# JGCRI/hector

Hardware: AMD Instinct MI355X
Metric: ensemble-member simulated years/sec (higher is better)
Workload: dtype f64

## Files before the change

hector_amd/csrc/ensemble_core.cpp:

```cpp
#include "ensemble_core.hpp"

#include <atomic>
#include <chrono>
#include <cstdint>
#include <cstdio>
#include <cstdlib>
#include <algorithm>
#include <cmath>
#include <cstring>
#include <dlfcn.h>
#include <fstream>
#include <sstream>
#include <string>
#include <stdexcept>
#include <map>
#include <mutex>

hipError_t hx_launch_spinup(int B, const HxArgs *d_args, int nmem_launch, int *d_steps,
                            hipStream_t st);
int hx_track_value_rows(int B);
int hx_pair_available();
hipError_t hx_launch_run_pair(const HxArgs *d_args, int npad, bool heatflux, bool kpm, int iy_from,
                              int iy_to, hipStream_t st, bool cons, int nbiome);
hipError_t hx_launch_prewarm(const int *d_stop, long long max_ticks, double *d_sink, int waves,
                             const double *mem, unsigned long long n_mem, hipStream_t st);
hipError_t hx_launch_run(int B, const HxArgs *d_args, int npad, bool heatflux, bool kpm, int con,
                         int iy_from, int iy_to, hipStream_t st, bool two_wave, int cus);
int hx_doeclim_block_years();
void hx_fill_chem_table_host(double *t);
hipError_t hx_launch_broadcast(double *table, int nrows, int npad, hipStream_t st);
hipError_t hx_launch_broadcast_u32(unsigned *v, int npad, hipStream_t st);
hipError_t hx_launch_alk(const HxArgs *d_args, int nmem_launch, hipStream_t st);
hipError_t hx_launch_or_flags(unsigned *status, const double *flag_row, int npad, hipStream_t st);
hipError_t hx_launch_gas(const double *par, const double *ser, const double *h0, int nh, int ns,
                         int npad, double *n2o_out, double *rf_other_out, hipStream_t st);
hipError_t hx_launch_diag(int kind, const HxDiagArgs &a, double *out, hipStream_t st);
hipError_t hx_launch_slr(const double *tgav, int npad, int start_year, int iy_to, double *out,
                         size_t var_stride, hipStream_t st);
hipError_t hx_launch_gather(const double *src, const int *lane_of_member, double *dst, int n,
                            int npad, int nyears, hipStream_t st);
hipError_t hx_launch_stats(const double *var, int n, int npad, int iy0, int nyears,
                           double *stats, hipStream_t st);
hipError_t hx_launch_derive(const double *params, double *derived, const double *ker,
                            int ker_per_member, int ns, int nbiome, int npad, hipStream_t st);
hipError_t hx_launch_doeclim_kernel(const double *diff_row, double *ker, int ns, int count,
                                    int stride, hipStream_t st);
#ifdef HX_HOST_EMULATION
#include "hx_dev_post.h"
#else
hipError_t hx_launch_score(const double *var, int n, int npad, const int *iy, const double *obs,
                           const double *sigma, int nobs, int b0, int b1, double *out, hipStream_t st);
hipError_t hx_launch_metric(const double *var, int n, int npad, const void *groups, int ngroups,
                            const int *rows, int year_start, double *out, hipStream_t st);
hipError_t hx_launch_pair_metric(const double *a, const double *b, const double *bvec, int bvec_iy0, int n,
                                 int npad, const void *specs, int nspecs, double *out, hipStream_t st);
hipError_t hx_launch_series_ew(int op, const double *a, const double *b, const double *bvec, const double *base,
                               int npad, int ns, int y_lo, int y_hi, double c0, double c1, double *z,
                               hipStream_t st);
hipError_t hx_launch_series_base(const double *a, int npad, int r0, int r1, double *base, hipStream_t st);
hipError_t hx_launch_series_cumsum(const double *a, int npad, int ns, int y0, int y_hi, double *z,
                                   hipStream_t st);
hipError_t hx_launch_series_runmean(const double *a, int npad, int ns, int w, int back, int y_hi, double *z,
                                    hipStream_t st);
hipError_t hx_launch_series_permute(const double *src, const int *src_lane, int npad, int ns, double *dst,
                                    hipStream_t st);
hipError_t hx_launch_mseries_fill(const double *row, int ns, int npad, double *table, hipStream_t st);
hipError_t hx_launch_mseries_mix(const double *coeff, const int *member_of_lane, int n, int npad, const int *rows,
                                 const double *basis, int nrows, int nbasis, double *table, hipStream_t st);
hipError_t hx_launch_bin(const double *var, int n, int npad, int iy0, int nrows, const unsigned long long *q,
                         const double *edges, int K, unsigned long long *sums, hipStream_t stream);
hipError_t hx_launch_q_minmax(const double *var, int n, int npad, int iy0, int ny,
                              const unsigned long long *q, void *st, hipStream_t stream);
hipError_t hx_launch_q_init(const void *st, int ny, const double *probs, int np, int skip, int *lo,
                            unsigned long long *prefix, unsigned long long *rem, hipStream_t stream);
hipError_t hx_launch_q_hist(const double *var, int n, int npad, int iy0, int ny,
                            const unsigned long long *q, const int *lo, const unsigned long long *prefix,
                            int np, int aggregate, unsigned long long *hist, hipStream_t stream);
hipError_t hx_launch_q_pick(int ny, int *lo, unsigned long long *prefix, unsigned long long *rem, int np,
                            unsigned long long *hist, hipStream_t stream);
hipError_t hx_launch_mom_prepare(const unsigned long long *q_mem, const double *pred_mem, int npred, int n,
                                 int npad, const int *lane_of_member, const double *c,
                                 unsigned long long *q_lane, double *qd_lane, double *e_lane, hipStream_t st);
int hx_mom_chunks(int n);
hipError_t hx_launch_moments(const double *var, int n, int npad, int iy0, int nrows, const double *qd,
                             const double *e, int npred, const double *shift, double *part, double *out,
                             hipStream_t st);
hipError_t hx_launch_grp_prepare(const int *lab_mem, int n, int npad, const int *lane_of_member, int *lab_lane,
                                 hipStream_t st);
hipError_t hx_launch_gmom_prepare(const unsigned long long *q_mem, const double *pred_mem, const int *lab_mem,
                                  int npred, int n, int npad, const int *lane_of_member, const double *c,
                                  unsigned long long *q_lane, double *qd_lane, double *e_lane, int *lab_lane,
                                  hipStream_t st);
hipError_t hx_launch_gq_minmax(const double *var, int n, int npad, int iy0, int ny, const unsigned long long *q,
                               const int *lab, int G, void *st, hipStream_t stream);
hipError_t hx_launch_gq_hist(const double *var, int n, int npad, int iy0, int ny, const unsigned long long *q,
                             const int *lab, int G, const int *lo, const unsigned long long *prefix, int np,
                             unsigned long long *hist, hipStream_t stream);
hipError_t hx_launch_gbin(const double *var, int n, int npad, int iy0, int nrows, const unsigned long long *q,
                          const int *lab, int G, const double *edges, int K, unsigned long long *sums,
                          hipStream_t stream);
hipError_t hx_launch_gmoments(const double *var, int n, int npad, int iy0, int nrows, const double *qd,
                              const double *e, const int *lab, int G, int npred, const double *shift,
                              double *part, double *out, hipStream_t st);
int hx_sobol_chunks(int nb);
hipError_t hx_launch_sobol_prepare(const int *lane_of_member, int npad, int k, int nb, const unsigned char *use,
                                   int *tab, unsigned char *flag, hipStream_t st);
hipError_t hx_launch_sobol_part(const double *var, int npad, int iy0, int nrows, const int *tab, int nb, int k,
                                const unsigned char *flag, void *st, unsigned char *on, hipStream_t stream);
hipError_t hx_launch_sobol_sums(const double *var, int npad, int iy0, int nrows, const int *tab, int nb, int k,
                                const void *st, const unsigned char *on, double *part, double *sums, double *shift,
                                long long *npart, hipStream_t stream);
hipError_t hx_launch_co_mask(const double *va, int ia0, int na, const double *vb, int ib0, int nb, int npad,
                             unsigned long long *q_lane, double *qd_lane, hipStream_t st);
int hx_co_chunks(int n, int na, int nb);
hipError_t hx_launch_co_gram(const double *va, int ia0, int na, const double *vb, int ib0, int nb, int n,
                             int npad, int sym, const double *qd, const double *shift_a,
                             const double *shift_b, double *part, double *cross, hipStream_t st);
int hx_sw_padded(int n);
void hx_sw_pack(const double *whiten, int n, double *wf);
hipError_t hx_launch_score_whiten(const double *var, int nmem, int npad, const int *iy, const double *obs,
                                  const double *wf, int n, const double *base, double *out, hipStream_t st);
int hx_project_steps(int n);
void hx_project_pack(const double *basis, int n, int m, double *bf);
hipError_t hx_launch_project(const double *var, int nmem, int npad, const int *iy, const double *center,
// ... 9 lines not shown
namespace {

struct ParamDef {
  const char *name; int row; bool per_biome; const char *units; bool spinup;
};
const ParamDef kParams[] = {
    {"S", HXP_S, false, "degC", false},
    {"diff", HXP_DIFF, false, "cm2/s", false},
    {"qco2", HXP_QCO2, false, "W/m2", false},
    {"aero_scalar", HXP_AERO, false, "(unitless)", false},
    {"vol_scalar", HXP_VOL, false, "(unitless)", false},
    {"C0", HXP_C0, false, "ppmv CO2", true},
    {"tt", HXP_TT, false, "m3/s", true},
    {"tu", HXP_TU, false, "m3/s", true},
    {"twi", HXP_TWI, false, "m3/s", true},
    {"tid", HXP_TID, false, "m3/s", true},
    {"preind_surface_c", HXP_PRE_SURF, false, "Pg C", true},
    {"preind_interdeep_c", HXP_PRE_ID, false, "Pg C", true},
    {"lo_warming_ratio", HXP_LO_RATIO, false, "(unitless)", false},
    {"beta", HXPB_BETA, true, "(unitless)", false},
    {"q10_rh", HXPB_Q10, true, "(unitless)", false},
    {"warmingfactor", HXPB_WF, true, "(unitless)", false},
    {"npp_flux0", HXPB_NPP0, true, "Pg C/yr", true},
    {"veg_c", HXPB_VEG0, true, "Pg C", true},
    {"detritus_c", HXPB_DET0, true, "Pg C", true},
    {"soil_c", HXPB_SOIL0, true, "Pg C", true},
    {"permafrost_c", HXPB_PF0, true, "Pg C", true},
    {"f_nppv", HXPB_F_NPPV, true, "(unitless)", true},
    {"f_nppd", HXPB_F_NPPD, true, "(unitless)", true},
    {"f_litterd", HXPB_F_LITTERD, true, "(unitless)", true},
    {"rh_ch4_frac", HXPB_RH_CH4_FRAC, true, "(unitless)", false},
    {"pf_mu", HXPB_PF_MU, true, "degC", false},
    {"pf_sigma", HXPB_PF_SIGMA, true, "degC", false},
    {"fpf_static", HXPB_FPF_STATIC, true, "(unitless)", false},
};

struct OutDef { const char *name; int idx; };
const OutDef kOutputs[] = {
    {"sst", HXO_SST}, {"land_tas", HXO_TLAND}, {"CO2_concentration", HXO_CO2},
    {"global_tas", HXO_TGAV}, {"RF_tot", HXO_RF_TOT}, {"RF_CO2", HXO_RF_CO2},
    {"ocean_c", HXO_OCEAN_C}, {"HL_pH", HXO_HL_PH}, {"atmos_co2", HXO_ATMOS_C},
    {"permafrost_c", HXO_PERMAFROST_C}, {"heatflux", HXO_HEATFLUX},
    {"CH4_concentration", HXO_CH4}, {"O3_concentration", HXO_O3}, {"veg_c", HXO_VEG_C},
    {"detritus_c", HXO_DET_C}, {"soil_c", HXO_SOIL_C}, {"thawedp_c", HXO_THAWED_C},
    {"earth_c", HXO_EARTH_C}, {"NBP", HXO_NBP}, {"ocean_uptake", HXO_OCEAN_UPTAKE},
    {"timesteps", HXO_NSTASH}, {"solver_steps", HXO_NSTEPS}, {"LL_pH", HXO_LL_PH},
    {"sst_reported", HXO_SST_LO},
    {"NPP", HXO_NPP}, {"RH", HXO_RH}, {"rh_det", HXO_RH_DET}, {"rh_soil", HXO_RH_SOIL},
    {"HL_ocean_uptake", HXO_HL_UPTAKE}, {"LL_ocean_uptake", HXO_LL_UPTAKE},
    {"HL_downwelling", HXO_HL_DO}, {"atmos_c_residual", HXO_CA_RESIDUAL},
    {"rh_ch4", HXO_RH_CH4}, {"f_frozen", HXO_F_FROZEN}, {"gmst", HXO_GMST},
    {"heatflux_mixed", HXO_FLUX_MIXED}, {"heatflux_interior", HXO_FLUX_INTERIOR},
    {"HL_ocean_c", HXO_C_HL}, {"LL_ocean_c", HXO_C_LL}, {"IO_ocean_c", HXO_C_IO},
    {"DO_ocean_c", HXO_C_DO}, {"HL_PCO2", HXO_PCO2_HL}, {"LL_PCO2", HXO_PCO2_LL},
    {"TAU_OH", HXO_TAU_OH},
};
const char *kOutputNames[HXO_NVAR];

struct DerivedDef { const char *name; int kind; int box; const char *deps[4]; };
enum { DK_SLR = 100, DK_SL_RC, DK_SLR_NI, DK_SL_RC_NI };
const DerivedDef kDerived[] = {
    {"HL_sst", HXG_TEMP, 0, {"sst"}}, {"LL_sst", HXG_TEMP, 1, {"sst"}},
    {"HL_DIC", HXG_DIC, 0, {"HL_ocean_c"}}, {"LL_DIC", HXG_DIC, 1, {"LL_ocean_c"}},
    {"HL_CO3", HXG_CO3, 0, {"sst", "HL_pH", "HL_PCO2"}},
    {"LL_CO3", HXG_CO3, 1, {"sst", "LL_pH", "LL_PCO2"}},
    {"HL_OmegaAr", HXG_OMEGA_AR, 0, {"sst", "HL_pH", "HL_PCO2"}},
    {"LL_OmegaAr", HXG_OMEGA_AR, 1, {"sst", "LL_pH", "LL_PCO2"}},
    {"HL_OmegaCa", HXG_OMEGA_CA, 0, {"sst", "HL_pH", "HL_PCO2"}},
    {"LL_OmegaCa", HXG_OMEGA_CA, 1, {"sst", "LL_pH", "LL_PCO2"}},
    {"HL_Revelle", HXG_REVELLE, 0, {"sst", "HL_pH", "HL_PCO2", "HL_ocean_c"}},
    {"LL_Revelle", HXG_REVELLE, 1, {"sst", "LL_pH", "LL_PCO2", "LL_ocean_c"}},
    {"ocean_tas", HXG_OCEAN_TAS, -1, {"global_tas"}},
    {"RF_N2O", HXG_RF_N2O, -1, {"CO2_concentration", "CH4_concentration"}},
    {"RF_CH4", HXG_RF_CH4, -1, {"CH4_concentration"}},
    {"RF_H2O_strat", HXG_RF_H2O, -1, {"CH4_concentration"}},
    {"RF_O3_trop", HXG_RF_O3, -1, {"O3_concentration"}},
    {"slr", DK_SLR, -1, {"global_tas"}}, {"sl_rc", DK_SL_RC, -1, {"global_tas"}},
    {"slr_no_ice", DK_SLR_NI, -1, {"global_tas"}}, {"sl_rc_no_ice", DK_SL_RC_NI, -1, {"global_tas"}},
};
const DerivedDef *derived_of(const std::string &name) {
  for (const DerivedDef &d : kDerived) if (name == d.name) return &d;
  return nullptr;
}

}

const char *const *EnsembleCore::output_capabilities(int *count) {
  for (auto &o : kOutputs) kOutputNames[o.idx] = o.name;
  if (count) *count = HXO_BIOME0;
  return kOutputNames;
}

void EnsembleCore::check(hipError_t e, const char *what) const {
  if (e != hipSuccess)
    throw std::runtime_error(std::string("HIP error in ") + what + ": " + hipGetErrorString(e));
}

EnsembleCore::EnsembleCore(const std::string &scenario_path, int n_members, int device)
    : scen_(Scenario::load(scenario_path)), n_(n_members), B_(1), device_(device) {
  if (n_members <= 0) throw std::runtime_error("n_members must be > 0");
  npad_ = (n_ + HX_WAVE - 1) / HX_WAVE * HX_WAVE;
  int ndev = 0;
  hipError_t e = hipGetDeviceCount(&ndev);
  if (e != hipSuccess || ndev <= 0)
    throw std::runtime_error(
        "hector_amd: no HIP device available -- the ensemble integrator has no CPU path");
  if (device < 0 || device >= ndev) throw std::runtime_error("invalid device index");
  check(hipSetDevice(device_), "hipSetDevice");
#ifndef HX_HOST_EMULATION
  {
    hipDeviceProp_t prop;
    check(hipGetDeviceProperties(&prop, device_), "hipGetDeviceProperties");
    simds_ = 4 * prop.multiProcessorCount;
  }
#endif
  check(hipStreamCreate(&stream_), "hipStreamCreate");
  if (const char *e2 = std::getenv("HECTOR_AMD_PAIR_MAX_MEMBERS")) pair_max_members_ = std::atoi(e2);
  if (const char *e3 = std::getenv("HECTOR_AMD_TWO_WAVE_FROM")) two_wave_from_ = std::atoi(e3);
  if (const char *e4 = std::getenv("HECTOR_AMD_PAIR_ORDER")) pair_costly_with_cheap_ = std::atoi(e4) != 0;
  if (const char *e5 = std::getenv("HECTOR_AMD_KEY_ORDER")) key_order_mode_ = std::atoi(e5);
  if (const char *e6 = std::getenv("HECTOR_AMD_COST_MODEL")) cost_model_ = std::atoi(e6) != 0;
  if (const char *e7 = std::getenv("HECTOR_AMD_SIMDS")) simds_ = std::max(1, std::atoi(e7));
  if (const char *e8 = std::getenv("HECTOR_AMD_PREWARM_MS")) prewarm_ms_ = std::max(0, std::atoi(e8));
  try {
    check(hipEventCreate(&ev0_), "hipEventCreate");
    check(hipEventCreate(&ev1_), "hipEventCreate");
    init_from_scenario();
  } catch (...) {
    if (ev0_) (void)hipEventDestroy(ev0_);
    if (ev1_) (void)hipEventDestroy(ev1_);
    (void)hipStreamDestroy(stream_);
    throw;
  }
}

void EnsembleCore::init_from_scenario() {
  for (int v = 0; v < HXO_NVAR; ++v) { d_out_[v] = nullptr; out_enabled_[v] = false; }
  out_enabled_[HXO_SST] = out_enabled_[HXO_TLAND] = true;
  out_enabled_[HXO_CO2] = out_enabled_[HXO_TGAV] = true;
  biome_names_ = {"global"};
  params_.assign(HX_NPARAM(1), std::vector<double>((size_t)npad_, 0.0));
  row_uniform_.assign(HX_NPARAM(1), true);
  auto setrow = [&](int row, double v) { std::fill(params_[row].begin(), params_[row].end(), v); };
  const Scenario &s = scen_;
  tracking_year_ = (int)s.scalar("core", "trackingDate", 0.0);
  if (tracking_year_ >= 9999 || tracking_year_ < 0) tracking_year_ = 0;
  setrow(HXP_S, s.scalar("temperature", "S"));
  setrow(HXP_DIFF, s.scalar("temperature", "diff"));
  setrow(HXP_QCO2, s.scalar("temperature", "qco2"));
  setrow(HXP_AERO, s.scalar("forcing", "aero_scalar", 1.0));
  setrow(HXP_VOL, s.scalar("forcing", "vol_scalar", 1.0));
  setrow(HXP_C0, s.scalar("simpleNbox", "C0"));
  setrow(HXP_TT, s.scalar("ocean", "tt"));
  setrow(HXP_TU, s.scalar("ocean", "tu"));
  setrow(HXP_TWI, s.scalar("ocean", "twi"));
  setrow(HXP_TID, s.scalar("ocean", "tid"));
  setrow(HXP_PRE_SURF, s.scalar("ocean", "preind_surface_c", 900));
  setrow(HXP_PRE_ID, s.scalar("ocean", "preind_interdeep_c", 37100));
  setrow(HXP_LO_RATIO, s.scalar("temperature", "lo_warming_ratio", 0.0));
  out_enabled_[HXO_SST_LO] = s.scalar("temperature", "lo_warming_ratio", 0.0) != 0.0;
  const int r = HXP_NGLOBAL;
  setrow(r + HXPB_BETA, s.scalar("simpleNbox", "beta", 0.0));
  setrow(r + HXPB_Q10, s.scalar("simpleNbox", "q10_rh", 0.0));
  setrow(r + HXPB_WF, s.scalar("simpleNbox", "warmingfactor", 1.0));
  setrow(r + HXPB_NPP0, s.scalar("simpleNbox", "npp_flux0", 0.0));
  setrow(r + HXPB_VEG0, s.scalar("simpleNbox", "veg_c", 0.0));
// ... 333 lines not shown
  check(hipMalloc(&d_derived_, sizeof(double) * np * HX_NDERIVED(B_)), "hipMalloc derived");
  check(hipMalloc(&d_lane_of_member_, sizeof(int) * np), "hipMalloc lane map");
  if (history_) {
    check(hipMalloc(&d_hist_, sizeof(double) * ns * np * HX_NSTATE(B_)), "hipMalloc state history");
    check(hipMalloc(&d_hist_status_, sizeof(unsigned) * ns * np), "hipMalloc status history");
  }
  if (spin_record_) {
    const size_t bytes = sizeof(double) * (size_t)kc_.max_spinup * HXSR_N * np;
    size_t free_b = 0, total_b = 0;
    if (hipMemGetInfo(&free_b, &total_b) == hipSuccess && bytes > free_b)
      throw std::runtime_error("spinup record: " + std::to_string(kc_.max_spinup) + " steps x " +
                               std::to_string((int)HXSR_N) + " variables x " + std::to_string(npad_) +
                               " members need " + std::to_string(bytes >> 20) + " MiB of device memory, " +
                               std::to_string(free_b >> 20) + " MiB are free");
    check(hipMalloc(&d_spin_rec_, bytes), "hipMalloc spinup record");
    check(hipMemsetAsync(d_spin_rec_, 0, bytes, stream_), "zero");
  }
  hist_valid_to_ = 0;
  check(hipMalloc(&d_dpart_, sizeof(double) * np * 2 * (size_t)hx_doeclim_block_years()),
        "hipMalloc doeclim partial sums");
  check(hipMalloc(&d_cost_, sizeof(double) * np), "hipMalloc lane cost");
  check(hipMalloc(&d_wave_clk_, sizeof(long long) * 4 * (np / HX_WAVE)), "hipMalloc wave clock");
  check(hipMemsetAsync(d_wave_clk_, 0, sizeof(long long) * 4 * (np / HX_WAVE), stream_), "zero");
  check(hipMalloc(&d_bscratch_, sizeof(double) * np * (size_t)(3 * B_)), "hipMalloc biome scratch");
  check(hipMemsetAsync(d_bscratch_, 0, sizeof(double) * np * (size_t)(3 * B_), stream_), "zero");
  cost_from_iy_ = -1;
  for (int v = 0; v < HXO_NVAR; ++v)
    if (out_enabled_[v]) {
      check(hipMalloc(&d_out_[v], sizeof(double) * ns * np), "hipMalloc out");
      check(hipMemsetAsync(d_out_[v], 0, sizeof(double) * ns * np, stream_), "memset out");
    }
  check(hipMemcpyAsync(d_shared_, shared_.data(), sizeof(double) * shared_.size(),
                       hipMemcpyHostToDevice, stream_), "upload shared");
  layout_dirty_ = false;
  params_dirty_ = true;
  rows_all_dirty_ = true;
  need_spinup_ = true; spin_valid_ = false;
}

HxBuffers EnsembleCore::buffers() const {
  HxBuffers b;
  b.params = d_params_; b.derived = d_derived_; b.state = d_state_; b.status = d_status_; b.shared = d_shared_;
  b.ker = d_ker_;
  b.dpart = d_dpart_;
  b.dpart2 = d_dpart_ ? d_dpart_ + (size_t)npad_ * hx_doeclim_block_years() : nullptr;
  for (int v = 0; v < HXO_NVAR; ++v) b.out[v] = d_out_[v];
  b.hist = d_hist_; b.hist_status = d_hist_status_;
  for (int k = 0; k < HXM_N; ++k) b.mseries[k] = d_mseries_[k];
  b.uparams = d_uparams_;
  b.uderived = d_uparams_ ? d_uparams_ + HX_NPARAM(B_) : nullptr;
  b.uni_k = (row_uniform_[HXP_TT] && row_uniform_[HXP_TU] && row_uniform_[HXP_TWI] && row_uniform_[HXP_TID]) ? 1 : 0;
  b.uni_avc = (row_uniform_[HXP_AERO] && row_uniform_[HXP_VOL] && row_uniform_[HXP_C0]) ? 1 : 0;
  b.uni_wf = 1;
  for (int bb = 0; bb < B_; ++bb) if (!row_uniform_[HXP_NGLOBAL + bb * HXPB_N + HXPB_WF]) b.uni_wf = 0;
  b.track_out_f = d_track_out_f_; b.track_out_v = d_track_out_v_;
  b.trk_slots = trk_iy() >= 0 ? scen_.ns() - trk_iy() + 1 : 0;
  b.uni_landk = b.uni_bio = 1;
  for (int bb = 0; bb < B_; ++bb) {
    const int r = HXP_NGLOBAL + bb * HXPB_N;
    for (int k : {HXPB_NPP0, HXPB_F_NPPV, HXPB_F_NPPD, HXPB_F_LITTERD, HXPB_RH_CH4_FRAC, HXPB_FPF_STATIC})
      if (!row_uniform_[r + k]) b.uni_landk = 0;
    for (int k : {HXPB_BETA, HXPB_PF_MU, HXPB_PF_SIGMA})
      if (!row_uniform_[r + k]) b.uni_bio = 0;
  }
  b.stash_diag = b.biome_diag = b.out_rare = 0;
  for (int v = 0; v < HXO_NVAR; ++v)
    if (d_out_[v] && v != HXO_SST && v != HXO_TLAND && v != HXO_CO2 && v != HXO_TGAV) b.out_rare = 1;
  for (int v = HXO_NPP; v <= HXO_CA_RESIDUAL; ++v) if (d_out_[v]) b.stash_diag = 1;
  for (int v = HXO_BIOME0; v < HXO_NVAR; ++v) if (d_out_[v]) b.biome_diag = 1;
  for (int bb = 0; bb < HX_BDYN; ++bb)
    if (d_out_[HXO_B(HXOB_NPP, bb)] || d_out_[HXO_B(HXOB_RH, bb)]) b.stash_diag = 1;
  b.out_mask0 = 0; b.ms_mask = 0;
  for (int v = 0; v < HXO_BIOME0; ++v) if (d_out_[v]) b.out_mask0 |= 1ull << v;
  for (int bb = 0; bb < HX_BDYN; ++bb)
    if (d_out_[HXO_B(HXOB_NPP, bb)] || d_out_[HXO_B(HXOB_RH, bb)]) b.out_mask0 |= 1ull << HX_OM_BIOME_FLUX;
  if (b.biome_diag) b.out_mask0 |= 1ull << HX_OM_BIOME_ANY;
  for (int k = 0; k < HXM_N; ++k) if (d_mseries_[k]) b.ms_mask |= 1u << k;
  b.n = n_; b.npad = npad_; b.ker_per_member = ker_per_member_ ? 1 : 0;
  b.nbiome = B_;
  b.cost = d_cost_;
  b.spin_rec = d_spin_rec_;
  b.bscratch = d_bscratch_;
  b.wave_clk = d_wave_clk_;
  return b;
}

int EnsembleCore::resolve_param(const std::string &capability, const ParamRef **) const {
  std::string biome, var = capability;
  size_t dot = capability.find('.');
  if (dot != std::string::npos) { biome = capability.substr(0, dot); var = capability.substr(dot + 1); }
  for (const ParamDef &d : kParams) {
    if (var != d.name) continue;
    if (!d.per_biome) {
      if (!biome.empty()) throw std::runtime_error("variable " + var + " takes no biome prefix");
      return d.row;
    }
    int b = -1;
    if (biome.empty()) biome = "global";
    for (int i = 0; i < B_; ++i) if (biome_names_[i] == biome) b = i;
    if (b < 0)
      throw std::runtime_error("Biome '" + biome + "' missing from biome list. Hit this error "
                               "while trying to retrieve variable: '" + capability + "'.");
    return HXP_NGLOBAL + b * HXPB_N + d.row;
  }
  throw std::runtime_error("Unknown variable name while parsing: " + capability);
}

static const ParamDef &def_of(const std::string &capability) {
  std::string var = capability;
  size_t dot = capability.find('.');
  if (dot != std::string::npos) var = capability.substr(dot + 1);
  for (const ParamDef &d : kParams) if (var == d.name) return d;
  throw std::runtime_error("Unknown variable name while parsing: " + capability);
}

namespace {
struct SharedParamDef { const char *name, *section, *units; };
const SharedParamDef kSharedParams[] = {
    {"M0", "CH4", "ppbv CH4"}, {"Tsoil", "CH4", "Years"}, {"Tstrat", "CH4", "Years"},
    {"N0", "N2O", "ppbv N2O"}, {"PO3", "ozone", "DU O3"}, {"TOH0", "OH", "Years"},
    {"delta_co2", "forcing", "(unitless)"}, {"delta_ch4", "forcing", "(unitless)"},
    {"delta_n2o", "forcing", "(unitless)"}, {"rho_bc", "forcing", "W/m2/Tg"},
    {"rho_oc", "forcing", "W/m2/Tg"}, {"rho_so2", "forcing", "W/m2/Gg"},
    {"rho_nh3", "forcing", "W/m2/Tg"},
    {"TN2O0", "N2O", "Years"}, {"UC_N2O", "N2O", "Tg/ppbv"},
};
}

static std::string shared_param_section(const Scenario &scen, const std::string &capability,
                                        std::string *units, std::string *key = nullptr) {
  if (key) *key = capability;
  for (const SharedParamDef &d : kSharedParams)
    if (capability == d.name) { if (units) *units = d.units; return d.section; }
  for (const Halocarbon &h : scen.halocarbons) {
    if (capability == "rho_" + h.name) { if (units) *units = "W/m2/pptv"; return h.name + "_halocarbon"; }
    if (capability == "delta_" + h.name) { if (units) *units = "(unitless)"; return h.name + "_halocarbon"; }
    if (capability == "tau_" + h.name) {
      if (units) *units = "Years";
      if (key) *key = "tau";
      return h.name + "_halocarbon";
    }
  }
  return "";
}

static bool gas_member_capable(const Scenario &scen, const std::string &capability) {
  if (capability == "N0" || capability == "TN2O0" || capability == "UC_N2O") return true;
  for (const Halocarbon &h : scen.halocarbons)
    if (capability == "rho_" + h.name || capability == "delta_" + h.name || capability == "tau_" + h.name)
      return true;
  return false;
}

void EnsembleCore::setvar(const std::string &capability, const double *values, int nvalues,
                          const char *units) {
  if (std::count(capability.begin(), capability.end(), '.') > 1)
    throw std::runtime_error("Invalid input variable: '" + capability + "'");
  if (capability == "trackingDate") {
    set_tracking_date((int)values[0]);
    return;
  }
  {
    std::string expect, key;
    const std::string sec = shared_param_section(scen_, capability, &expect, &key);
    if (!sec.empty()) {
      if (units && units[0] && expect != units)
// ... 564 lines not shown
      if (!std::isnan(pt.second[(size_t)m])) pts.emplace_hint(pts.end(), pt.first, pt.second[(size_t)m]);
    const std::vector<double> dense = Scenario::densify_points(pts, capability, scen_.start, scen_.end);
    for (size_t iy = 0; iy < dense.size(); ++iy) ms[iy * (size_t)n_ + (size_t)m] = dense[iy];
  }
}

void EnsembleCore::upload_member_series() {
  const size_t np = (size_t)npad_, ns = (size_t)scen_.ns();
  std::vector<double> flat;
  for (const MemberSeriesDef &d : kMemberSeries) {
    const std::vector<double> &ms = member_series_[d.k];
    if (ms.empty() && !mix_[d.k].nbasis) {
      if (d_mseries_[d.k]) {
        check(hipStreamSynchronize(stream_), "sync member series");
        (void)hipFree(d_mseries_[d.k]);
        d_mseries_[d.k] = nullptr;
      }
      continue;
    }
    if (!d_mseries_[d.k]) check(hipMalloc(&d_mseries_[d.k], sizeof(double) * ns * np), "hipMalloc member series");
    if (!ms.empty()) {
      flat.assign(ns * np, 0.0);
      for (size_t iy = (size_t)d.lag; iy < ns; ++iy)
        for (size_t l = 0; l < np; ++l)
          flat[iy * np + l] = ms[(iy - (size_t)d.lag) * n_ + (size_t)std::min(member_of_lane_[l], n_ - 1)];
      check(hipMemcpyAsync(d_mseries_[d.k], flat.data(), sizeof(double) * flat.size(),
                           hipMemcpyHostToDevice, stream_), "upload member series");
      check(hipStreamSynchronize(stream_), "sync member series");
    }
    if (mix_[d.k].nbasis) build_mix_table(d.k, d.lag, d.section, d.name, !ms.empty());
  }
  upload_args();
  mseries_dirty_ = false;
}

void EnsembleCore::build_mix_table(int k, int lag, const std::string &section, const std::string &capability,
                                   bool dense) {
  const MemberMix &mx = mix_[k];
  const size_t np = (size_t)npad_, ns = (size_t)scen_.ns(), ny = mx.years.size(), K = (size_t)mx.nbasis;
  std::vector<int> ints(member_of_lane_.begin(), member_of_lane_.begin() + (std::ptrdiff_t)np);
  std::vector<size_t> col;
  for (size_t i = 0; i < ny; ++i) {
    const size_t r = (size_t)(mx.years[i] - scen_.start + lag);
    if (r < ns) { ints.push_back((int)r); col.push_back(i); }
  }
  const size_t nr = col.size();
  std::vector<double> dbl(ns + K * nr);
  if (!dense && scen_.has_series(section, capability)) {
    const std::vector<double> &base = scen_.series(section, capability);
    for (size_t iy = (size_t)lag; iy < ns; ++iy) dbl[iy] = base[iy - (size_t)lag];
  }
  for (size_t kk = 0; kk < K; ++kk)
    for (size_t j = 0; j < nr; ++j) dbl[ns + kk * nr + j] = mx.basis[kk * ny + col[j]];
  const size_t b_dbl = sizeof(double) * dbl.size(), b_coeff = sizeof(double) * K * (size_t)n_,
               b_int = sizeof(int) * ints.size();
  if (b_dbl + b_coeff + b_int > mix_cap_) {
    check(hipStreamSynchronize(stream_), "sync mix scratch");
    if (d_mix_) (void)hipFree(d_mix_);
    d_mix_ = nullptr; mix_cap_ = 0;
    check(hipMalloc(&d_mix_, b_dbl + b_coeff + b_int), "hipMalloc mix scratch");
    mix_cap_ = b_dbl + b_coeff + b_int;
  }
  double *d_dbl = reinterpret_cast<double *>(d_mix_), *d_coeff = d_dbl + dbl.size();
  int *d_int = reinterpret_cast<int *>(d_mix_ + b_dbl + b_coeff);
  check(hipMemcpyAsync(d_dbl, dbl.data(), b_dbl, hipMemcpyHostToDevice, stream_), "upload mix basis");
  check(hipMemcpyAsync(d_coeff, mx.coeff.data(), b_coeff, hipMemcpyHostToDevice, stream_), "upload mix coefficients");
  check(hipMemcpyAsync(d_int, ints.data(), b_int, hipMemcpyHostToDevice, stream_), "upload mix rows");
  if (!dense) check(hx_launch_mseries_fill(d_dbl, (int)ns, npad_, d_mseries_[k], stream_), "member series fill kernel");
  if (nr)
    check(hx_launch_mseries_mix(d_coeff, d_int, n_, npad_, d_int + np, d_dbl + ns, (int)nr, mx.nbasis,
                                d_mseries_[k], stream_), "member series mix kernel");
  check(hipStreamSynchronize(stream_), "sync member series mix");
}

void EnsembleCore::upload_args() {
  HxArgs a;
  a.buf = buffers();
  a.kc = kc_;
  for (int k = 0; k < HXM_N; ++k)
    if (!member_series_[k].empty()) a.kc.con_mask |= constraint_bit(k);
  member_con_mask_ = a.kc.con_mask & ~kc_.con_mask;
  check(hipMemcpyAsync(d_args_, &a, sizeof a, hipMemcpyHostToDevice, stream_), "upload args");
  check(hipStreamSynchronize(stream_), "sync args");
}

void EnsembleCore::run_gas_kernel() {
  gas_dirty_ = false;
  auto fr = [](void *p) { if (p) (void)hipFree(p); };
  if (gas_member_.empty()) {
    if (d_mseries_[HXM_N2O]) {
      sync();
      fr(d_mseries_[HXM_N2O]); fr(d_mseries_[HXM_RF_OTHER]);
      d_mseries_[HXM_N2O] = d_mseries_[HXM_RF_OTHER] = nullptr;
      upload_args();
    }
    return;
  }
  const Scenario &s = scen_;
  const size_t np = (size_t)npad_, ns = (size_t)s.ns();
  const size_t nh = s.halocarbons.size();
  std::vector<size_t> horder(nh);
  for (size_t h = 0; h < nh; ++h) horder[h] = h;
  std::sort(horder.begin(), horder.end(), [&](size_t a, size_t b) {
    return s.halocarbons[a].name < s.halocarbons[b].name;
  });
  auto member_value = [&](const std::string &cap, double dflt, size_t lane) {
    auto it = gas_member_.find(cap);
    if (it == gas_member_.end()) return dflt;
    return it->second[(size_t)std::min(member_of_lane_[lane], n_ - 1)];
  };
  std::vector<double> par((3 + 3 * nh) * np), ser((4 + 2 * nh) * ns), h0(nh);
  for (size_t l = 0; l < np; ++l) {
    par[l] = member_value("N0", s.scalar("N2O", "N0"), l);
    par[np + l] = member_value("TN2O0", s.scalar("N2O", "TN2O0"), l);
    par[2 * np + l] = member_value("UC_N2O", s.scalar("N2O", "UC_N2O"), l);
    for (size_t k = 0; k < nh; ++k) {
      const Halocarbon &H = s.halocarbons[horder[k]];
      par[(3 + 3 * k) * np + l] = member_value("tau_" + H.name, H.tau, l);
      par[(4 + 3 * k) * np + l] = component_disabled(H.name + "_halocarbon")
                                      ? 0.0 : member_value("rho_" + H.name, H.rho, l);
      par[(5 + 3 * k) * np + l] = member_value("delta_" + H.name, H.delta, l);
    }
  }
  const auto &n2o_em = s.series("N2O", "N2O_emissions");
  const auto &n2o_nat = s.series("N2O", "N2O_natural_emissions");
  const std::vector<double> nanv(ns, std::nan(""));
  auto con = [&](const std::string &sec, const std::string &key) -> const std::vector<double> & {
    return s.has_series(sec, key) ? s.series(sec, key) : nanv;
  };
  const auto &n2o_con = con("N2O", "N2O_constrain");
  const auto albedo = s.has_series("simpleNbox", "RF_albedo") ? s.series("simpleNbox", "RF_albedo")
                                                                : std::vector<double>(ns, -0.2);
  const auto misc = s.has_series("forcing", "RF_misc") ? s.series("forcing", "RF_misc")
                                                        : std::vector<double>(ns, 0.0);
  for (size_t iy = 0; iy < ns; ++iy) {
    ser[iy] = n2o_em[iy] + n2o_nat[iy];
    ser[ns + iy] = n2o_con[iy];
    ser[2 * ns + iy] = albedo[iy];
    ser[3 * ns + iy] = misc[iy];
  }
  for (size_t k = 0; k < nh; ++k) {
    const Halocarbon &H = s.halocarbons[horder[k]];
    const auto &hc = con(H.name + "_halocarbon", H.name + "_constrain");
    h0[k] = H.H0;
    for (size_t iy = 0; iy < ns; ++iy) {
      const double emissMol = H.emissions[iy] / H.molarMass * 1.0;
      ser[(4 + 2 * k) * ns + iy] = emissMol / (0.1 * 1.8);
      ser[(5 + 2 * k) * ns + iy] = hc[iy];
    }
  }
  sync();
  fr(d_gas_par_); fr(d_gas_ser_);
  d_gas_par_ = d_gas_ser_ = nullptr;
  double *d_h0 = nullptr;
  check(hipMalloc(&d_gas_par_, sizeof(double) * par.size()), "hipMalloc gas parameters");
  check(hipMalloc(&d_gas_ser_, sizeof(double) * (ser.size() + nh)), "hipMalloc gas series");
  d_h0 = d_gas_ser_ + ser.size();
  if (!d_mseries_[HXM_N2O]) {
    check(hipMalloc(&d_mseries_[HXM_N2O], sizeof(double) * ns * np), "hipMalloc N2O series");
    check(hipMalloc(&d_mseries_[HXM_RF_OTHER], sizeof(double) * ns * np), "hipMalloc RF series");
  }
  check(hipMemcpyAsync(d_gas_par_, par.data(), sizeof(double) * par.size(), hipMemcpyHostToDevice,
                       stream_), "upload gas parameters");
  check(hipMemcpyAsync(d_gas_ser_, ser.data(), sizeof(double) * ser.size(), hipMemcpyHostToDevice,
                       stream_), "upload gas series");
  check(hipMemcpyAsync(d_h0, h0.data(), sizeof(double) * nh, hipMemcpyHostToDevice, stream_),
// ... 452 lines not shown
  if (!(kc_.delta_n2o >= -1 && kc_.delta_n2o <= 1)) throw std::runtime_error("bad delta N2O value");
  if (!(kc_.delta_co2 >= -1 && kc_.delta_co2 <= 1)) throw std::runtime_error("bad delta CO2 value");
}

void EnsembleCore::prepare() {
  check(hipSetDevice(device_), "hipSetDevice");
  StageClock clk;
  if (layout_dirty_) { alloc_device(); clk.lap("alloc_device"); }
  if (shared_dirty_ || params_dirty_ || need_spinup_) prewarm_begin();
  if (shared_dirty_) {
    build_shared();
    check(hipMemcpyAsync(d_shared_, shared_.data(), sizeof(double) * shared_.size(),
                         hipMemcpyHostToDevice, stream_), "upload shared");
    check(hipStreamSynchronize(stream_), "sync shared");
    shared_dirty_ = false;
    params_dirty_ = true;
  }
  if (params_dirty_) {
    check_parameters();
    clk.lap("check_parameters");
    upload_params();
    clk.lap("upload_params");
    if (order_changed_)
      for (int k = 0; k < HXM_N; ++k)
        if (!member_series_[k].empty() || mix_[k].nbasis) mseries_dirty_ = true;
    gas_dirty_ = true;
  }
  if (gas_dirty_ || (!gas_member_.empty() && !d_mseries_[HXM_N2O])) run_gas_kernel();
  if (mseries_dirty_) upload_member_series();
  clk.lap("gas kernel / member series");
  if (!need_spinup_) return;
  bool uniform = true;
  for (const ParamDef &d : kParams) {
    if (!d.spinup) continue;
    if (d.per_biome) {
      for (int b = 0; b < B_; ++b)
        if (!row_uniform_[HXP_NGLOBAL + b * HXPB_N + d.row]) uniform = false;
    } else if (!row_uniform_[d.row]) uniform = false;
  }
  const size_t np = (size_t)npad_;
  const bool reuse = spin_valid_ && uniform && spin_uniform_ && !std::getenv("HECTOR_AMD_ALWAYS_SPINUP");
  spin_uniform_ = uniform;
  if (reuse) {
    check(hipMemcpyAsync(d_state_, d_state_ + np * HX_NSTATE(B_), sizeof(double) * np * HX_NSTATE(B_),
                         hipMemcpyDeviceToDevice, stream_), "restore state");
    check(hipMemcpyAsync(d_status_, d_status_ + 2 * np, sizeof(unsigned) * np, hipMemcpyDeviceToDevice,
                         stream_), "restore status");
  } else {
    if (!uniform || std::getenv("HECTOR_AMD_PREWARM_STOP")) prewarm_end();
    check(hipEventRecord(ev0_, stream_), "event");
    check(hx_launch_spinup(B_, d_args_, uniform ? 1 : npad_, d_spin_steps_, stream_), "spinup");
    check(hx_launch_alk(d_args_, uniform ? 1 : npad_, stream_), "alkalinity tuning");
    if (uniform) {
      check(hx_launch_broadcast(d_state_, HX_NSTATE(B_), npad_, stream_), "broadcast state");
      check(hx_launch_broadcast_u32(d_status_, npad_, stream_), "broadcast status");
      check(hx_launch_broadcast_u32(reinterpret_cast<unsigned *>(d_spin_steps_), npad_, stream_),
            "broadcast steps");
      for (int v = 0; v < HXO_NVAR; ++v)
        if (d_out_[v]) check(hx_launch_broadcast(d_out_[v], 1, npad_, stream_), "broadcast out");
    }
    check(hipMemcpyAsync(d_status_ + 2 * np, d_status_, sizeof(unsigned) * np, hipMemcpyDeviceToDevice,
                         stream_), "keep spinup status");
  }
  check(hx_launch_or_flags(d_status_, d_derived_ + (size_t)HXD_FLAG * npad_, npad_, stream_),
        "derive flags");
  if (!reuse)
    check(hipMemcpyAsync(d_state_ + np * HX_NSTATE(B_), d_state_, sizeof(double) * np * HX_NSTATE(B_),
                         hipMemcpyDeviceToDevice, stream_), "snapshot state");
  check(hipMemcpyAsync(d_status_ + np, d_status_, sizeof(unsigned) * np, hipMemcpyDeviceToDevice,
                       stream_), "snapshot status");
  if (reuse) {
    spin_ms_ = 0.0;
    clk.lap("post-spinup state reused");
  } else {
    check(hipEventRecord(ev1_, stream_), "event");
    check(hipEventSynchronize(ev1_), "spinup sync");
    float ms = 0;
    check(hipEventElapsedTime(&ms, ev0_, ev1_), "elapsed");
    spin_ms_ = ms;
    clk.lap("spinup + snapshot (waited)");
  }
  spin_valid_ = uniform;
  need_spinup_ = false;
  ++out_epoch_;
  last_iy_ = 0;
  hist_valid_to_ = 0;
  dirty_from_iy_ = -1;
}

void EnsembleCore::reset(double date) {
  ++out_epoch_;
  if (date < scen_.start) {
    need_spinup_ = true; spin_valid_ = false;
    last_iy_ = 0;
    dirty_from_iy_ = -1;
    return;
  }
  const int iy = (int)date - scen_.start;
  if (iy == 0 && !(need_spinup_ || layout_dirty_ || params_dirty_)) maybe_calibrate_lanes();
  if (need_spinup_ || layout_dirty_ || params_dirty_) {
    if (iy != 0) throw std::runtime_error("reset: the core has pending changes from date 0");
    prepare();
    return;
  }
  if (iy == last_iy_) return;
  if (iy > last_iy_) throw std::runtime_error("reset: date is after the current date");
  const size_t np = (size_t)npad_, rows = (size_t)HX_NSTATE(B_);
  sync();
  if (iy == 0) {
    check(hipMemcpyAsync(d_state_, d_state_ + np * rows, sizeof(double) * np * rows,
                         hipMemcpyDeviceToDevice, stream_), "restore state");
    check(hipMemcpyAsync(d_status_, d_status_ + np, sizeof(unsigned) * np, hipMemcpyDeviceToDevice,
                         stream_), "restore status");
  } else {
    if (!d_hist_ || iy > hist_valid_to_)
      throw std::runtime_error("reset: no state history for that date (enable_history() before "
                               "running; only reset(0) and reset(startDate) work without it)");
    check(hipMemcpyAsync(d_state_, d_hist_ + (size_t)iy * rows * np, sizeof(double) * np * rows,
                         hipMemcpyDeviceToDevice, stream_), "restore state from history");
    check(hipMemcpyAsync(d_status_, d_hist_status_ + (size_t)iy * np, sizeof(unsigned) * np,
                         hipMemcpyDeviceToDevice, stream_), "restore status from history");
  }
  last_iy_ = iy;
  cost_from_iy_ = -1;
  if (dirty_from_iy_ >= iy) dirty_from_iy_ = -1;
}

void EnsembleCore::prewarm_begin() {
#ifndef HX_HOST_EMULATION
  if (prewarm_ms_ <= 0 || prewarm_on_) return;
  {
    const double now = std::chrono::duration<double>(std::chrono::steady_clock::now().time_since_epoch()).count();
    if (last_gpu_activity_s_ >= 0 && now - last_gpu_activity_s_ < 0.005) return;
  }
  if (!aux_stream_) check(hipStreamCreateWithFlags(&aux_stream_, hipStreamNonBlocking), "prewarm stream");
  if (!d_prewarm_) check(hipMalloc((void **)&d_prewarm_, 64 + sizeof(double) * 1024), "prewarm flag");
  check(hipMemsetAsync(d_prewarm_, 0, 64, aux_stream_), "prewarm flag");
  int waves = 3 * simds_;
  if (const char *e = std::getenv("HECTOR_AMD_PREWARM_WAVES")) waves = std::max(1, std::min(8 * simds_, std::atoi(e)));
  const bool sweep = std::getenv("HECTOR_AMD_PREWARM_MEM") && d_out_[HXO_SST];
  check(hx_launch_prewarm(reinterpret_cast<const int *>(d_prewarm_), (long long)prewarm_ms_ * 100000ll,
                          reinterpret_cast<double *>(d_prewarm_ + 64), waves,
                          sweep ? d_out_[HXO_SST] : nullptr,
                          sweep ? (unsigned long long)scen_.ns() * (unsigned long long)npad_ : 0ull, aux_stream_),
        "prewarm kernel");
  prewarm_on_ = true;
#endif
}
void EnsembleCore::prewarm_end() {
#ifndef HX_HOST_EMULATION
  if (!prewarm_on_) return;
  check(hipMemsetAsync(d_prewarm_, 1, 4, stream_), "prewarm stop");
  prewarm_on_ = false;
  last_run_prewarmed_ = true;
#endif
}

void EnsembleCore::run(double runtodate) {
  prepare();
  if (runtodate < 0.0) runtodate = scen_.end;
  if (runtodate > scen_.end)
    throw std::runtime_error("Requested run-to date is after the configured end date.");
  const int target = (int)runtodate - scen_.start;
  if (dirty_from_iy_ >= 0 && dirty_from_iy_ < last_iy_) {
    const int back = (d_hist_ && dirty_from_iy_ <= hist_valid_to_) ? dirty_from_iy_ : 0;
    dirty_from_iy_ = -1;
    reset((double)(scen_.start + back));
  }
  dirty_from_iy_ = -1;
  if (target < last_iy_ + 1) return;
  if (last_iy_ == 0) {
    check(hipMemsetAsync(d_cost_, 0, sizeof(double) * (size_t)npad_, stream_), "zero lane cost");
    cost_from_iy_ = 0;
  }
  last_run_prewarmed_ = false;
  prewarm_end();
  check(hipEventRecord(ev0_, stream_), "event");
  const bool hf = d_out_[HXO_HEATFLUX] || d_out_[HXO_FLUX_MIXED] || d_out_[HXO_FLUX_INTERIOR];
  const int con_mask = kc_.con_mask | member_con_mask_;
  bool ext = con_mask != 0;
  for (int v = HXO_NPP; v < HXO_NVAR; ++v) if (d_out_[v]) ext = true;
  for (int k = 0; k < HXM_N; ++k) if (d_mseries_[k]) ext = true;
  const bool force_nbp = getenv("HECTOR_AMD_EXTENDED_NBP") != nullptr;
  int con = ext ? (((con_mask & HXC_NBP) || force_nbp) ? 1 : -1) : 0;
  if (con == -1 && con_mask == 0 && !getenv("HECTOR_AMD_EXTENDED_CONS")) {
    bool any_ms = false;
    for (int k = 0; k < HXM_N; ++k) if (d_mseries_[k]) any_ms = true;
    if (!any_ms && B_ >= 1 && B_ <= 4) con = -2;
  }
  if (d_track_out_f_) {
    if (con_mask & (HXC_CO2 | HXC_NBP))
      throw std::runtime_error("carbon tracking together with a CO2 or NBP constraint is not "
                               "supported (the constraint residual is an untracked source)");
    con = 2;
  }
  const int pair_cons = con_mask & (HXC_CO2 | HXC_TAS | HXC_FTOT | HXC_CH4);
  bool plain = (con_mask & ~(HXC_CO2 | HXC_TAS | HXC_FTOT | HXC_CH4)) == 0 && !d_track_out_f_ &&
               !(pair_cons && ker_per_member_);
  for (int k = 0; k < HXM_N; ++k) if (d_mseries_[k]) plain = false;
  bool pair = hx_pair_available() && B_ <= 4 && plain && n_ <= pair_max_members_;
  if (B_ > 1 && (ker_per_member_ || d_out_[HXO_HEATFLUX])) pair = false;
  for (int v = 0; v < HXO_NVAR && pair; ++v)
    if (d_out_[v]) {
      static const int ok[] = {HXO_SST, HXO_TLAND, HXO_CO2, HXO_TGAV, HXO_NSTASH, HXO_RF_TOT, HXO_RF_CO2,
                               HXO_ATMOS_C, HXO_OCEAN_C, HXO_OCEAN_UPTAKE, HXO_HL_PH, HXO_LL_PH, HXO_CH4,
                               HXO_O3, HXO_NBP, HXO_VEG_C, HXO_DET_C, HXO_SOIL_C, HXO_PERMAFROST_C,
                               HXO_THAWED_C, HXO_EARTH_C, HXO_HEATFLUX, HXO_NPP, HXO_RH, HXO_RH_DET,
                               HXO_RH_SOIL, HXO_RH_CH4, HXO_F_FROZEN, HXO_GMST};
      if (std::find(std::begin(ok), std::end(ok), v) == std::end(ok)) pair = false;
      if (B_ > 1 && (v == HXO_NPP || v == HXO_RH || v == HXO_RH_DET || v == HXO_RH_SOIL)) pair = false;
    }
  last_run_pair_ = pair;
  const bool w2 = !pair && con <= 1 && two_wave_expected();
  last_run_w2_ = w2;
  last_run_con_ = con;
  if (pair)
    check(hx_launch_run_pair(d_args_, npad_, d_out_[HXO_HEATFLUX] != nullptr, ker_per_member_, last_iy_, target,
                             stream_, pair_cons != 0, B_), "run kernel (pair)");
  else
  check(hx_launch_run(B_, d_args_, npad_, hf || con == 2, ker_per_member_, con, last_iy_, target,
                      stream_, w2, simds_ / 4),
        "run kernel");
  check(hipEventRecord(ev1_, stream_), "event");
  run_timed_ = true;
  slr_valid_to_ = -1;
  ++out_epoch_;
  if (d_hist_) hist_valid_to_ = target;
  last_iy_ = target;
}

void EnsembleCore::sync() {
  check(hipStreamSynchronize(stream_), "stream sync");
  last_gpu_activity_s_ = std::chrono::duration<double>(std::chrono::steady_clock::now().time_since_epoch()).count();
  if (run_timed_) {
    float ms = 0;
    check(hipEventElapsedTime(&ms, ev0_, ev1_), "elapsed");
    run_ms_ = ms;
    run_timed_ = false;
  }
}

int EnsembleCore::wave_clock(long long *ticks, int cap) {
  if (!d_wave_clk_ || last_iy_ == 0) return 0;
  sync();
  const int nw = (npad_ / HX_WAVE) * (last_run_pair_ ? 2 : 1);
  std::vector<long long> t((size_t)nw * 2);
  check(hipMemcpy(t.data(), d_wave_clk_, sizeof(long long) * t.size(), hipMemcpyDeviceToHost), "wave clock");
  long long t0 = t[0];
  for (int w = 0; w < nw; ++w) t0 = std::min(t0, t[(size_t)2 * w]);
  const int n = std::min(nw, cap);
  for (int w = 0; w < n; ++w) { ticks[2 * w] = t[(size_t)2 * w] - t0; ticks[2 * w + 1] = t[(size_t)2 * w + 1] - t0; }
  return n;
}

bool EnsembleCore::fetch_host(const std::string &capability_in, int year0, int year1,
                              double *out_host) {
  const std::string capability = capability_in.compare(0, 4, "Fadj") == 0
// ... 380 lines not shown
  {
    static const char *const combos[][3] = {{"pH", "LL_pH", "HL_pH"}, {"PCO2", "LL_PCO2", "HL_PCO2"},
                                            {"DIC", "LL_DIC", "HL_DIC"}, {"CO3", "LL_CO3", "HL_CO3"},
                                            {"ML_ocean_c", "LL_ocean_c", "HL_ocean_c"}};
    for (auto &c : combos)
      if (capability == c[0]) {
        const size_t cnt = (size_t)(year1 - year0 + 1) * (size_t)n_;
        std::vector<double> hl(cnt);
        fetchvars(c[1], year0, year1, out_host);
        fetchvars(c[2], year0, year1, hl.data());
        const bool sum = capability == "ML_ocean_c";
        const double part_high = 0.15, part_low = 1 - 0.15;
        for (size_t i = 0; i < cnt; ++i)
          out_host[i] = sum ? out_host[i] + hl[i] : part_low * out_host[i] + part_high * hl[i];
        return;
      }
  }
  const bool n2o_members = capability == "N2O_concentration" && d_mseries_[HXM_N2O];
  const DerivedDef *dd = derived_of(capability);
  const int si = find_series(capability);
  const int v = (dd || n2o_members || si >= 0) ? -1 : out_index(capability);
  if (!dd && !n2o_members && si < 0 && !d_out_[v])
    throw std::runtime_error("variable " + capability + " was not enabled with set_outputs()");
  if (si >= 0 && (year0 < scen_.start || year1 > scen_.start + series_[(size_t)si].valid_iy || year1 < year0))
    throw std::runtime_error("fetchvars: dates must lie between startDate and " +
                             std::to_string(scen_.start + series_[(size_t)si].valid_iy) + ", the date series " +
                             capability + " was defined at");
  if (si < 0 && (year0 < scen_.start || year1 > last_date() || year1 < year0))
    throw std::runtime_error("fetchvars: dates must lie between startDate and the current date");
  sync();
  const int iy0 = year0 - scen_.start, ny = year1 - year0 + 1;
  const size_t need = (size_t)ny * (size_t)n_;
  if (need > gather_cap_) {
    if (d_gather_) (void)hipFree(d_gather_);
    d_gather_ = nullptr;
    check(hipMalloc(&d_gather_, sizeof(double) * need), "hipMalloc gather");
    gather_cap_ = need;
  }
  const double *src = nullptr;
  if (dd) {
    const size_t dneed = (size_t)ny * (size_t)npad_;
    if (dneed > diag_cap_) {
      if (d_diag_) (void)hipFree(d_diag_);
      d_diag_ = nullptr;
      check(hipMalloc(&d_diag_, sizeof(double) * dneed), "hipMalloc diag");
      diag_cap_ = dneed;
    }
    compute_derived(capability, iy0, ny, d_diag_);
    src = d_diag_;
  } else if (si >= 0) {
    series_to_current_lanes(series_[(size_t)si]);
    src = series_[(size_t)si].block + (size_t)iy0 * npad_;
  } else if (n2o_members) {
    src = d_mseries_[HXM_N2O] + (size_t)iy0 * npad_;
  } else {
    src = d_out_[v] + (size_t)iy0 * npad_;
  }
  check(hx_launch_gather(src, d_lane_of_member_, d_gather_, n_, npad_, ny, stream_), "gather");
  if (row_pitch)
    check(hipMemcpy2DAsync(out_host, sizeof(double) * row_pitch, d_gather_, sizeof(double) * (size_t)n_,
                           sizeof(double) * (size_t)n_, (size_t)ny, hipMemcpyDeviceToHost, stream_), "fetch");
  else
    check(hipMemcpyAsync(out_host, d_gather_, sizeof(double) * need, hipMemcpyDeviceToHost, stream_),
          "fetch");
  check(hipStreamSynchronize(stream_), "fetch sync");
}

const double *EnsembleCore::device_var(const std::string &capability, int *npad) {
  const PostSource ps = post_source(capability, "hx_device_var");
  if (ps.v >= 0 && !d_out_[ps.v])
    throw std::runtime_error("variable " + capability + " was not enabled with set_outputs()");
  if (npad) *npad = npad_;
  return ps.block;
}

void EnsembleCore::stats_device(const std::string &capability, int year0, int year1,
                                double *d_stats) {
  stats_async(capability, year0, year1, d_stats);
  check(hipStreamSynchronize(stream_), "stats sync");
}

void EnsembleCore::stats_async(const std::string &capability, int year0, int year1,
                               double *d_stats) {
  const PostSource ps = post_source(capability, "stats");
  if (ps.v >= 0 && !d_out_[ps.v])
    throw std::runtime_error("variable " + capability + " was not enabled with set_outputs()");
  if (year0 < scen_.start || year1 > scen_.start + ps.last_iy || year1 < year0)
    throw std::runtime_error("stats: dates must lie between startDate and the current date");
  check(hx_launch_stats(ps.block, n_, npad_, year0 - scen_.start, year1 - year0 + 1, d_stats,
                        stream_), "stats kernel");
}

void EnsembleCore::status(unsigned *out_host) {
  prepare();
  sync();
  std::vector<unsigned> tmp((size_t)npad_);
  check(hipMemcpy(tmp.data(), d_status_, sizeof(unsigned) * (size_t)npad_, hipMemcpyDeviceToHost),
        "status");
  for (int i = 0; i < n_; ++i) out_host[i] = tmp[(size_t)lane_of_member_[(size_t)i]];
}

void EnsembleCore::state_row(int row, double *out_host) {
  prepare();
  sync();
  if (row < 0 || row >= HX_NSTATE(B_)) throw std::runtime_error("state_row: bad row");
  std::vector<double> tmp((size_t)npad_);
  check(hipMemcpy(tmp.data(), d_state_ + (size_t)row * npad_, sizeof(double) * (size_t)npad_,
                  hipMemcpyDeviceToHost), "state row");
  for (int i = 0; i < n_; ++i) out_host[i] = tmp[(size_t)lane_of_member_[(size_t)i]];
}

int EnsembleCore::spinup_steps(int member) {
  prepare();
  sync();
  int v = 0;
  if (member < 0 || member >= n_) throw std::runtime_error("spinup_steps: bad member index");
  check(hipMemcpy(&v, d_spin_steps_ + lane_of_member_[(size_t)member], sizeof(int),
                  hipMemcpyDeviceToHost), "steps");
  return v;
}


int EnsembleCore::member_score(const std::string &capability, const int *years, const double *obs,
                               const double *sigma, int n, int base_year0, int base_year1,
                               double *out_host) {
  if (n < 1 || !years || !obs || !out_host)
    throw std::runtime_error("hx_member_score: n < 1 or a null argument");
  const PostSource ps = post_source(capability, "hx_member_score");
  if (ps.v >= 0 && !d_out_[ps.v])
    throw std::runtime_error("variable " + capability + " was not enabled with set_outputs()");
  const int last = scen_.start + ps.last_iy;
  const bool has_base = base_year0 <= base_year1;
  std::vector<int> iy((size_t)n);
  int used = 0;
  for (int i = 0; i < n; ++i) {
    if (years[i] < scen_.start || years[i] > last)
      throw std::runtime_error("hx_member_score: dates must lie between startDate and the current date");
    iy[(size_t)i] = years[i] - scen_.start;
    if (obs[i] == obs[i]) ++used;
  }
  if (has_base && (base_year0 < scen_.start || base_year1 > last))
    throw std::runtime_error("hx_member_score: the reference period must lie between startDate and the current date");
  if (!d_lane_of_member_) throw std::runtime_error("hx_member_score: run the core first");
  sync();
  const size_t nn = (size_t)n, doubles = 2 * nn + (size_t)npad_ + (size_t)n_;
  const size_t bytes = sizeof(double) * doubles + sizeof(int) * nn;
  if (bytes > score_cap_) {
    if (d_score_) (void)hipFree(d_score_);
    d_score_ = nullptr; score_cap_ = 0;
    check(hipMalloc(&d_score_, bytes), "hipMalloc score");
    score_cap_ = bytes;
  }
  double *d_obs = d_score_, *d_sig = d_obs + nn, *d_lane = d_sig + nn, *d_mem = d_lane + npad_;
  int *d_iy = reinterpret_cast<int *>(d_mem + n_);
  check(hipMemcpyAsync(d_obs, obs, sizeof(double) * nn, hipMemcpyHostToDevice, stream_), "score obs");
  if (sigma)
    check(hipMemcpyAsync(d_sig, sigma, sizeof(double) * nn, hipMemcpyHostToDevice, stream_), "score sigma");
  check(hipMemcpyAsync(d_iy, iy.data(), sizeof(int) * nn, hipMemcpyHostToDevice, stream_), "score years");
  check(hx_launch_score(ps.block, n_, npad_, d_iy, d_obs, sigma ? d_sig : nullptr, n,
                        has_base ? base_year0 - scen_.start : 1, has_base ? base_year1 - scen_.start : 0,
                        d_lane, stream_), "score kernel");
  check(hx_launch_gather(d_lane, d_lane_of_member_, d_mem, n_, npad_, 1, stream_), "score gather");
  check(hipMemcpyAsync(out_host, d_mem, sizeof(double) * (size_t)n_, hipMemcpyDeviceToHost, stream_), "score fetch");
  check(hipStreamSynchronize(stream_), "score sync");
  return used;
}

int hxq_host_start(const unsigned long long *st, unsigned long long *pre) {
  *pre = 0;
  if (st[3] == 0) return 0;
  const unsigned long long kmin = ~st[0], diff = kmin ^ st[1];
  if (!diff) { *pre = kmin; return 0; }
  int lo = 0;
  while (lo < 64 && (diff >> lo)) ++lo;
  if (lo < 64) *pre = (kmin >> lo) << lo;
  return lo;
}
unsigned long long hxq_host_target(double p, unsigned long long W) {
  const double t = std::ceil(p * (double)W);
  return t < 1.0 ? 1ull : (unsigned long long)t;
}
void hxq_host_pick(int lo, const unsigned long long *hist, unsigned long long *prefix,
                   unsigned long long *rem) {
  const int shift = lo >= 8 ? lo - 8 : 0;
  unsigned long long cum = 0, bin = 255;
  for (unsigned long long b = 0; b < 256; ++b) {
// ... 1442 lines not shown
```

hector_amd/csrc/ensemble_core.hpp:

```cpp
#pragma once
#include <hip/hip_runtime.h>

#include <cstdint>
#include <map>
#include <string>
#include <vector>

#include "../../include/hector_amd.h"
#include "hx_layout.h"
#include "hx_scenario.hpp"

namespace hx {

int hx_cost_models_export_file(const char *path);
int hx_cost_models_load_file(const char *path);

struct PairCall {
  const char *cap_b;
  const double *b_vec;
  int b_year0, b_year1;
  const hx_pair_metric *specs;
  int nspecs;
};

class EnsembleCore {
 public:
  EnsembleCore(const std::string &scenario_path, int n_members, int device);
  ~EnsembleCore();
  EnsembleCore(const EnsembleCore &) = delete;
  EnsembleCore &operator=(const EnsembleCore &) = delete;

  int n_members() const { return n_; }
  int n_biomes() const { return B_; }
  int start_date() const { return scen_.start; }
  int end_date() const { return scen_.end; }
  int last_date() const { return scen_.start + last_iy_; }
  const std::vector<std::string> &biomes() const { return biome_names_; }

  void setvar(const std::string &capability, const double *values, int nvalues,
              const char *units);
  void getvar(const std::string &capability, double *out) const;

  void split_biome(const std::vector<std::string> &names, const double *fveg,
                   const double *fdet, const double *fsoil, const double *fpf,
                   const double *fnpp);
  void split_biome_of(const std::string &old_biome, const std::vector<std::string> &names,
                      const double *fveg, const double *fdet, const double *fsoil,
                      const double *fpf, const double *fnpp);
  void create_biome(const std::string &biome);
  void delete_biome(const std::string &biome);
  void rename_biome(const std::string &oldname, const std::string &newname);
  int biome_index(const std::string &biome) const;

  void set_outputs(const std::vector<std::string> &capabilities);
  void set_member_sorting(bool on);
  void set_lane_calibration(bool on) { calibrate_lanes_ = on; }
  bool lanes_calibrated() const { return !lane_cost_.empty(); }
  int lane_order_source() const { return lane_order_source_; }
  void set_cost_model(bool on) { cost_model_ = on; }
  void set_prewarm(int ms) { prewarm_ms_ = ms < 0 ? 0 : (ms > 200 ? 200 : ms); }
  int prewarm_ms() const { return prewarm_ms_; }
  bool last_run_prewarmed() const { return last_run_prewarmed_; }
  void enable_history(bool on);
  void enable_spinup_record(bool on);
  static const std::vector<std::string> &spinup_record_vars();
  int spinup_record(int member, double *values, int max_steps);
  void setvar_dated(const std::string &capability, const int *years, const double *values,
                    int n, const char *units);
  void lane_of_member(int *out);
  void setvar_dated_members(const std::string &capability, const int *years, const double *values,
                            int nyears, const char *units);
  void setvar_dated_mix(const std::string &capability, const int *years, int nyears, const double *basis,
                        int nbasis, const double *coeff, const char *units);
  void check_dated_mix(const std::string &capability, const int *years, int nyears, const double *basis,
                       int nbasis, const double *coeff, const char *units) const;
  static const char *const *output_capabilities(int *count);

  void reset(double date);
  void run(double runtodate);
  void sync();
  void fetchvars(const std::string &capability, int year0, int year1, double *out_host,
                 size_t row_pitch = 0);
  bool host_output(const std::string &capability);
  void set_tracking_date(int year);
  int tracking_date() const { return tracking_year_; }
  std::vector<std::string> tracking_pools() const;
  void tracking_data(int member, int year0, int year1, double *values, double *fractions,
                     unsigned long long *source_masks = nullptr);
  std::string run_name() const;
  void var_info(const std::string &capability, std::string *component, std::string *units) const;
  const std::vector<std::string> &halocarbon_names() const { return halo_names_; }
  const double *device_var(const std::string &capability, int *npad);
  void stats_device(const std::string &capability, int year0, int year1, double *d_stats);
  void stats_async(const std::string &capability, int year0, int year1, double *d_stats);
  int member_score(const std::string &capability, const int *years, const double *obs,
                   const double *sigma, int n, int base_year0, int base_year1, double *out_host);
  void member_score_whitened(const std::string &capability, const int *years, const double *obs,
                             const double *whiten, int n, int base_year0, int base_year1, double *out_host);
  void member_project(const std::string &capability, const int *years, const double *center,
                      const double *basis, int n, int m, int base_year0, int base_year1, double *out_host,
                      size_t row_pitch = 0);
  void quantiles(const std::string &capability, int year0, int year1, const unsigned long long *q,
                 const double *probs, int nprobs, double *out_host, long long *n_part);
  void q_begin(const std::string &capability, int year0, int year1, const unsigned long long *q,
               int nprobs, unsigned long long *st_host);
  void q_pass(const int *lo, const unsigned long long *prefix, unsigned long long *hist_host);
  void member_metrics(const std::string &capability, const hx_metric *specs, int nspecs,
                      double *out_host, const char *fn = "hx_member_metrics");
  void metric_quantiles(const std::string &capability, const hx_metric *specs, int nspecs,
                        const unsigned long long *q, const double *probs, int nprobs, double *out_host,
                        long long *n_part);
  void mq_begin(const std::string &capability, const hx_metric *specs, int nspecs,
                const unsigned long long *q, int nprobs, unsigned long long *st_host);
  void bin_sums(const std::string &capability, int year0, int year1, const unsigned long long *q,
                const double *edges, int nedges, unsigned long long *sums_host);
  void metric_bin_sums(const std::string &capability, const hx_metric *specs, int nspecs,
                       const unsigned long long *q, const double *edges, int nedges,
                       unsigned long long *sums_host);
  void mom_begin(const std::string &capability, int year0, int year1, const hx_metric *specs, int nspecs,
                 const unsigned long long *q, const double *pred, int npred, const double *c,
                 unsigned long long *st_host, const char *fn);
  void mom_finish(const double *shift_host, double *sums_host);
  void grp_quantiles(const std::string &capability, int year0, int year1, const hx_metric *specs, int nspecs,
                     const int *labels, int ngroups, const unsigned long long *q, const double *probs,
                     int nprobs, double *out_host, long long *n_part, const char *fn);
  void grp_q_begin(const std::string &capability, int year0, int year1, const hx_metric *specs, int nspecs,
                   const int *labels, int ngroups, const unsigned long long *q, int nprobs,
                   unsigned long long *st_host, const char *fn);
  void grp_bin_sums(const std::string &capability, int year0, int year1, const hx_metric *specs, int nspecs,
                    const int *labels, int ngroups, const unsigned long long *q, const double *edges,
                    int nedges, unsigned long long *sums_host, const char *fn);
  void grp_mom_begin(const std::string &capability, int year0, int year1, const hx_metric *specs, int nspecs,
                     const int *labels, int ngroups, const unsigned long long *q, const double *pred,
                     int npred, const double *c, unsigned long long *st_host, const char *fn);
  void grp_mom_finish(const double *shift_host, double *sums_host);
  void member_pair_metrics(const std::string &cap_a, const PairCall &pc, double *out_host, size_t row_pitch = 0);
  void pair_metric_quantiles(const std::string &cap_a, const PairCall &pc, const unsigned long long *q,
                             const double *probs, int nprobs, double *out_host, long long *n_part);
  void pmq_begin(const std::string &cap_a, const PairCall &pc, const unsigned long long *q, int nprobs,
                 unsigned long long *st_host);
  void pair_metric_bin_sums(const std::string &cap_a, const PairCall &pc, const unsigned long long *q,
                            const double *edges, int nedges, unsigned long long *sums_host);
  void pair_mom_begin(const std::string &cap_a, const PairCall &pc, const unsigned long long *q,
                      const double *pred, int npred, const double *c, unsigned long long *st_host);
  void comom_check(const std::string &cap_a, int a0, int a1, const std::string *cap_b, int b0, int b1);
  void comom_begin(const std::string &cap_a, int a0, int a1, const std::string *cap_b, int b0, int b1,
                   const unsigned long long *q, unsigned long long *st_host);
  void comom_finish(const double *shift_host, double *sums_host, double *cross_host);
  void sobol_check(const std::string &capability, int year0, int year1, const hx_metric *specs, int nspecs,
                   const char *fn);
  void sobol_begin(const std::string &capability, int year0, int year1, const hx_metric *specs, int nspecs,
                   int k, int n_base, const unsigned char *use, const char *fn);
  void sobol_finish(double *shift_host, double *sums_host, long long *n_part_host);
  void series_define(const std::string &name, const std::string &a, const hx_series_op &op);
  void series_drop(const std::string &name);
  void series_list(std::vector<std::string> *names, std::vector<int> *valid_to) const;
  int device() const { return device_; }
  void status(unsigned *out_host);
  void state_row(int row, double *out_host);
  int spinup_steps(int member);

  double last_run_kernel_ms() const { return run_ms_; }
  bool component_output_enabled(const std::string &section) const { return scen_.scalar(section, "output", 1.0) > 0; }
  void set_pair_kernel_limit(int max_members) { pair_max_members_ = max_members < 0 ? 0 : max_members; }
  void set_two_wave_from(int min_members) { two_wave_from_ = min_members; }
  int wave_clock(long long *ticks, int cap);
  const char *last_run_kernel() const { return last_run_pair_ ? "pair" : last_run_w2_ ? "run2" : "run"; }
  int last_run_variant() const { return last_run_con_; }
  double last_spinup_ms() const { return spin_ms_; }
  hipStream_t stream() const { return stream_; }

 private:
  struct ParamRef { int row; bool per_biome; const char *units; bool affects_spinup; };
  int resolve_param(const std::string &capability, const ParamRef **ref) const;
  int out_index(const std::string &capability) const;
  void build_shared();
  void alloc_device();
  void free_device();
  void upload_params();
  void prepare();
  HxBuffers buffers() const;
  void check(hipError_t e, const char *what) const;

  Scenario scen_;
  int n_, npad_, B_, device_;
  std::vector<std::string> biome_names_;
  std::vector<std::vector<double>> params_;
  std::vector<bool> row_uniform_;
  std::vector<int> member_of_lane_, lane_of_member_;
  bool sort_members_ = true, calibrate_lanes_ = true;
  std::vector<double> lane_cost_;
  double *d_cost_ = nullptr;
  long long *d_wave_clk_ = nullptr;
  double *d_bscratch_ = nullptr;
  int cost_from_iy_ = -1;
  void maybe_calibrate_lanes();
  uint64_t cost_model_key(const std::vector<int> &varying) const;
  void fit_cost_model(const std::vector<double> &member_cost);
  bool predict_cost(const std::vector<int> &varying, std::vector<double> &out) const;
  int lane_order_source_ = 0;
  bool cost_model_ = true, cost_fitted_ = false;
  void assign_lanes();
  bool params_dirty_ = true, need_spinup_ = true, layout_dirty_ = true, ker_per_member_ = false;
  std::vector<char> row_dirty_;
  bool rows_all_dirty_ = true, order_changed_ = true;
  std::vector<int> uploaded_order_;
  bool spin_valid_ = false;
  int last_iy_ = 0;
  HxConst kc_{};
  std::vector<double> member_series_[HXM_N];
  std::map<int, std::vector<double>> member_points_[HXM_N];
  void densify_member_constraint(int k, const std::string &capability);
  double *d_mseries_[HXM_N] = {};
  bool mseries_dirty_ = false;
  void upload_member_series();
  struct MemberMix {
    int nbasis = 0;
    std::vector<int> years;
    std::vector<double> basis, coeff;
    bool covers(int year) const;
  };
  MemberMix mix_[HXM_N];
  char *d_mix_ = nullptr;
  size_t mix_cap_ = 0;
  void build_mix_table(int k, int lag, const std::string &section, const std::string &capability, bool dense);
  void upload_args();
  bool component_disabled(const std::string &section) const;
  void check_component_enabled(const std::string &capability) const;
  std::map<std::string, std::vector<double>> gas_member_;
  double *d_gas_par_ = nullptr, *d_gas_ser_ = nullptr;
  void run_gas_kernel();
  bool gas_dirty_ = false;
  int member_con_mask_ = 0;
  void init_from_scenario();
  std::vector<std::string> halo_names_;
  std::vector<std::vector<double>> halo_conc_;
  std::vector<double> shared_, ker_;
  bool out_enabled_[HXO_NVAR];
  double *d_params_ = nullptr, *d_state_ = nullptr, *d_shared_ = nullptr, *d_ker_ = nullptr;
  double *d_out_[HXO_NVAR];
  unsigned *d_status_ = nullptr;
  int *d_spin_steps_ = nullptr;
  HxArgs *d_args_ = nullptr;
  double *d_uparams_ = nullptr;
  int tracking_year_ = 0;
  double *d_track_out_f_ = nullptr, *d_track_out_v_ = nullptr;
  int trk_iy() const {
    return (tracking_year_ > scen_.start && tracking_year_ <= scen_.end) ? tracking_year_ - scen_.start : -1;
  }
  double *d_derived_ = nullptr, *d_dpart_ = nullptr, *d_gather_ = nullptr, *d_hist_ = nullptr;
  unsigned *d_hist_status_ = nullptr;
  void remap_biome_outputs(const std::vector<int> &old_of_new);
  bool history_ = false, shared_dirty_ = false;
  bool spin_record_ = false, spin_uniform_ = false;
  double *d_spin_rec_ = nullptr;
  int hist_valid_to_ = 0;
  int dirty_from_iy_ = -1;
  int *d_lane_of_member_ = nullptr;
  size_t gather_cap_ = 0, diag_cap_ = 0;
  double *d_diag_ = nullptr, *d_slr_ = nullptr;
  int slr_valid_to_ = -1;
  void check_parameters() const;
  bool fetch_host(const std::string &capability, int year0, int year1, double *out_host);
  void compute_derived(const std::string &capability, int iy0, int ny, double *dst);
  double *d_score_ = nullptr;
  size_t score_cap_ = 0;
  double *d_whiten_ = nullptr;
  size_t whiten_cap_ = 0;
  double *d_project_ = nullptr;
  size_t project_cap_ = 0;
  unsigned long long *d_q_ = nullptr;
  unsigned long long *d_qstate_ = nullptr;
  unsigned long long *d_qhist_ = nullptr;
  size_t qstate_cap_ = 0, qhist_cap_ = 0;
  const double *q_src_ = nullptr;
  int q_iy0_ = 0, q_ny_ = 0, q_np_ = 0;
  bool q_weighted_ = false;
  int post_flags_ = 0;
  const double *q_check(const std::string &capability, int year0, int year1, int nprobs,
                        const char *fn = "hx_ensemble_quantiles");
  void q_upload(const unsigned long long *q, int ny, int np);
  void q_select(const double *src, int iy0, int ny, const unsigned long long *q, const double *probs,
                int np, double *out_host, long long *n_part);
  void q_begin_block(const double *src, int iy0, int ny, const unsigned long long *q, int np,
                     unsigned long long *st_host);
  void bin_block(const double *src, int iy0, int nrows, const unsigned long long *q, const double *edges,
                 int nedges, unsigned long long *sums_host);
  unsigned char *d_metplan_ = nullptr;
  double *d_met_ = nullptr;
  size_t metplan_cap_ = 0, met_cap_ = 0;
  unsigned long long *d_bin_ = nullptr;
// ... 77 lines not shown
```

hector_amd/csrc/hx_dev_member.h:

```cpp
#pragma once

extern __shared__ double hx_dyn_park[][64];

namespace {

#define HX_FENCE() asm volatile("" ::: "memory")

#if !defined(HX_HOST_EMULATION) && !defined(HX_NO_SROW)
#define HX_SROW(p) asm("" : "+s"(p))
#else
#define HX_SROW(p)
#endif
#if !defined(HX_HOST_EMULATION) && !defined(HX_NO_VOFF)
#define HX_VOFF(o) asm("" : "+v"(o))
#else
#define HX_VOFF(o)
#endif

enum HxPark {
  PK_CH4 = 0, PK_SST, PK_EOS, PK_TLAND, PK_TWIN, PK_TL_M1, PK_TL_M2, PK_F_PREV,
  PK_BASE_TOT, PK_BASE_CO2,
  PK_LN_CH4, PK_LN_CO2R,
  PK_AERO, PK_VOL,
  PK_D0,
// ... 179 lines not shown
struct LandK<HX_DYN> {
  ParamCol npp0, f_nppv, f_nppd, f_litterd, rh_ch4_frac, fpf_static;
};
template <int B>
__device__ __forceinline__ void load_landk(const Member<B> &m, LandK<B> &k) {
  HX_FENCE();
  if constexpr (B == HX_DYN) {
    const ParamCol c{m.upar, m.bufp->params, m.npad, m.moff, 0};
    k.npp0 = c; k.npp0.col = HXPB_NPP0; k.f_nppv = c; k.f_nppv.col = HXPB_F_NPPV;
    k.f_nppd = c; k.f_nppd.col = HXPB_F_NPPD; k.f_litterd = c; k.f_litterd.col = HXPB_F_LITTERD;
    k.rh_ch4_frac = c; k.rh_ch4_frac.col = HXPB_RH_CH4_FRAC;
    k.fpf_static = c; k.fpf_static.col = HXPB_FPF_STATIC;
  } else if constexpr (hx_w2<B>()) {
    const int r = HXP_NGLOBAL;
    if (m.upar) {
      hx_ccd u = m.upar + r;
      k.npp0[0] = u[HXPB_NPP0]; k.f_nppv[0] = u[HXPB_F_NPPV]; k.f_nppd[0] = u[HXPB_F_NPPD];
      k.f_litterd[0] = u[HXPB_F_LITTERD]; k.rh_ch4_frac[0] = u[HXPB_RH_CH4_FRAC];
      k.fpf_static[0] = u[HXPB_FPF_STATIC];
    } else {
      const double *p = m.bufp->params;
      k.npp0[0] = w2_ld<true>(p, m.npad, r + HXPB_NPP0, m.moff);
      k.f_nppv[0] = w2_ld<true>(p, m.npad, r + HXPB_F_NPPV, m.moff);
      k.f_nppd[0] = w2_ld<true>(p, m.npad, r + HXPB_F_NPPD, m.moff);
      k.f_litterd[0] = w2_ld<true>(p, m.npad, r + HXPB_F_LITTERD, m.moff);
      k.rh_ch4_frac[0] = w2_ld<true>(p, m.npad, r + HXPB_RH_CH4_FRAC, m.moff);
      k.fpf_static[0] = w2_ld<true>(p, m.npad, r + HXPB_FPF_STATIC, m.moff);
    }
  } else if constexpr (B == 1) {
    constexpr int o = hx_pkb1<B>();
    k.npp0[0] = PKM(m, o + PKB_NPP0); k.f_nppv[0] = PKM(m, o + PKB_F_NPPV);
    k.f_nppd[0] = PKM(m, o + PKB_F_NPPD); k.f_litterd[0] = PKM(m, o + PKB_F_LITTERD);
    k.rh_ch4_frac[0] = PKM(m, o + PKB_RH_CH4_FRAC); k.fpf_static[0] = PKM(m, o + PKB_FPF_STATIC);
  } else {
    if (m.upar) {
#pragma unroll
      for (int b = 0; b < hx_nbc<B>(); ++b) {
        hx_ccd r = m.upar + (HXP_NGLOBAL + b * HXPB_N);
        k.npp0[b] = r[HXPB_NPP0]; k.f_nppv[b] = r[HXPB_F_NPPV]; k.f_nppd[b] = r[HXPB_F_NPPD];
        k.f_litterd[b] = r[HXPB_F_LITTERD]; k.rh_ch4_frac[b] = r[HXPB_RH_CH4_FRAC];
        k.fpf_static[b] = r[HXPB_FPF_STATIC];
      }
      return;
    }
#pragma unroll
    for (int b = 0; b < hx_nbc<B>(); ++b) {
      const int r0 = HXP_NGLOBAL + b * HXPB_N;
      if constexpr (hx_tbl<B>()) {
        const double *p = m.bufp->params;
        k.npp0[b] = w2_ld(p, m.npad, r0 + HXPB_NPP0, m.moff);
        k.f_nppv[b] = w2_ld(p, m.npad, r0 + HXPB_F_NPPV, m.moff);
        k.f_nppd[b] = w2_ld(p, m.npad, r0 + HXPB_F_NPPD, m.moff);
        k.f_litterd[b] = w2_ld(p, m.npad, r0 + HXPB_F_LITTERD, m.moff);
        k.rh_ch4_frac[b] = w2_ld(p, m.npad, r0 + HXPB_RH_CH4_FRAC, m.moff);
        k.fpf_static[b] = w2_ld(p, m.npad, r0 + HXPB_FPF_STATIC, m.moff);
      } else {
      hx_gcd r = m.par + (size_t)r0 * m.npad;
      k.npp0[b] = r[(size_t)HXPB_NPP0 * m.npad];
      k.f_nppv[b] = r[(size_t)HXPB_F_NPPV * m.npad];
      k.f_nppd[b] = r[(size_t)HXPB_F_NPPD * m.npad];
      k.f_litterd[b] = r[(size_t)HXPB_F_LITTERD * m.npad];
      k.rh_ch4_frac[b] = r[(size_t)HXPB_RH_CH4_FRAC * m.npad];
      k.fpf_static[b] = r[(size_t)HXPB_FPF_STATIC * m.npad];
      }
    }
  }
}

__device__ __forceinline__ double ldp(const HxBuffers &b, int row, int mem) {
  return HX_GCD(b.params)[(size_t)row * b.npad + mem];
}
__device__ __forceinline__ double ldd(const HxBuffers &b, int row, int mem) {
  return HX_GCD(b.derived)[(size_t)row * b.npad + mem];
}
__device__ __forceinline__ double lds_(const HxBuffers &b, int row, int mem) {
  return HX_GCD(b.state)[(size_t)row * b.npad + mem];
}
__device__ __forceinline__ void sts_(const HxBuffers &b, int row, int mem, double v) {
  HX_GD(b.state)[(size_t)row * b.npad + mem] = v;
}
__device__ __forceinline__ void sto_(const HxBuffers &b, int var, size_t off, double v) {
  HX_GD(b.out[var])[off] = v;
}

template <int B>
__device__ __forceinline__ void bind_member(const HxBuffers &buf, int mem, Member<B> &m,
                                            double (*park)[64], int lane) {
  m.bufp = &buf;
  m.par = HX_GCD(buf.params) + mem;
  m.der = HX_GCD(buf.derived) + mem;
  m.npad = buf.npad;
  m.moff = (unsigned)mem * 8u;
  m.pk = park;
  m.lane = lane;
  m.upar = (B != 1 && buf.uni_landk) ? HX_CCD(buf.uparams) : nullptr;
  m.nb = buf.nbiome;
  if constexpr (!hx_one<B>()) {
    const int bm = (B == HX_DYN) ? buf.nbiome : hx_bmax<B>();
    const int o = pk_ff0<B>() + (hx_slim_park<B>() ? 0 : bm);
    if constexpr (hx_pools_only_park<B>()) {
      ParkArr *arr[4] = {&m.veg, &m.det, &m.soil, &m.pf};
#pragma unroll
      for (int k = 0; k < 4; ++k) { arr[k]->base = park + o + k * bm; arr[k]->lane = lane; }
      m.thawed = GlobArr{buf.state, HXS_NGLOBAL + HXSB_THAWED, HXSB_N, m.npad, m.moff};
      m.tempferts = GlobArr{buf.state, HXS_NGLOBAL + HXSB_TEMPFERTS, HXSB_N, m.npad, m.moff};
      m.co2fert = GlobArr{buf.bscratch, 0, 1, m.npad, m.moff};
      m.tempfertd = GlobArr{buf.bscratch, bm, 1, m.npad, m.moff};
      m.f_new_thaw = GlobArr{buf.bscratch, 2 * bm, 1, m.npad, m.moff};
      m.ffz = GlobArr{buf.state, HXS_NGLOBAL + HXSB_F_FROZEN, HXSB_N, m.npad, m.moff};
    } else if constexpr (hx_slim_park<B>()) {
      ParkArr *arr[HX_NBIOME_ARR - 1] = {&m.veg, &m.det, &m.soil, &m.pf, &m.thawed, &m.tempferts,
                                         &m.co2fert, &m.tempfertd};
#pragma unroll
      for (int k = 0; k < HX_NBIOME_ARR - 1; ++k) { arr[k]->base = park + o + k * bm; arr[k]->lane = lane; }
      m.f_new_thaw = GlobArr{buf.bscratch, 0, 1, m.npad, m.moff};
      m.ffz = GlobArr{buf.state, HXS_NGLOBAL + HXSB_F_FROZEN, HXSB_N, m.npad, m.moff};
    } else {
    ParkArr *arr[HX_NBIOME_ARR] = {&m.veg, &m.det, &m.soil, &m.pf, &m.thawed, &m.tempferts,
                                   &m.co2fert, &m.tempfertd, &m.f_new_thaw};
#pragma unroll
    for (int k = 0; k < HX_NBIOME_ARR; ++k) {
      arr[k]->base = park + o + k * bm;
      arr[k]->lane = lane;
    }
    }
  }
  m.C0 = ldp(buf, HXP_C0, mem);
  if constexpr (!hx_w2<B>()) {
  PKM(m, PK_AERO) = ldp(buf, HXP_AERO, mem);
  PKM(m, PK_VOL) = ldp(buf, HXP_VOL, mem);
  }
  if constexpr (!hx_lean_park<B>()) {
#pragma unroll
    for (int k = 0; k < 14; ++k) PKM(m, PK_D0 + k) = ldd(buf, HXD_A0 + k, mem);
#pragma unroll
    for (int k = 0; k < 7; ++k) PKM(m, PK_K0 + k) = ldd(buf, HXD_KLH + k, mem);
  }
  if constexpr (B == 1) {
    constexpr int o = hx_pkb1<B>();
    const int r = HXP_NGLOBAL;
    PKM(m, o + PKB_NPP0) = ldp(buf, r + HXPB_NPP0, mem);
    PKM(m, o + PKB_F_NPPV) = ldp(buf, r + HXPB_F_NPPV, mem);
    PKM(m, o + PKB_F_NPPD) = ldp(buf, r + HXPB_F_NPPD, mem);
    PKM(m, o + PKB_F_LITTERD) = ldp(buf, r + HXPB_F_LITTERD, mem);
    PKM(m, o + PKB_RH_CH4_FRAC) = ldp(buf, r + HXPB_RH_CH4_FRAC, mem);
    PKM(m, o + PKB_FPF_STATIC) = ldp(buf, r + HXPB_FPF_STATIC, mem);
    PKM(m, o + PKB_BETA) = ldp(buf, r + HXPB_BETA, mem);
    PKM(m, o + PKB_WF) = ldp(buf, r + HXPB_WF, mem);
    PKM(m, o + PKB_LNQ10) = ldd(buf, HXD_NGLOBAL, mem);
    PKM(m, o + PKB_MU) = ldp(buf, r + HXPB_PF_MU, mem);
    PKM(m, o + PKB_SIGMA) = ldp(buf, r + HXPB_PF_SIGMA, mem);
  }
}

template <int B>
__device__ __forceinline__ void w2_park_out(const Member<B> &m) {
  const ChemK *k[2] = {&m.kH, &m.kL};
#pragma unroll
  for (int b = 0; b < 2; ++b) {
    const int o = 11 * b;
    PKM(m, w2_slot(o + 0)) = k[b]->A2; PKM(m, w2_slot(o + 1)) = k[b]->A1; PKM(m, w2_slot(o + 2)) = k[b]->C4;
    PKM(m, w2_slot(o + 3)) = k[b]->C3; PKM(m, w2_slot(o + 4)) = k[b]->C2; PKM(m, w2_slot(o + 5)) = k[b]->C1;
    PKM(m, w2_slot(o + 6)) = k[b]->C0; PKM(m, w2_slot(o + 7)) = k[b]->K1; PKM(m, w2_slot(o + 8)) = k[b]->K1K2;
    PKM(m, w2_slot(o + 9)) = k[b]->rKh; PKM(m, w2_slot(o + 10)) = k[b]->g;
  }
  PKM(m, w2_slot(22)) = m.cHL; PKM(m, w2_slot(23)) = m.cLL; PKM(m, w2_slot(24)) = m.hH;
  PKM(m, w2_slot(25)) = m.hL; PKM(m, w2_slot(26)) = m.pco2H; PKM(m, w2_slot(27)) = m.pco2L;
  HX_FENCE();
}
template <int B>
__device__ __forceinline__ void w2_park_in(Member<B> &m) {
  HX_FENCE();
  ChemK *k[2] = {&m.kH, &m.kL};
#pragma unroll
  for (int b = 0; b < 2; ++b) {
    const int o = 11 * b;
    k[b]->A2 = PKM(m, w2_slot(o + 0)); k[b]->A1 = PKM(m, w2_slot(o + 1)); k[b]->C4 = PKM(m, w2_slot(o + 2));
    k[b]->C3 = PKM(m, w2_slot(o + 3)); k[b]->C2 = PKM(m, w2_slot(o + 4)); k[b]->C1 = PKM(m, w2_slot(o + 5));
    k[b]->C0 = PKM(m, w2_slot(o + 6)); k[b]->K1 = PKM(m, w2_slot(o + 7)); k[b]->K1K2 = PKM(m, w2_slot(o + 8));
    k[b]->rKh = PKM(m, w2_slot(o + 9)); k[b]->g = PKM(m, w2_slot(o + 10));
  }
  m.cHL = PKM(m, w2_slot(22)); m.cLL = PKM(m, w2_slot(23)); m.hH = PKM(m, w2_slot(24));
  m.hL = PKM(m, w2_slot(25)); m.pco2H = PKM(m, w2_slot(26)); m.pco2L = PKM(m, w2_slot(27));
}

template <int B>
__device__ __forceinline__ void load_state(const HxBuffers &buf, int mem, Member<B> &m) {
  m.cHL = lds_(buf, HXS_C_HL, mem); m.cLL = lds_(buf, HXS_C_LL, mem);
  m.cIO = lds_(buf, HXS_C_IO, mem); m.cDO = lds_(buf, HXS_C_DO, mem);
  m.atmos = lds_(buf, HXS_ATMOS, mem); m.earth = lds_(buf, HXS_EARTH, mem);
  m.cum_luc_va = lds_(buf, HXS_CUM_LUC_VA, mem);
  m.cum_pf_ch4 = lds_(buf, HXS_CUM_PF_CH4, mem);
  m.masstot = lds_(buf, HXS_MASSTOT, mem);
  m.max_ts = lds_(buf, HXS_MAX_TS, mem);
  m.ts_timeout = (int)lds_(buf, HXS_TS_TIMEOUT, mem);
  m.lastflux_ann = lds_(buf, HXS_LASTFLUX_ANN, mem);
  m.sdt = lds_(buf, HXS_SOLVER_DT, mem);
  if constexpr (!hx_w2<B>()) { m.alkH = lds_(buf, HXS_ALK_HL, mem); m.alkL = lds_(buf, HXS_ALK_LL, mem); }
  m.hH = lds_(buf, HXS_H_HL, mem); m.hL = lds_(buf, HXS_H_LL, mem);
#pragma unroll hx_ur<B>()
  for (int b = 0; b < nbio<B>(m); ++b) {
    const int r = HXS_NGLOBAL + b * HXSB_N;
    m.veg[b] = lds_(buf, r + HXSB_VEG, mem); m.det[b] = lds_(buf, r + HXSB_DET, mem);
    m.soil[b] = lds_(buf, r + HXSB_SOIL, mem); m.pf[b] = lds_(buf, r + HXSB_PF, mem);
    m.thawed[b] = lds_(buf, r + HXSB_THAWED, mem);
    m.tempferts[b] = lds_(buf, r + HXSB_TEMPFERTS, mem);
  }
  m.status = HX_GU(buf.status)[mem];
}

template <int B>
__device__ __forceinline__ void store_state(const HxBuffers &buf_, int mem,
                                            const Member<B> &m, double *base = nullptr) {
  HxBuffers buf = buf_;
  if (base) buf.state = base;
  sts_(buf, HXS_C_HL, mem, m.cHL); sts_(buf, HXS_C_LL, mem, m.cLL);
  sts_(buf, HXS_C_IO, mem, m.cIO); sts_(buf, HXS_C_DO, mem, m.cDO);
  sts_(buf, HXS_ATMOS, mem, m.atmos); sts_(buf, HXS_EARTH, mem, m.earth);
  sts_(buf, HXS_CUM_LUC_VA, mem, m.cum_luc_va);
  sts_(buf, HXS_CUM_PF_CH4, mem, m.cum_pf_ch4);
  sts_(buf, HXS_MASSTOT, mem, m.masstot);
  sts_(buf, HXS_MAX_TS, mem, m.max_ts);
  sts_(buf, HXS_TS_TIMEOUT, mem, (double)m.ts_timeout);
  sts_(buf, HXS_LASTFLUX_ANN, mem, m.lastflux_ann);
  sts_(buf, HXS_SOLVER_DT, mem, m.sdt);
  if constexpr (hx_w2<B>()) {
    if (base) {
      sts_(buf, HXS_ALK_HL, mem, lds_(buf_, HXS_ALK_HL, mem));
      sts_(buf, HXS_ALK_LL, mem, lds_(buf_, HXS_ALK_LL, mem));
    }
  } else {
  sts_(buf, HXS_ALK_HL, mem, m.alkH); sts_(buf, HXS_ALK_LL, mem, m.alkL);
  }
  sts_(buf, HXS_H_HL, mem, m.hH); sts_(buf, HXS_H_LL, mem, m.hL);
#pragma unroll hx_ur<B>()
  for (int b = 0; b < nbio<B>(m); ++b) {
    const int r = HXS_NGLOBAL + b * HXSB_N;
    sts_(buf, r + HXSB_VEG, mem, m.veg[b]); sts_(buf, r + HXSB_DET, mem, m.det[b]);
    sts_(buf, r + HXSB_SOIL, mem, m.soil[b]); sts_(buf, r + HXSB_PF, mem, m.pf[b]);
    sts_(buf, r + HXSB_THAWED, mem, m.thawed[b]);
    sts_(buf, r + HXSB_TEMPFERTS, mem, m.tempferts[b]);
  }
  if (!base) HX_GU(buf.status)[mem] = m.status;
}

template <int B>
__device__ __forceinline__ void store_park_state(const HxBuffers &buf_, int mem,
                                                 const Member<B> &m, double *base = nullptr) {
  HxBuffers buf = buf_;
  if (base) buf.state = base;
  sts_(buf, HXS_CH4, mem, PKM(m, PK_CH4)); sts_(buf, HXS_SST, mem, PKM(m, PK_SST));
  sts_(buf, HXS_TLAND, mem, PKM(m, PK_TLAND)); sts_(buf, HXS_TWIN, mem, PKM(m, PK_TWIN));
  sts_(buf, HXS_TL_M1, mem, PKM(m, PK_TL_M1)); sts_(buf, HXS_TL_M2, mem, PKM(m, PK_TL_M2));
  sts_(buf, HXS_F_PREV, mem, PKM(m, PK_F_PREV));
  sts_(buf, HXS_BASE_TOT, mem, PKM(m, PK_BASE_TOT));
  sts_(buf, HXS_BASE_CO2, mem, PKM(m, PK_BASE_CO2));
  if constexpr (hx_w2<B>()) {
    if (base) sts_(buf, HXS_EOS_VEGC, mem, lds_(buf_, HXS_EOS_VEGC, mem));
  } else {
  if (base) sts_(buf, HXS_EOS_VEGC, mem, PKM(m, PK_EOS));
  }
  if (hx_slim_park<B>() && !base) return;
#pragma unroll hx_ur<B>()
  for (int b = 0; b < nbio<B>(m); ++b)
    sts_(buf, HXS_NGLOBAL + b * HXSB_N + HXSB_F_FROZEN, mem, ffrozen_of<B>(m, b));
}

}
```

hector_amd/csrc/hx_dev_pair.h:

```cpp
#pragma once

namespace {

enum PairStep {
  PS_N0 = 0, PS_X3, PS_N4, PS_D4, PS_X0, PS_X4,
  PS_NL, PS_DL,
  PS_N
};
enum PairYear {
  PY_PN = 0, PY_CH4, PY_O3, PY_STATUS1, PY_PCO2L,
  PY_S3C, PY_DTOT, PY_SOIL, PY_TOT0,
  PY_MAXTS, PY_STATUS0, PY_TLAND, PY_LNC, PY_CLL,
  PY_KL_K1, PY_KL_K2, PY_KL_KB, PY_KL_KW, PY_KL_KH,
  PY_HSTAT,
  PY_HL, PY_HLO,
  PY_N
};

struct PairCtl {
  double t, dtl, t_target, t_start, sdt, ode_start, max_ts;
  int retry, fails, nsteps;
  bool first_call, stepping, alive;
};

// ... 175 lines not shown
__device__ __forceinline__ bool pair_control(PairCtl &c, double err, unsigned &status) {
#pragma clang fp contract(off)
  constexpr double EPS = 2.220446049250313e-16;
  if (__builtin_expect(err > 1.0, 0)) {
    c.dtl *= fmax(0.9 * pow_m13(err), 0.2);
    if (++c.fails > 500) { status |= HX_ERR_STEPFAIL; c.alive = false; c.stepping = false; }
    return false;
  }
  c.t += c.dtl;
  const double grow = 0.9 * pow_m15(fmax(0.00032, err));
  if (err < 0.5) c.dtl *= grow;
  c.fails = 0;
  c.nsteps++;
  if (!((c.t_target - c.t) > EPS)) c.stepping = false;
  if (c.nsteps > HX_MAX_STEPS_PER_YEAR) { status |= HX_ERR_STEPFAIL; c.alive = false; c.stepping = false; }
  return true;
}

__device__ __forceinline__ bool pair_clip_need(PairCtl &c) {
#pragma clang fp contract(off)
  constexpr double EPS = 2.220446049250313e-16;
  if (c.stepping && ((c.t + c.dtl) - c.t_target) > EPS) c.dtl = c.t_target - c.t;
  return c.stepping && ((c.t + c.dtl) - c.ode_start) > c.max_ts;
}

__device__ __forceinline__ bool pair_retry(PairCtl &c, unsigned &status) {
#pragma clang fp contract(off)
  constexpr double EPS = 2.220446049250313e-16;
  if (((c.t + c.dtl) - c.t_target) > EPS) c.dtl = c.t_target - c.t;
  bool reload = false;
  while (c.stepping && ((c.t + c.dtl) - c.ode_start) > c.max_ts) {
    ++c.retry;
    c.t_target = c.t_start + (c.t_target - c.t_start) / 2.0;
    c.t = c.t_start;
    c.sdt = c.t_target - c.t;
    c.dtl = c.sdt;
    reload = true;
    c.fails = 0;
    if (c.retry >= 8) { status |= HX_ERR_RETRIES; c.alive = false; c.stepping = false; }
  }
  if (reload) c.first_call = true;
  return reload;
}

#ifdef HX_PHASE_CLOCK
__device__ __forceinline__ void hx_pstamp(long long *clkp, int k) {
  volatile long long *clk = clkp;
  asm volatile("" ::: "memory");
  const long long now = (long long)__builtin_readcyclecounter();
  clk[k] += now - clk[23];
  clk[23] = now;
  asm volatile("" ::: "memory");
}
#define PSTAMP(k) hx_pstamp(s_pclk[role], (k))
#ifdef HX_PHASE_CLOCK_FINE
#define PSTAMPF(k) PSTAMP(k)
#else
#define PSTAMPF(k)
#endif
#else
#define PSTAMP(k)
#define PSTAMPF(k)
#endif

}

template <bool KERPM, bool HF, bool CONS = false, int NB = 1>
#ifdef HX_PAIR_TWO_PER_SIMD
#define HX_PAIR_OCC __attribute__((amdgpu_waves_per_eu(2, 2)))
#else
#define HX_PAIR_OCC
#endif
__global__ __launch_bounds__(128) HX_PAIR_OCC void hx_pair_kernel(const HxArgs *__restrict__ args, int iy_from,
                                                      int iy_to) {
  __shared__ double s_tblk[HX_DBLK + 1][64];
  __shared__ double s_st[2][PS_N][64];
  __shared__ double s_yr[PY_N][64];
  const int lane = threadIdx.x & 63, role = threadIdx.x >> 6;
  const int mem = blockIdx.x * 64 + lane;
  const HxBuffers &buf = args->buf;
  const HxConst &kc = args->kc;
  const size_t np = (size_t)buf.npad;
  hx_wave_stamp(buf, 2 * blockIdx.x + role, 0, lane);
  unsigned status = HX_GU(buf.status)[mem];
  PairCtl c;
  c.sdt = lds_(buf, HXS_SOLVER_DT, mem);
  c.max_ts = lds_(buf, HXS_MAX_TS, mem);
  c.alive = status == 0;
  c.nsteps = 0;
  int par = 0;
  int blk0 = -1;
  const double eps_abs = kc.eps_abs, eps_rel = kc.eps_rel;
#ifdef HX_PHASE_CLOCK
  __shared__ long long s_pclk[2][24];
  if (lane == 0) { for (int k = 0; k < 23; ++k) s_pclk[role][k] = 0; s_pclk[role][23] = (long long)__builtin_readcyclecounter(); }
#endif

  if (role == 0) {
    double cHL = lds_(buf, HXS_C_HL, mem), cLL = lds_(buf, HXS_C_LL, mem),
           cIO = lds_(buf, HXS_C_IO, mem), cDO = lds_(buf, HXS_C_DO, mem);
    double atmos = lds_(buf, HXS_ATMOS, mem);
    const double alkH = lds_(buf, HXS_ALK_HL, mem), alkL = lds_(buf, HXS_ALK_LL, mem);
    double hH = lds_(buf, HXS_H_HL, mem);
    int ts_timeout = (int)lds_(buf, HXS_TS_TIMEOUT, mem);
    double lastflux_ann = lds_(buf, HXS_LASTFLUX_ANN, mem);
    double tland = lds_(buf, HXS_TLAND, mem), sst = lds_(buf, HXS_SST, mem),
           f_prev = lds_(buf, HXS_F_PREV, mem), base_tot = lds_(buf, HXS_BASE_TOT, mem),
           base_co2 = lds_(buf, HXS_BASE_CO2, mem);
    const double C0 = ldp(buf, HXP_C0, mem), p_aero = ldp(buf, HXP_AERO, mem),
                 p_vol = ldp(buf, HXP_VOL, mem);
    const double kLH = ldd(buf, HXD_KLH, mem), kLI = ldd(buf, HXD_KLI, mem),
                 kHD = ldd(buf, HXD_KHD, mem), kIL = ldd(buf, HXD_KIL, mem),
                 kIH = ldd(buf, HXD_KIH, mem), kID = ldd(buf, HXD_KID, mem),
                 kDI = ldd(buf, HXD_KDI, mem);
    const double dA0 = ldd(buf, HXD_A0, mem), dA1 = ldd(buf, HXD_A1, mem), dA2 = ldd(buf, HXD_A2, mem),
                 dA3 = ldd(buf, HXD_A3, mem), dIB0 = ldd(buf, HXD_IB0, mem), dIB1 = ldd(buf, HXD_IB1, mem),
                 dIB2 = ldd(buf, HXD_IB2, mem), dIB3 = ldd(buf, HXD_IB3, mem), dQC1 = ldd(buf, HXD_QC1, mem),
                 dQC2 = ldd(buf, HXD_QC2, mem), dDQ1 = ldd(buf, HXD_DQ1, mem), dDQ2 = ldd(buf, HXD_DQ2, mem),
                 dDPS = ldd(buf, HXD_DPSCALE, mem);
    auto ldk = [&](int idx) -> double {
      if constexpr (KERPM) return HX_GCD(buf.ker)[(size_t)idx * np + mem];
      else return HX_CCD(buf.ker)[idx];
    };
    const double ker_lag1 = ldk(kc.ns - 2 + HX_KPAD);
    const double ker2_lag1 = HF ? ldk(kc.ns - 1 + HX_KPAD) : 0.0;
    const double dHFS = HF ? ldd(buf, HXD_HFSCALE, mem) : 0.0;
    ChemK kH, kL;
    double pco2H = 0, pco2L = 0;
    s_tblk[0][lane] = sst;
    auto store_ocean = [&](double *base) {
      HxBuffers b2 = buf;
      if (base) b2.state = base;
      sts_(b2, HXS_C_HL, mem, cHL); sts_(b2, HXS_C_LL, mem, cLL);
      sts_(b2, HXS_C_IO, mem, cIO); sts_(b2, HXS_C_DO, mem, cDO);
      sts_(b2, HXS_ATMOS, mem, atmos);
      sts_(b2, HXS_MAX_TS, mem, c.max_ts); sts_(b2, HXS_TS_TIMEOUT, mem, (double)ts_timeout);
      sts_(b2, HXS_LASTFLUX_ANN, mem, lastflux_ann); sts_(b2, HXS_SOLVER_DT, mem, c.sdt);
      sts_(b2, HXS_H_HL, mem, hH);
      sts_(b2, HXS_TLAND, mem, tland); sts_(b2, HXS_SST, mem, sst);
      sts_(b2, HXS_F_PREV, mem, f_prev); sts_(b2, HXS_BASE_TOT, mem, base_tot);
      sts_(b2, HXS_BASE_CO2, mem, base_co2);
      if (base) sts_(b2, HXS_ALK_HL, mem, alkH);
    };
    double dpart_pf = 0, dpast_in = 0;
    [[maybe_unused]] double dpart2_pf = 0, hint_in = 0;
    bool sums_done = true;
    auto history_sums = [&](int iy) {
      const int jb = iy - blk0;
      double acc = dpart_pf;
      [[maybe_unused]] double acc2 = dpart2_pf;
      const int kq = kc.ns - iy - 1 + HX_KPAD + (blk0 - 1);
      const int nchunk = (jb + 7) >> 3;
      for (int cc = 0; cc < nchunk; ++cc) {
        double T[8], K[8];
#pragma unroll
        for (int q = 0; q < 8; ++q) { T[q] = s_tblk[8 * cc + q][lane]; K[q] = ldk(kq + 8 * cc + q); }
#pragma unroll
        for (int q = 0; q < 8; ++q) acc += ((8 * cc + q < jb) ? T[q] : 0.0) * K[q];
        if constexpr (HF) {
#pragma unroll
          for (int q = 0; q < 8; ++q) K[q] = ldk(kq + 8 * cc + q + 1);
#pragma unroll
          for (int q = 0; q < 8; ++q) acc2 += ((8 * cc + q < jb) ? T[q] : 0.0) * K[q];
        }
      }
      dpast_in = acc;
      if constexpr (HF) hint_in = acc2;
      sums_done = true;
    };

    auto year_consts = [&](double sst_v) {
      const double TcH = sst_v + 18 + (-16.4), TcL = sst_v + 18 + 2.9;
      double ex[12];
#ifndef HX_NO_CHEM_FIT
      const bool fit_in = chem_fit_applies(TcH, TcL);
      chem_constants_fit(TcH, TcL, kc.kfit, ex);
      if (__builtin_expect(__any(!fit_in), 0))
#endif
      {
        double lg[2] = {TcH + 273.15, TcL + 273.15}, e12[12];
        hx_log_batch<2>(lg);
        chem_exponents(TcH, lg[0], &e12[0]);
        chem_exponents(TcL, lg[1], &e12[6]);
        hx_exp_chunks<12>(e12);
#pragma unroll
        for (int i = 0; i < 12; ++i) {
#ifndef HX_NO_CHEM_FIT
          ex[i] = fit_in ? ex[i] : e12[i];
#else
          ex[i] = e12[i];
#endif
// ... 179 lines not shown
        const double sqM = hx_sqrt(ch4), sqC = hx_sqrt(co2c);
        const double C_alpha_max = C0 - (b1 / (2 * a1));
        double alpha_prime;
        if (co2c > C_alpha_max) alpha_prime = d1 - ((b1 * b1) / (4 * a1));
        else if (C0 < co2c && co2c < C_alpha_max)
          alpha_prime = d1 + a1 * ((co2c - C0) * (co2c - C0)) + b1 * (co2c - C0);
        else alpha_prime = d1;
        const double sarf_co2 = (alpha_prime + c1 * sqN) * ln_co2r;
        const double fco2 = (sarf_co2 * kc.delta_co2) + sarf_co2;
        const double sarf_n2o = (a2 * sqC + b2 * sqN + c2 * sqM + d2) * (sqN - sqN0);
        const double fn2o = (kc.delta_n2o * sarf_n2o) + sarf_n2o;
        const double sarf_ch4 = (a3 * sqM + b3 * sqN + d3) * (sqM - kc.sqrtM0);
        const double fch4 = (kc.delta_ch4 * sarf_ch4) + sarf_ch4;
        const double fh2o = 0.0485 * ((ch4 - kc.M0f) * kc.inv_h2o_span);
        const double fo3 = kc.o3_rf * o3;
        double ftot = ((((((fco2 + fn2o) + fch4) + fh2o) + fo3) + rf_other) +
                       p_aero * sh[HXSH_RF_AERO]) + p_vol * sh[HXSH_RF_VOL];
        if constexpr (CONS) {
          const double cf = sh[HXSH_FTOT_CON];
          if ((kc.con_mask & HXC_FTOT) && !isnan(cf)) ftot = cf;
        }
        if (iy == kc.baseyear_idx) { base_tot = ftot; base_co2 = fco2; }
        else { rf_tot = ftot - base_tot; rf_co2 = fco2 - base_co2; }
      }
      const double dpast = (dpast_in + sst * ker_lag1) * dDPS;
      const double DelQ = rf_tot - f_prev;
      const double DQ1 = dDQ1 * (rf_tot + f_prev) + DelQ * dQC1;
      const double DQ2 = dDQ2 * (rf_tot + f_prev) + DelQ * dQC2;
      const double X1 = DQ1 + (dA0 * tland + dA1 * sst);
      const double X2 = (DQ2 + dpast) + (dA2 * tland + dA3 * sst);
      double tl_new = dIB0 * X1 + dIB1 * X2;
      double sst_new = dIB2 * X1 + dIB3 * X2;
      double tgav = D_flnd * tl_new + (1.0 - D_flnd) * D_bsi * sst_new;
      if constexpr (CONS) {
        const double ct = sh[HXSH_TAS_CON];
        if ((kc.con_mask & HXC_TAS) && !isnan(ct)) {
          tgav = ct;
          tl_new = (tgav - (1.0 - D_flnd) * D_bsi * sst_new) / D_flnd;
          sst_new = (tgav - D_flnd * tl_new) / ((1.0 - D_flnd) * D_bsi);
        }
      }
      s_tblk[slot][lane] = sst_new;
      if (slot == HX_DBLK) s_tblk[0][lane] = sst_new;
      s_yr[PY_TLAND][lane] = tl_new;
      s_yr[PY_LNC][lane] = ln_co2r;
      const size_t o = (size_t)iy * np + mem;
      if constexpr (HF) {
        const double hint = hint_in + sst * ker2_lag1;
        const double hmix = D_cas * (sst_new - sst);
        const double hi = dHFS * (2.0 * sst_new - hint);
        sto_(buf, HXO_HEATFLUX, o, hmix + D_fso * hi);
      }
      f_prev = rf_tot; tland = tl_new; sst = sst_new;
      sto_(buf, HXO_SST, o, sst_new);
      sto_(buf, HXO_TLAND, o, tl_new);
      if (buf.out[HXO_CO2]) sto_(buf, HXO_CO2, o, co2c);
      if (buf.out[HXO_TGAV]) sto_(buf, HXO_TGAV, o, tgav);
      if (buf.out[HXO_RF_TOT]) sto_(buf, HXO_RF_TOT, o, rf_tot);
      if (buf.out[HXO_RF_CO2]) sto_(buf, HXO_RF_CO2, o, rf_co2);
      if (__builtin_expect(!!(buf.out_rare), 0)) {
        if (buf.out[HXO_ATMOS_C]) sto_(buf, HXO_ATMOS_C, o, atmos);
        if (buf.out[HXO_OCEAN_C]) sto_(buf, HXO_OCEAN_C, o, cDO + cIO + cLL + cHL);
        if (buf.out[HXO_OCEAN_UPTAKE]) sto_(buf, HXO_OCEAN_UPTAKE, o, annualflux_sum);
        if (buf.out[HXO_HL_PH]) sto_(buf, HXO_HL_PH, o, -log10(hH));
        if (buf.out[HXO_CH4]) sto_(buf, HXO_CH4, o, ch4);
        if (buf.out[HXO_O3]) sto_(buf, HXO_O3, o, o3);
        if (buf.out[HXO_GMST]) sto_(buf, HXO_GMST, o, D_flnd * tl_new + (1.0 - D_flnd) * sst_new);
      }
      if (__builtin_expect(!!(buf.hist), 0)) {
        store_ocean(buf.hist + (size_t)iy * (size_t)HX_NSTATE(NB) * np);
        s_yr[PY_HSTAT][lane] = (double)status;
      }
      if (iy < iy_to) year_consts(sst);
      PSTAMP(10);
      __syncthreads();
      PSTAMP(11);
    }
    store_ocean(nullptr);
  } else {
    double veg[NB], det[NB], soil[NB], pf[NB], thawed[NB], tempferts[NB], ffrozen[NB];
#pragma unroll
    for (int b = 0; b < NB; ++b) {
      const int rs = HXS_NGLOBAL + b * HXSB_N;
      veg[b] = lds_(buf, rs + HXSB_VEG, mem); det[b] = lds_(buf, rs + HXSB_DET, mem);
      soil[b] = lds_(buf, rs + HXSB_SOIL, mem); pf[b] = lds_(buf, rs + HXSB_PF, mem);
      thawed[b] = lds_(buf, rs + HXSB_THAWED, mem); tempferts[b] = lds_(buf, rs + HXSB_TEMPFERTS, mem);
      ffrozen[b] = lds_(buf, rs + HXSB_F_FROZEN, mem);
    }
    double earth = lds_(buf, HXS_EARTH, mem), cum_luc_va = lds_(buf, HXS_CUM_LUC_VA, mem),
           cum_pf_ch4 = lds_(buf, HXS_CUM_PF_CH4, mem), masstot = lds_(buf, HXS_MASSTOT, mem);
    const double eos = lds_(buf, HXS_EOS_VEGC, mem);
    double ch4 = lds_(buf, HXS_CH4, mem), ln_ch4 = hx_log(ch4), o3 = 0;
    double twin = lds_(buf, HXS_TWIN, mem), tl_m1 = lds_(buf, HXS_TL_M1, mem),
           tl_m2 = lds_(buf, HXS_TL_M2, mem);
    double tland = lds_(buf, HXS_TLAND, mem);
    double lnc = hx_log(hx_div(lds_(buf, HXS_ATMOS, mem) * PGC2PPM, ldp(buf, HXP_C0, mem)));
    double cLL = lds_(buf, HXS_C_LL, mem), hL = lds_(buf, HXS_H_LL, mem);
    const double alkL = lds_(buf, HXS_ALK_LL, mem);
    double npp0[NB], f_nppv[NB], f_nppd[NB], f_litterd[NB], rh_ch4_frac[NB], fpf_static[NB], beta[NB], wf[NB],
        lnq10[NB], pmu[NB], psigma[NB];
#pragma unroll
    for (int b = 0; b < NB; ++b) {
      const int r = HXP_NGLOBAL + b * HXPB_N;
      npp0[b] = ldp(buf, r + HXPB_NPP0, mem); f_nppv[b] = ldp(buf, r + HXPB_F_NPPV, mem);
      f_nppd[b] = ldp(buf, r + HXPB_F_NPPD, mem); f_litterd[b] = ldp(buf, r + HXPB_F_LITTERD, mem);
      rh_ch4_frac[b] = ldp(buf, r + HXPB_RH_CH4_FRAC, mem); fpf_static[b] = ldp(buf, r + HXPB_FPF_STATIC, mem);
      beta[b] = ldp(buf, r + HXPB_BETA, mem); wf[b] = ldp(buf, r + HXPB_WF, mem);
      lnq10[b] = ldd(buf, HXD_NGLOBAL + b, mem);
      pmu[b] = ldp(buf, r + HXPB_PF_MU, mem); psigma[b] = ldp(buf, r + HXPB_PF_SIGMA, mem);
    }
    auto rh_tp_co2 = [&](int b) { return ((thawed[b] * (1 - fpf_static[b])) * 0.02) * tempferts[b] * (1.0 - rh_ch4_frac[b]); };
    auto rh_tp_ch4 = [&](int b) { return ((thawed[b] * (1 - fpf_static[b])) * 0.02) * tempferts[b] * rh_ch4_frac[b]; };
    auto rh_ch4_total = [&]() { double x = 0;
#pragma unroll
      for (int b = 0; b < NB; ++b) x += rh_tp_ch4(b);
      return x; };
    ChemK kL;
    kL.Tr = 0; kL.g = 0;
    double pco2L = 0;
    double tfs_cand[NB], tl_old_pf = 0;
#pragma unroll
    for (int b = 0; b < NB; ++b) tfs_cand[b] = 0;
    auto store_land = [&](double *base) {
      HxBuffers b2 = buf;
      if (base) b2.state = base;
#pragma unroll
      for (int b = 0; b < NB; ++b) {
        const int rr = HXS_NGLOBAL + b * HXSB_N;
        sts_(b2, rr + HXSB_VEG, mem, veg[b]); sts_(b2, rr + HXSB_DET, mem, det[b]);
        sts_(b2, rr + HXSB_SOIL, mem, soil[b]); sts_(b2, rr + HXSB_PF, mem, pf[b]);
        sts_(b2, rr + HXSB_THAWED, mem, thawed[b]); sts_(b2, rr + HXSB_TEMPFERTS, mem, tempferts[b]);
        sts_(b2, rr + HXSB_F_FROZEN, mem, ffrozen[b]);
      }
      sts_(b2, HXS_EARTH, mem, earth); sts_(b2, HXS_CUM_LUC_VA, mem, cum_luc_va);
      sts_(b2, HXS_CUM_PF_CH4, mem, cum_pf_ch4); sts_(b2, HXS_MASSTOT, mem, masstot);
      sts_(b2, HXS_CH4, mem, ch4); sts_(b2, HXS_TWIN, mem, twin);
      sts_(b2, HXS_TL_M1, mem, tl_m1); sts_(b2, HXS_TL_M2, mem, tl_m2);
      sts_(b2, HXS_H_LL, mem, hL);
      if (base) { sts_(b2, HXS_ALK_LL, mem, alkL); sts_(b2, HXS_EOS_VEGC, mem, eos); }
    };
    auto prefetch = [&](int iyn) {
      const int iold = iyn - 203;
      tl_old_pf = HX_GCD(buf.out[HXO_TLAND])[(size_t)(iold >= 1 ? iold : 0) * np + mem];
    };
    auto prepare = [&](int iyn) {
      hx_ccd shn = HX_CCD(buf.shared) + (size_t)iyn * HXSH_STRIDE;
      const int iold = iyn - 203;
      const double prev_ch4 = ch4;
      const double rh_ch4 = (iyn > 1) ? rh_ch4_total() : 0.0;
      double toh = 0.0;
      if (prev_ch4 != kc.M0)
        toh = ((kc.CCH4 * (ln_ch4 - kc.lnM0) + shn[HXSH_OH_B]) + shn[HXSH_OH_C]) + shn[HXSH_OH_D];
      if (iyn >= 3) {
        twin += tl_m2;
        if (iold >= 1) twin -= tl_old_pf;
      }
      double ex[1 + NB];
      ex[0] = -toh;
#pragma unroll
      for (int b = 0; b < NB; ++b) {
        const double Trm = (iyn > 1) ? (twin * wf[b]) * 0.005 : 0.0;
        ex[1 + b] = lnq10[b] * (Trm * 0.1);
      }
      hx_exp_batch<1 + NB>(ex);
#pragma unroll
      for (int b = 0; b < NB; ++b) tfs_cand[b] = ex[1 + b];
      const double tau_oh = kc.TOH0 * ex[0];
      const double emisTocon = ((shn[HXSH_CH4_EM] + rh_ch4 * PG_C_TO_TG_CH4) + shn[HXSH_CH4N]) * kc.inv_UC_CH4;
      const double dCH4 = ((emisTocon - prev_ch4 * kc.inv_Tsoil) - prev_ch4 * kc.inv_Tstrat) -
                          hx_div(prev_ch4, tau_oh);
      ch4 = prev_ch4 + dCH4;
      if constexpr (CONS) {
        const double cm = shn[HXSH_CH4_CON];
        if ((kc.con_mask & HXC_CH4) && !isnan(cm)) ch4 = cm;
      }
      ln_ch4 = hx_log(ch4);
      o3 = ((5 * ln_ch4 + shn[HXSH_O3_NOX]) + shn[HXSH_O3_CO]) + shn[HXSH_O3_NMVOC];
      if (blk0 < 0 || iyn >= blk0 + HX_DBLK) {
        blk0 = iyn;
        if constexpr (KERPM)
          doeclim_pass_dev<true, HF>(buf.out[HXO_SST], buf.ker, const_cast<double *>(buf.dpart),
// ... 300 lines not shown
```

hector_amd/csrc/hx_fleet.cpp:

```cpp
#include "hx_fleet.hpp"

#include <algorithm>
#include <cmath>
#include <cstdlib>
#include <cstring>
#include <exception>
#include <stdexcept>
#include <thread>

#ifndef HX_HOST_EMULATION
#include <dlfcn.h>
#include <rccl/rccl.h>
#endif

hipError_t hx_launch_combine_stats(const double *slots, int world, int rows, double *out,
                                   hipStream_t st);

namespace hx {

namespace {

void hip_ck(hipError_t e, const char *what) {
  if (e != hipSuccess)
    throw std::runtime_error(std::string("HIP error in ") + what + ": " + hipGetErrorString(e));
// ... 907 lines not shown
  if (n_procs < 1 || proc_rank < 0 || proc_rank >= n_procs || !id_bytes)
    throw std::runtime_error("hx_comm_init_rank: bad arguments");
  if (duplicates_) {
    if (n_procs != 1)
      throw std::runtime_error("hx_comm_init_rank: a rehearsal core (duplicate devices) cannot join "
                               "other processes");
    world_ = n_shards(); first_rank_ = 0; comm_ready_ = true;
    return;
  }
#ifndef HX_HOST_EMULATION
  Rccl &r = rccl();
  ncclUniqueId id;
  std::memcpy(id.internal, id_bytes, sizeof(id.internal));
  const int L = n_shards();
  world_ = n_procs * L;
  first_rank_ = proc_rank * L;
  std::vector<ncclComm_t> comms((size_t)L, nullptr);
  try {
    {
      RcclGroup group(r, L > 1);
      for (int s = 0; s < L; ++s) {
        hip_ck(hipSetDevice(shards_[(size_t)s].device), "hipSetDevice");
        nccl_ck(r.CommInitRank(&comms[(size_t)s], world_, id, first_rank_ + s), "ncclCommInitRank");
      }
      group.end();
    }
    for (int s = 0; s < L; ++s)
      if (!comms[(size_t)s]) throw std::runtime_error("ncclCommInitRank returned no communicator");
    for (int s = 0; s < L; ++s) shards_[(size_t)s].comm = comms[(size_t)s];
    free_stats_buffers();
  } catch (...) {
    for (int s = 0; s < L; ++s)
      if (comms[(size_t)s]) { (void)hipSetDevice(shards_[(size_t)s].device); (void)r.CommAbort(comms[(size_t)s]); }
    for (Shard &s : shards_) s.comm = nullptr;
    world_ = 1; first_rank_ = 0;
    throw;
  }
  comm_ready_ = true;
#else
  throw std::runtime_error("the host-emulation build has no RCCL");
#endif
}

void Fleet::ensure_comm() {
  if (comm_ready_ || shards_.size() == 1) return;
  if (duplicates_) { world_ = n_shards(); first_rank_ = 0; comm_ready_ = true; return; }
  char id[128];
  unique_id(id);
  comm_init_rank(1, 0, id);
}

void Fleet::free_stats_buffers() {
  for (Shard &s : shards_) {
    if (!s.d_local && !s.d_slots && !s.d_result) continue;
    (void)hipSetDevice(s.device);
    if (s.d_local) (void)hipFree(s.d_local);
    if (s.d_slots) (void)hipFree(s.d_slots);
    if (s.d_result) (void)hipFree(s.d_result);
    s.d_local = s.d_slots = s.d_result = nullptr;
  }
  stats_cap_ = 0;
}

void Fleet::ensure_stats_buffers(size_t blk) {
  if (blk <= stats_cap_) return;
  free_stats_buffers();
  for (Shard &s : shards_) {
    use(s);
    hip_ck(hipMalloc(&s.d_local, sizeof(double) * blk), "hipMalloc stats block");
    hip_ck(hipMalloc(&s.d_slots, sizeof(double) * blk * (size_t)world_), "hipMalloc stats slots");
    hip_ck(hipMalloc(&s.d_result, sizeof(double) * blk), "hipMalloc stats result");
  }
  stats_cap_ = blk;
}

void Fleet::ensemble_stats(const std::vector<std::string> &caps, int year0, int year1,
                           double *out_host, double *d_out) {
  if (caps.empty()) throw std::runtime_error("ensemble_stats: no variables");
  const int ny = year1 - year0 + 1;
  if (ny < 1) throw std::runtime_error("ensemble_stats: year1 < year0");
  ensure_comm();
  const int world = comm_ready_ ? world_ : 1;
  const size_t nv = caps.size(), rows = nv * (size_t)ny, blk = rows * 5;
  ensure_stats_buffers(blk);
  for (Shard &s : shards_) {
    use(s);
    for (size_t v = 0; v < nv; ++v)
      s.core->stats_async(caps[v], year0, year1, s.d_local + v * (size_t)ny * 5);
  }
  if (world == 1) {
    Shard &s = shards_[0];
    hip_ck(hipMemcpyAsync(s.d_slots, s.d_local, sizeof(double) * blk, hipMemcpyDeviceToDevice,
                          s.core->stream()), "stats copy");
  } else if (duplicates_) {
    for (Shard &s : shards_) { use(s); hip_ck(hipStreamSynchronize(s.core->stream()), "stats sync"); }
    for (Shard &dst : shards_) {
      use(dst);
      for (size_t r = 0; r < shards_.size(); ++r)
        hip_ck(hipMemcpyAsync(dst.d_slots + r * blk, shards_[r].d_local, sizeof(double) * blk,
                              hipMemcpyDeviceToDevice, dst.core->stream()), "stats exchange");
    }
  } else {
#ifndef HX_HOST_EMULATION
    Rccl &r = rccl();
    RcclGroup group(r, shards_.size() > 1);
    for (Shard &s : shards_) {
      use(s);
      nccl_ck(r.AllGather(s.d_local, s.d_slots, blk, ncclDouble, (ncclComm_t)s.comm, s.core->stream()),
              "ncclAllGather");
    }
    group.end();
#endif
  }
  for (Shard &s : shards_) {
    use(s);
    hip_ck(hx_launch_combine_stats(s.d_slots, world, (int)rows, s.d_result, s.core->stream()),
           "combine statistics");
  }
  Shard &s0 = shards_[0];
  use(s0);
  if (d_out)
    hip_ck(hipMemcpyAsync(d_out, s0.d_result, sizeof(double) * blk, hipMemcpyDeviceToDevice,
                          s0.core->stream()), "stats result");
  if (out_host)
    hip_ck(hipMemcpyAsync(out_host, s0.d_result, sizeof(double) * blk, hipMemcpyDeviceToHost,
                          s0.core->stream()), "stats result to host");
  for (Shard &s : shards_) { use(s); hip_ck(hipStreamSynchronize(s.core->stream()), "stats sync"); }
}

}
```

hector_amd/csrc/hx_kernels.hip:

```cpp
#include <hip/hip_runtime.h>
#include <cstdlib>
#include <math.h>
#include <stdint.h>

#include <hx_addrspace.h>

#include "hx_layout.h"

#define HX_DBLK 32
#define HX_KPAD 32

#ifndef HX_HOST_EMULATION
#define HX_WAVES_PER_SIMD(B) __attribute__((amdgpu_waves_per_eu(hx_w2<B>() ? 2 : 1, hx_w2<B>() ? 2 : 8)))
#else
#define HX_WAVES_PER_SIMD(B)
#endif

#if !defined(HX_NO_CHEM_FIT) && !defined(HX_FIT_IN_PHASE_A)
#define HX_FIT_CARRIED 1
#endif

#include "hx_dev_const.h"
#include "hx_dev_clock.h"
#include "hx_dev_math.h"
// ... 353 lines not shown
  double v1 = 0;
#pragma unroll hx_ur<B>()
  for (int b = 0; b < nbio<B>(m); ++b) {
    v1 += m.veg[b];
    sts_(buf, HXS_NGLOBAL + b * HXSB_N + HXSB_F_FROZEN, mem, 1.0);
  }
  sts_(buf, HXS_EOS_VEGC, mem, v1);
  sts_(buf, HXS_CH4, mem, kc.M0f);
  sts_(buf, HXS_TLAND, mem, 0.0); sts_(buf, HXS_SST, mem, 0.0);
  sts_(buf, HXS_F_PREV, mem, 0.0); sts_(buf, HXS_BASE_TOT, mem, 0.0);
  sts_(buf, HXS_BASE_CO2, mem, 0.0);
  sts_(buf, HXS_TL_M1, mem, 0.0); sts_(buf, HXS_TL_M2, mem, 0.0);
  sts_(buf, HXS_TWIN, mem, 0.0);
  const size_t o = (size_t)mem;
  auto put = [&](int var, double v) { if (buf.out[var]) sto_(buf, var, o, v); };
  put(HXO_SST, 0.0); put(HXO_TLAND, 0.0);
  put(HXO_CO2, m.atmos * PGC2PPM); put(HXO_TGAV, 0.0);
  put(HXO_RF_TOT, 0.0); put(HXO_RF_CO2, 0.0);
  put(HXO_OCEAN_C, m.cDO + m.cIO + m.cLL + m.cHL);
  put(HXO_HL_PH, 0.0); put(HXO_LL_PH, 0.0); put(HXO_ATMOS_C, m.atmos);
  {
    double v = 0, d = 0, s = 0, p = 0, th = 0;
#pragma unroll hx_ur<B>()
    for (int b = 0; b < nbio<B>(m); ++b) { v += m.veg[b]; d += m.det[b]; s += m.soil[b];
                                   p += m.pf[b]; th += m.thawed[b]; }
    put(HXO_PERMAFROST_C, p); put(HXO_VEG_C, v); put(HXO_DET_C, d);
    put(HXO_SOIL_C, s); put(HXO_THAWED_C, th);
  }
  put(HXO_HEATFLUX, 0.0); put(HXO_CH4, kc.M0f); put(HXO_O3, 0.0);
  put(HXO_EARTH_C, m.earth); put(HXO_NBP, 0.0); put(HXO_OCEAN_UPTAKE, 0.0);
  put(HXO_NSTASH, 0.0); put(HXO_NSTEPS, 0.0);
  put(HXO_C_HL, m.cHL); put(HXO_C_LL, m.cLL); put(HXO_C_IO, m.cIO); put(HXO_C_DO, m.cDO);
  put(HXO_F_FROZEN, 1.0); put(HXO_TAU_OH, kc.TOH0);
#pragma unroll hx_ur<B>()
  for (int b = 0; b < nbio<B>(m); ++b) {
    put(HXO_B(HXOB_VEG, b), m.veg[b]); put(HXO_B(HXOB_DET, b), m.det[b]);
    put(HXO_B(HXOB_SOIL, b), m.soil[b]); put(HXO_B(HXOB_PF, b), m.pf[b]);
    put(HXO_B(HXOB_THAWED, b), m.thawed[b]); put(HXO_B(HXOB_F_FROZEN, b), 1.0);
    put(HXO_B(HXOB_TEMPFERTD, b), 1.0); put(HXO_B(HXOB_TEMPFERTS, b), 1.0);
  }
  if (spinup_steps) spinup_steps[mem] = steps;
}

#ifdef HX_ROWIO_ALL
template <int B> constexpr bool hx_rowio() { return true; }
#else
template <int B> constexpr bool hx_rowio() { return hx_tbl<B>(); }
#endif
template <int B, bool HF, bool KERPM, int CON>
__global__ __launch_bounds__(CON == 3 ? 64 * (1 + trk_waves<(B < 1 || B > 4 ? 1 : B)>()) : 64) HX_WAVES_PER_SIMD(B)
void hx_run_kernel(const HxArgs *__restrict__ args, int iy_from, int iy_to) {
  static_assert(CON != 3 || (B >= 1 && B <= 4), "tracking companions: the unrolled kernels");
  static_assert(!hx_w2<B>() || CON <= 1, "two-wavefront flavour: the plain and the extended kernel");
  __shared__ double s_tblk[B == 1 ? HX_DBLK : 1][64];
  const int lane = threadIdx.x & 63;
  const int mem = blockIdx.x * 64 + lane;
  if (mem >= args->buf.npad) return;
  [[maybe_unused]] double (*s_trk_rec)[64] = nullptr;
  [[maybe_unused]] int *s_trk_cmd = nullptr;
  if constexpr (CON == 3) {
    __shared__ double s_rec[2 * trkr_n(B)][64];
    __shared__ int s_cmd[5];
    s_trk_rec = s_rec; s_trk_cmd = s_cmd;
    if (threadIdx.x >= 64) {
      if (threadIdx.x < 128) {
        s_rec[TRKR_ACTIVE][lane] = 0.0; s_rec[trkr_n(B) + TRKR_ACTIVE][lane] = 0.0;
        s_cmd[4] = 0;
      }
      __syncthreads();
      track_companion<B>(args, iy_from, lane, ((int)(threadIdx.x >> 6) - 1) * trk_nc<B>(), s_trk_rec, s_trk_cmd);
      return;
    }
    __syncthreads();
  }
  __shared__ double s_park_fixed[B == HX_DYN ? 1 : hx_npark<B>()][64];
  double (*s_park)[64] = (B == HX_DYN) ? hx_dyn_park : s_park_fixed;
  Member<B> m;
  hx_wave_stamp(args->buf, blockIdx.x, 0, lane);
  bind_member<B>(args->buf, mem, m, s_park, lane);
#ifdef HX_PHASE_CLOCK
  for (int k = 0; k < HX_NCLK; ++k) hx_s_clk[k] = 0;
  hx_s_clk[HX_NCLK] = (long long)__builtin_readcyclecounter();
#endif
  load_state<B>(args->buf, mem, m);
  {
    const HxBuffers &buf = args->buf;
    PKM(m, PK_CH4) = lds_(buf, HXS_CH4, mem); PKM(m, PK_SST) = lds_(buf, HXS_SST, mem);
    if constexpr (!hx_w2<B>()) PKM(m, PK_EOS) = lds_(buf, HXS_EOS_VEGC, mem);
    PKM(m, PK_TLAND) = lds_(buf, HXS_TLAND, mem);
    PKM(m, PK_TWIN) = lds_(buf, HXS_TWIN, mem); PKM(m, PK_TL_M1) = lds_(buf, HXS_TL_M1, mem);
    PKM(m, PK_TL_M2) = lds_(buf, HXS_TL_M2, mem); PKM(m, PK_F_PREV) = lds_(buf, HXS_F_PREV, mem);
    PKM(m, PK_BASE_TOT) = lds_(buf, HXS_BASE_TOT, mem);
    PKM(m, PK_BASE_CO2) = lds_(buf, HXS_BASE_CO2, mem);
    PKM(m, PK_LN_CH4) = hx_log(lds_(buf, HXS_CH4, mem));
    PKM(m, PK_LN_CO2R) = hx_log(hx_div(m.atmos * PGC2PPM, m.C0));
    if constexpr (!hx_slim_park<B>()) {
#pragma unroll hx_ur<B>()
    for (int b = 0; b < nbio<B>(m); ++b)
      PKM(m, pk_ff0<B>() + b) = lds_(buf, HXS_NGLOBAL + b * HXSB_N + HXSB_F_FROZEN, mem);
    }
  }
  constexpr bool want_hf = HF;
  int blk0 = -1;
#ifdef HX_BLOCK_STAGGER
  const int blk_len0 = 1 + (int)((blockIdx.x * 13u) & (HX_DBLK - 1));
#else
  const int blk_len0 = HX_DBLK;
#endif
  int blk_end = 0;
  double pf_tl_old = 0.0, pf_dpart = 0.0;
  constexpr bool KPF = KERPM && !hx_w2<B>() && hx_nbc<B>() >= 1 && hx_nbc<B>() <= 4;
  [[maybe_unused]] double kpf[KPF ? HX_DBLK + 1 : 1];
  if constexpr (KPF) {
#pragma unroll
    for (int r = 0; r <= HX_DBLK; ++r) kpf[r] = 0.0;
  }
  if constexpr (!hx_w2<B>()) {
    const int iold0 = iy_from + 1 - 203;
    pf_tl_old = HX_GCD(args->buf.out[HXO_TLAND])[(size_t)(iold0 >= 1 ? iold0 : 0) * args->buf.npad + mem];
  }
  double ya[12], yc4[4];
  auto load_year_a = [&](int iyn) {
    hx_ccd shn = HX_CCD(args->buf.shared) + (size_t)(iyn < args->kc.ns ? iyn : args->kc.ns - 1) * HXSH_STRIDE;
    ya[0] = shn[HXSH_OH_B]; ya[1] = shn[HXSH_OH_C]; ya[2] = shn[HXSH_OH_D]; ya[3] = shn[HXSH_CH4_EM];
    ya[4] = shn[HXSH_CH4N]; ya[5] = shn[HXSH_O3_NOX]; ya[6] = shn[HXSH_O3_CO]; ya[7] = shn[HXSH_O3_NMVOC];
    ya[8] = shn[HXSH_FFI]; ya[9] = shn[HXSH_DACCS]; ya[10] = shn[HXSH_LUC_E]; ya[11] = shn[HXSH_LUC_U];
  };
#ifndef HX_YA_PREFETCH
  constexpr bool YAL = true;
#else
  constexpr bool YAL = hx_w2<B>();
#endif
  if constexpr (!YAL) load_year_a(iy_from + 1);
#ifndef HX_W2_NO_KEEP
  constexpr bool W2K = hx_w2<B>();
#else
  constexpr bool W2K = false;
#endif
  [[maybe_unused]] double w2k_eos = 0, w2k_alkH = 0, w2k_alkL = 0, w2k_lnq = 0;
  if constexpr (W2K) {
    const HxBuffers &buf = args->buf;
    HX_W2_LOCAL(m);
    w2k_eos = w2_ld<true>(buf.state, m.npad, HXS_EOS_VEGC, m.moff);
    w2k_alkH = w2_ld<true>(buf.state, m.npad, HXS_ALK_HL, m.moff);
    w2k_alkL = w2_ld<true>(buf.state, m.npad, HXS_ALK_LL, m.moff);
    w2k_lnq = w2_ld<true>(buf.derived, m.npad, HXD_NGLOBAL, m.moff);
    const int iold0 = iy_from + 1 - 203;
    pf_tl_old = hx_ldm<true>(HX_GCD(buf.out[HXO_TLAND]) + (size_t)(iold0 >= 1 ? iold0 : 0) * buf.npad, m.moff);
  }
  if constexpr (CON >= 2) m.trk_iy = args->kc.trk_iy;
  if constexpr (CON == 3) { m.trk_rec = s_trk_rec; m.trk_cmd = s_trk_cmd; }
  int cost_steps = 0, cost_stash = 0;
#ifdef HX_FIT_CARRIED
  constexpr bool FITC = !hx_cons<CON>() || (!hx_w2<B>() && (CON == 1 || CON == -1));
  [[maybe_unused]] double fitc[12];
  if constexpr (FITC) {
    const double s0 = PKM(m, PK_SST);
    chem_constants_fit(s0 + 18 + (-16.4), s0 + 18 + 2.9, args->kc.kfit, fitc);
  }
#endif

#ifndef HX_NO_CWF
  constexpr bool CWF = !hx_w2<B>() && !hx_tbl<B>() && hx_nbc<B>() >= 2 && hx_nbc<B>() <= 4;
#else
  constexpr bool CWF = false;
#endif
  [[maybe_unused]] double c_wf[CWF ? hx_nbc<B>() : 1], c_lnq[CWF ? hx_nbc<B>() : 1];
  if constexpr (CWF) {
#pragma unroll
    for (int b = 0; b < hx_nbc<B>(); ++b) {
      c_wf[b] = ldp(args->buf, HXP_NGLOBAL + b * HXPB_N + HXPB_WF, mem);
      c_lnq[b] = ldd(args->buf, HXD_NGLOBAL + b, mem);
    }
  }
  [[maybe_unused]] unsigned cmk = 0, msk = 0;
  [[maybe_unused]] unsigned long long omk = 0;
  if constexpr (CON) {
    cmk = (unsigned)args->kc.con_mask; msk = args->buf.ms_mask; omk = args->buf.out_mask0;
    m.omk = omk;
  }
#ifndef HX_HOST_EMULATION
#define HX_MASKS_LOCAL() do { if constexpr (CON) asm volatile("" : "+s"(cmk), "+s"(msk), "+s"(omk)); } while (0)
// ... 779 lines not shown
      HX_STAMP(m, 14);
      if (HX_RARE(buf.hist)) {
        double *slab = buf.hist + (size_t)iy * (size_t)HX_NSTATE(nbio<B>(m)) * buf.npad;
        store_state<B>(buf, mem, m, slab);
        store_park_state<B>(buf, mem, m, slab);
        HX_GU(buf.hist_status)[(size_t)iy * buf.npad + mem] = m.status;
      }
    }
  }
  HX_FENCE();
  if constexpr (CON == 3) track_post(s_trk_cmd, TRKC_DONE, 0);
  store_state<B>(args->buf, mem, m);
  store_park_state<B>(args->buf, mem, m);
  if (args->buf.cost) HX_GD(args->buf.cost)[mem] += (double)(4 * cost_steps + 5 * cost_stash);
  hx_wave_stamp(args->buf, blockIdx.x, 1, lane);
#ifdef HX_PHASE_CLOCK
  if (args->buf.out[HXO_TGAV])
    for (int k = 0; k < HX_NCLK; ++k)
      HX_GD(args->buf.out[HXO_TGAV])[(size_t)k * args->buf.npad + mem] = (double)hx_s_clk[k];
#endif
}

__global__ void hx_broadcast_rows_kernel(double *table, int nrows, int npad) {
  const int mem = blockIdx.x * blockDim.x + threadIdx.x;
  if (mem >= npad || mem == 0) return;
  for (int r = 0; r < nrows; ++r) table[(size_t)r * npad + mem] = table[(size_t)r * npad];
}
__global__ void hx_broadcast_u32_kernel(unsigned *v, int npad) {
  const int mem = blockIdx.x * blockDim.x + threadIdx.x;
  if (mem >= npad || mem == 0) return;
  v[mem] = v[0];
}
__global__ void hx_or_flags_kernel(unsigned *status, const double *flag_row, int npad) {
  const int mem = blockIdx.x * blockDim.x + threadIdx.x;
  if (mem >= npad) return;
  status[mem] |= (unsigned)flag_row[mem];
}

__global__ __launch_bounds__(64) void hx_gas_kernel(const double *par, const double *ser,
                                                    const double *h0, int nh, int ns, int npad,
                                                    double *n2o_out, double *rf_other_out) {
  const int mem = blockIdx.x * blockDim.x + threadIdx.x;
  if (mem >= npad) return;
  const size_t np = (size_t)npad;
  const double N0 = par[mem], TN2O0 = par[np + mem], UC = par[2 * np + mem];
  const double *em = ser, *ncon = ser + ns, *alb = ser + 2 * (size_t)ns, *misc = ser + 3 * (size_t)ns;
  constexpr int MAXH = 40;
  double conc[MAXH], expfac[MAXH];
  for (int h = 0; h < nh && h < MAXH; ++h) {
    conc[h] = h0[h];
    expfac[h] = exp(-(1 / par[(size_t)(3 + 3 * h) * np + mem]));
  }
  const double N0f = isnan(ncon[0]) ? N0 : ncon[0];
  double n2o = N0f;
  n2o_out[mem] = n2o;
  rf_other_out[mem] = (0.0 + alb[0]) + misc[0];
  for (int iy = 1; iy < ns; ++iy) {
    const double tau_n = TN2O0 * pow(n2o / N0f, -0.05);
    n2o = n2o + (em[iy] / UC - n2o / tau_n);
    if (!isnan(ncon[iy])) n2o = ncon[iy];
    double rf_h = 0.0;
    for (int h = 0; h < nh && h < MAXH; ++h) {
      const double tau = par[(size_t)(3 + 3 * h) * np + mem], rho = par[(size_t)(4 + 3 * h) * np + mem],
                   delta = par[(size_t)(5 + 3 * h) * np + mem];
      const double dconc = ser[(size_t)(4 + 2 * h) * ns + iy], hc = ser[(size_t)(5 + 2 * h) * ns + iy];
      conc[h] = conc[h] * expfac[h] + dconc * tau * (1.0 - expfac[h]);
      if (!isnan(hc)) conc[h] = hc;
      const double rf_un = rho * conc[h];
      rf_h = rf_h + (rf_un + delta * rf_un);
    }
    n2o_out[(size_t)iy * np + mem] = n2o;
    rf_other_out[(size_t)iy * np + mem] = (rf_h + alb[iy]) + misc[iy];
  }
}

__global__ __launch_bounds__(256) void hx_gather_kernel(const double *src, const int *lane_of_member,
                                                        double *dst, int n, int npad, int nyears) {
  const int mem = blockIdx.x * blockDim.x + threadIdx.x;
  const int y = blockIdx.y;
  if (mem >= n || y >= nyears) return;
  dst[(size_t)y * n + mem] = src[(size_t)y * npad + lane_of_member[mem]];
}

__global__ __launch_bounds__(256) void hx_stats_kernel(const double *var, int n, int npad,
                                                       int iy0, double *stats) {
  const int iy = iy0 + blockIdx.x;
  const double *row = var + (size_t)iy * npad;
  double sa[4] = {0, 0, 0, 0}, qa[4] = {0, 0, 0, 0};
  double mn = INFINITY, mx = -INFINITY;
  const int n2 = n >> 1;
  const double2 *row2 = reinterpret_cast<const double2 *>(row);
  int i = threadIdx.x;
  for (; i + 3 * (int)blockDim.x < n2; i += 4 * blockDim.x) {
    double2 v[4];
#pragma unroll
    for (int k = 0; k < 4; ++k) v[k] = row2[i + k * (int)blockDim.x];
#pragma unroll
    for (int k = 0; k < 4; ++k) {
      sa[k] += v[k].x + v[k].y;
      qa[k] += v[k].x * v[k].x + v[k].y * v[k].y;
      mn = fmin(mn, fmin(v[k].x, v[k].y));
      mx = fmax(mx, fmax(v[k].x, v[k].y));
    }
  }
  for (; i < n2; i += blockDim.x) {
    const double2 v = row2[i];
    sa[0] += v.x + v.y; qa[0] += v.x * v.x + v.y * v.y;
    mn = fmin(mn, fmin(v.x, v.y)); mx = fmax(mx, fmax(v.x, v.y));
  }
  if ((n & 1) && threadIdx.x == 0) {
    const double v = row[n - 1];
    sa[0] += v; qa[0] += v * v; mn = fmin(mn, v); mx = fmax(mx, v);
  }
  double s = (sa[0] + sa[1]) + (sa[2] + sa[3]), s2 = (qa[0] + qa[1]) + (qa[2] + qa[3]);
  double cnt = (threadIdx.x == 0) ? (double)n : 0.0;
#pragma unroll
  for (int off = 32; off > 0; off >>= 1) {
    s += __shfl_down(s, off, 64); s2 += __shfl_down(s2, off, 64);
    cnt += __shfl_down(cnt, off, 64);
    mn = fmin(mn, __shfl_down(mn, off, 64)); mx = fmax(mx, __shfl_down(mx, off, 64));
  }
  __shared__ double red[4][5];
  const int w = threadIdx.x >> 6;
  if ((threadIdx.x & 63) == 0) { red[w][0] = cnt; red[w][1] = s; red[w][2] = s2;
                                 red[w][3] = mn; red[w][4] = mx; }
  __syncthreads();
  if (threadIdx.x == 0) {
    for (int k = 1; k < 4; ++k) { red[0][0] += red[k][0]; red[0][1] += red[k][1];
      red[0][2] += red[k][2]; red[0][3] = fmin(red[0][3], red[k][3]);
      red[0][4] = fmax(red[0][4], red[k][4]); }
    double *o = stats + (size_t)blockIdx.x * 5;
    o[0] = red[0][0]; o[1] = red[0][1]; o[2] = red[0][2]; o[3] = red[0][3]; o[4] = red[0][4];
  }
}

__global__ __launch_bounds__(256) void hx_combine_stats_kernel(const double *slots, int world,
                                                               int rows, double *out) {
  const int r = blockIdx.x * blockDim.x + threadIdx.x;
  if (r >= rows) return;
  const double *p = slots + (size_t)r * 5;
  double cnt = p[0], s = p[1], s2 = p[2], mn = p[3], mx = p[4];
  for (int k = 1; k < world; ++k) {
    p += (size_t)rows * 5;
    cnt += p[0]; s += p[1]; s2 += p[2]; mn = fmin(mn, p[3]); mx = fmax(mx, p[4]);
  }
  double *o = out + (size_t)r * 5;
  o[0] = cnt; o[1] = s; o[2] = s2; o[3] = mn; o[4] = mx;
}

__global__ __launch_bounds__(256) void hx_doeclim_table_kernel(const double *diff_row,
                                                               double *ker, int ns, int count,
                                                               int stride) {
  const int mem = blockIdx.x * blockDim.x + threadIdx.x;
  const int i = blockIdx.y;
  if (mem >= count || i >= ns) return;
  const double keff = (D_secs / 10000) * diff_row[mem];
  const double tb = (D_zbot * D_zbot) / keff;
  const double sq2 = sqrt(2.0), sqpt = sqrt(M_PI * tb);
  double KT0, KTA1, KTB1, KTA2, KTB2, KTA3, KTB3;
  if (i == ns - 1) {
    KT0 = 4.0 - 2.0 * sq2;
    KTA1 = -8.0 * exp(-tb) + 4.0 * sq2 * exp(-0.5 * tb);
    KTB1 = 4.0 * sqpt * (1.0 + erf(sqrt(0.5 * tb)) - 2.0 * erf(sqrt(tb)));
    KTA2 = 8.0 * exp(-4.0 * tb) - 4.0 * sq2 * exp(-2.0 * tb);
    KTB2 = -8.0 * sqpt * (1.0 + erf(sqrt(2.0 * tb)) - 2.0 * erf(2.0 * sqrt(tb)));
    KTA3 = -8.0 * exp(-9.0 * tb) + 4.0 * sq2 * exp(-4.5 * tb);
    KTB3 = 12.0 * sqpt * (1.0 + erf(sqrt(4.5 * tb)) - 2.0 * erf(3.0 * sqrt(tb)));
  } else {
    const double a = (double)(ns - i), b = (double)(ns + 1 - i), c = (double)(ns - 1 - i);
    const double ra = sqrt(a), rb = sqrt(b), rc = sqrt(c);
    const double ua = sqrt(tb / a), ub = sqrt(tb / b), uc = sqrt(tb / c);
    KT0 = 4.0 * ra - 2.0 * rb - 2.0 * rc;
    KTA1 = -8.0 * ra * exp(-tb / a) + 4.0 * rb * exp(-tb / b) + 4.0 * rc * exp(-tb / c);
    KTB1 = 4.0 * sqpt * (erf(uc) + erf(ub) - 2.0 * erf(ua));
    KTA2 = 8.0 * ra * exp(-4.0 * tb / a) - 4.0 * rb * exp(-4.0 * tb / b) -
           4.0 * rc * exp(-4.0 * tb / c);
    KTB2 = -8.0 * sqpt * (erf(2.0 * uc) + erf(2.0 * ub) - 2.0 * erf(2.0 * ua));
    KTA3 = -8.0 * ra * exp(-9.0 * tb / a) + 4.0 * rb * exp(-9.0 * tb / b) +
           4.0 * rc * exp(-9.0 * tb / c);
    KTB3 = 12.0 * sqpt * (erf(3.0 * uc) + erf(3.0 * ub) - 2.0 * erf(3.0 * ua));
  }
  ker[(size_t)(i + HX_KPAD) * stride + mem] = KT0 + KTA1 + KTB1 + KTA2 + KTB2 + KTA3 + KTB3;
}

__global__ __launch_bounds__(64) void hx_alk_kernel(const HxArgs *__restrict__ args, int nmem) {
#ifndef HX_HOST_EMULATION
  __builtin_amdgcn_s_setprio(3);
#endif
  const int mem = blockIdx.x * 64 + threadIdx.x;
  if (mem >= nmem) return;
  const HxBuffers &buf = args->buf;
  const double cHL = lds_(buf, HXS_C_HL, mem), cLL = lds_(buf, HXS_C_LL, mem);
  const double co2 = lds_(buf, HXS_ATMOS, mem) * PGC2PPM;
  const double sst = lds_(buf, HXS_SST, mem);
  unsigned status = HX_GU(buf.status)[mem];
  ChemK kH, kL;
  chem_constants2(sst + 18 + (-16.4), sst + 18 + 2.9, kH, kL);
  double hH = 0, hL = 0;
  const double alkH = equilibrate_alk(kH, cHL, 1.0 / O_vHL, O_AsHL, co2, 1.000, hH, status);
  const double alkL = equilibrate_alk(kL, cLL, 1.0 / O_vLL, O_AsLL, co2, -1.000, hL, status);
  sts_(buf, HXS_ALK_HL, mem, alkH); sts_(buf, HXS_ALK_LL, mem, alkL);
  sts_(buf, HXS_H_HL, mem, hH); sts_(buf, HXS_H_LL, mem, hL);
  HX_GU(buf.status)[mem] = status;
}

__device__ __forceinline__ double diag_rf(int kind, const HxDiagArgs &a, int iy, int mem) {
  hx_ccd sh = HX_CCD(a.shared) + (size_t)iy * HXSH_STRIDE;
  const size_t o = (size_t)iy * a.npad + mem;
  const double a2 = -3.4197e-4, b2 = 2.5455e-4, c2 = -2.4357e-4, d2 = 0.12173;
  const double a3 = -8.9603e-5, b3 = -1.2462e-4, d3 = 0.045194;
  double sqN = sh[HXSH_SQRT_N2O], sqN0 = a.sqrtN0;
  if (a.n2o_members) { sqN = sqrt(a.n2o_members[o]); sqN0 = sqrt(a.n2o_members[mem]); }
  if (kind == HXG_RF_O3) return 0.042 * a.o3[o];
  const double ch4 = a.ch4[o], sqM = sqrt(ch4);
// ... 419 lines not shown
                     inv_vol, out);
  return hipGetLastError();
}
__global__ __launch_bounds__(64) void hx_prewarm_kernel(const int *stop, long long max_ticks, double *sink,
                                                         const double *mem, unsigned long long n_mem) {
#ifndef HX_HOST_EMULATION
  const long long t0 = (long long)__builtin_amdgcn_s_memrealtime();
  double a = 1.0 + 1e-9 * threadIdx.x, b = 0.999999, c = 1e-7, d = a, e = a + c, f = a - c, acc = 0.0;
  unsigned long long pos = (unsigned long long)blockIdx.x * 64 + threadIdx.x;
  const unsigned long long stride = (unsigned long long)gridDim.x * 64;
  for (;;) {
#pragma unroll
    for (int k = 0; k < 32; ++k) { a = fma(a, b, c); d = fma(d, b, c); e = fma(e, b, c); f = fma(f, b, c); }
    if (n_mem) {
#pragma unroll
      for (int k = 0; k < 4; ++k) { acc += __builtin_nontemporal_load(mem + pos % n_mem); pos += stride; }
    }
    if (__builtin_nontemporal_load(stop) != 0) break;
    if ((long long)__builtin_amdgcn_s_memrealtime() - t0 > max_ticks) break;
  }
  if (((a + d) + (e + f)) + acc == 12345.678) sink[blockIdx.x & 1023] = a;
#endif
}
hipError_t hx_launch_prewarm(const int *d_stop, long long max_ticks, double *d_sink, int waves,
                             const double *mem, unsigned long long n_mem, hipStream_t st) {
  hipLaunchKernelGGL(hx_prewarm_kernel, dim3(waves), dim3(64), 0, st, d_stop, max_ticks, d_sink, mem, n_mem);
  return hipGetLastError();
}
hipError_t hx_launch_diag(int kind, const HxDiagArgs &a, double *out, hipStream_t st) {
  hipLaunchKernelGGL(hx_diag_kernel, dim3((a.npad + 255) / 256, a.ny), dim3(256), 0, st, kind, a, out);
  return hipGetLastError();
}
hipError_t hx_launch_slr(const double *tgav, int npad, int start_year, int iy_to, double *out,
                         size_t var_stride, hipStream_t st) {
  hipLaunchKernelGGL(hx_slr_kernel, dim3((npad + 63) / 64), dim3(64), 0, st, tgav, npad,
                     start_year, iy_to, out, var_stride);
  return hipGetLastError();
}
hipError_t hx_launch_broadcast(double *table, int nrows, int npad, hipStream_t st) {
  hipLaunchKernelGGL(hx_broadcast_rows_kernel, dim3((npad + 255) / 256), dim3(256), 0, st,
                     table, nrows, npad);
  return hipGetLastError();
}
hipError_t hx_launch_broadcast_u32(unsigned *v, int npad, hipStream_t st) {
  hipLaunchKernelGGL(hx_broadcast_u32_kernel, dim3((npad + 255) / 256), dim3(256), 0, st, v, npad);
  return hipGetLastError();
}
hipError_t hx_launch_gas(const double *par, const double *ser, const double *h0, int nh, int ns,
                         int npad, double *n2o_out, double *rf_other_out, hipStream_t st) {
  if (nh > 40) return hipErrorInvalidValue;
  hipLaunchKernelGGL(hx_gas_kernel, dim3((npad + 63) / 64), dim3(64), 0, st, par, ser, h0, nh, ns,
                     npad, n2o_out, rf_other_out);
  return hipGetLastError();
}
hipError_t hx_launch_or_flags(unsigned *status, const double *flag_row, int npad, hipStream_t st) {
  hipLaunchKernelGGL(hx_or_flags_kernel, dim3((npad + 255) / 256), dim3(256), 0, st, status,
                     flag_row, npad);
  return hipGetLastError();
}
hipError_t hx_launch_doeclim_kernel(const double *diff_row, double *ker, int ns, int count,
                                    int stride, hipStream_t st) {
  hipLaunchKernelGGL(hx_doeclim_table_kernel, dim3((count + 255) / 256, ns), dim3(256), 0, st,
                     diff_row, ker, ns, count, stride);
  return hipGetLastError();
}
hipError_t hx_launch_derive(const double *params, double *derived, const double *ker,
                            int ker_per_member, int ns, int nbiome, int npad, hipStream_t st) {
  hipLaunchKernelGGL(hx_derive_kernel, dim3((npad + 255) / 256), dim3(256), 0, st, params,
                     derived, ker, ker_per_member, ns, nbiome, npad);
  return hipGetLastError();
}
hipError_t hx_launch_gather(const double *src, const int *lane_of_member, double *dst, int n,
                            int npad, int nyears, hipStream_t st) {
  hipLaunchKernelGGL(hx_gather_kernel, dim3((n + 255) / 256, nyears), dim3(256), 0, st, src,
                     lane_of_member, dst, n, npad, nyears);
  return hipGetLastError();
}
hipError_t hx_launch_combine_stats(const double *slots, int world, int rows, double *out,
                                   hipStream_t st) {
  hipLaunchKernelGGL(hx_combine_stats_kernel, dim3((rows + 255) / 256), dim3(256), 0, st, slots,
                     world, rows, out);
  return hipGetLastError();
}
hipError_t hx_launch_stats(const double *var, int n, int npad, int iy0, int nyears,
                           double *stats, hipStream_t st) {
  hipLaunchKernelGGL(hx_stats_kernel, dim3(nyears), dim3(256), 0, st, var, n, npad, iy0, stats);
  return hipGetLastError();
}
}
```

hector_amd/csrc/hx_layout.h:

```cpp
#pragma once
#include <stdint.h>

#define HX_MAXB 4
#define HX_BDYN 32
#define HX_WAVE 64

enum HxParamRow {
  HXP_S = 0,
  HXP_DIFF,
  HXP_QCO2,
  HXP_AERO,
  HXP_VOL,
  HXP_C0,
  HXP_TT, HXP_TU, HXP_TWI, HXP_TID,
  HXP_PRE_SURF, HXP_PRE_ID,
  HXP_LO_RATIO,
  HXP_NGLOBAL
};
enum HxBiomeParam {
  HXPB_BETA = 0, HXPB_Q10, HXPB_WF, HXPB_NPP0,
  HXPB_VEG0, HXPB_DET0, HXPB_SOIL0, HXPB_PF0,
  HXPB_F_NPPV, HXPB_F_NPPD, HXPB_F_LITTERD,
  HXPB_RH_CH4_FRAC, HXPB_PF_MU, HXPB_PF_SIGMA, HXPB_FPF_STATIC,
  HXPB_N
// ... 89 lines not shown
#define HXC_TAS 4
#define HXC_FTOT 8
#define HXC_CH4 16
#define HXC_LO 32

struct HxConst {
  int start_year, ns, baseyear_idx, max_spinup, spinup_chem;
  double eps_abs, eps_rel, dt0, eps_spinup;
  double M0, lnM0, Tsoil, Tstrat, UC_CH4, TOH0, CCH4;
  double M0f, sqrtM0;
  double inv_UC_CH4, inv_Tsoil, inv_Tstrat, inv_h2o_span;
  int con_mask;
  int trk_iy;
  double N0, sqrtN0;
  double delta_co2, delta_ch4, delta_n2o;
  double o3_rf;
  double tab[32];
  double mtab[32];
  double ctab[40];
  double kfit[14 * 12];
};
#include "hx_chem_fit.inc"
static_assert(HX_CHEM_FIT_DEGREE == 13, "HxConst::kfit is sized for degree 13");
inline void hx_fill_chem_fit(double *t) {
  for (int i = 0; i < (HX_CHEM_FIT_DEGREE + 1) * 12; ++i) t[i] = hx_chem_fit_table[i];
}
inline void hx_fill_math_table(double *t) {
  const double v[26] = {1.6059043836821613e-10, 2.0876756987868099e-09, 2.5052108385441719e-08,
                        2.7557319223985893e-07, 2.7557319223985888e-06, 2.4801587301587302e-05,
                        1.9841269841269841e-04, 1.3888888888888889e-03, 8.3333333333333332e-03,
                        4.1666666666666664e-02, 1.6666666666666666e-01, 0.5,
                        1.4426950408889634074, -6.93147180369123816490e-01, -1.90821492927058770002e-10, 0.0,
                        6.666666666666735130e-01, 3.999999999940941908e-01, 2.857142874366239149e-01,
                        2.222219843214978396e-01, 1.818357216161805012e-01, 1.531383769920937332e-01,
                        1.479819860511658591e-01, 6.93147180369123816490e-01, 1.90821492927058770002e-10,
                        0.70710678118654752440};
  for (int i = 0; i < 26; ++i) t[i] = v[i];
  for (int i = 26; i < 32; ++i) t[i] = 0.0;
}
inline void hx_fill_tableau(double *t) {
  const double c1 = 35.0 / 384, c3 = 500.0 / 1113, c4 = 125.0 / 192, c5 = -2187.0 / 6784, c6 = 11.0 / 84;
  const double v[30] = {1.0 / 5, 1.0 / 5,
                        3.0 / 40, 9.0 / 40, 3.0 / 10,
                        44.0 / 45, -56.0 / 15, 32.0 / 9, 4.0 / 5,
                        19372.0 / 6561, -25360.0 / 2187, 64448.0 / 6561, -212.0 / 729, 8.0 / 9,
                        9017.0 / 3168, -355.0 / 33, 46732.0 / 5247, 49.0 / 176, -5103.0 / 18656,
                        c1, c3, c4, c5, c6,
                        c1 - 5179.0 / 57600, c3 - 7571.0 / 16695, c4 - 393.0 / 640,
                        c5 - (-92097.0 / 339200), c6 - 187.0 / 2100, -1.0 / 40};
  for (int i = 0; i < 30; ++i) t[i] = v[i];
  t[30] = t[31] = 0.0;
}

struct HxBuffers {
  const double *params;
  double *state;
  unsigned *status;
  const double *derived;
  const double *shared;
  const double *ker;
  const double *dpart;
  const double *dpart2;
  double *hist;
  unsigned *hist_status;
  int n, npad, ker_per_member;
  int nbiome;
  const double *mseries[HXM_N];
  const double *uparams;
  int uni_landk, uni_bio;
  const double *uderived;
  int uni_k, uni_avc, uni_wf;
  double *track_out_f;
  double *track_out_v;
  int trk_slots;
  int out_rare;
  int biome_diag;
  int stash_diag;
  unsigned long long out_mask0;
  unsigned ms_mask;
  double *cost;
  double *spin_rec;
  double *bscratch;
  long long *wave_clk;
  double *out[HXO_NVAR];
};
enum { HXSR_NBP = 0, HXSR_NPP, HXSR_RH, HXSR_RH_DET, HXSR_RH_SOIL, HXSR_ATMOS_C, HXSR_CA_RESIDUAL,
       HXSR_VEG_C, HXSR_DET_C, HXSR_SOIL_C, HXSR_PERMAFROST_C, HXSR_THAWED_C, HXSR_EARTH_C,
       HXSR_HL_UPTAKE, HXSR_LL_UPTAKE, HXSR_C_DO, HXSR_C_HL, HXSR_C_IO, HXSR_C_LL, HXSR_HL_DO,
       HXSR_OCEAN_UPTAKE, HXSR_N };

enum HxDiagKind {
  HXG_TEMP = 0, HXG_DIC, HXG_CO3, HXG_OMEGA_AR, HXG_OMEGA_CA, HXG_REVELLE, HXG_OCEAN_TAS,
  HXG_RF_N2O, HXG_RF_CH4, HXG_RF_H2O, HXG_RF_O3
};

struct HxDiagArgs {
  const double *sst, *ph, *pco2, *carbon;
  const double *co2, *ch4, *o3, *tgav;
  const double *lo_ratio;
  const double *shared;
  const double *n2o_members;
  double deltaT, inv_vol;
  double sqrtN0, sqrtM0, M0f, delta_n2o, delta_ch4;
  int base_idx, npad, iy0, ny;
};


struct HxArgs {
  HxConst kc;
  HxBuffers buf;
};
```

Baseline: 6.329 billion.

## Read reset snapshot directly in run kernels and batch stats launches

Reset to year zero no longer copies the snapshot state and status back into the working buffers on the device. Instead the run kernels read their initial state through new state_in/status_in pointers that can point at the snapshot, and they zero the lane cost themselves, which also removes a memset and a host sync. The stats kernel now handles several variables per launch through a 2-D grid, and the single-shard fleet path issues one batched call. The cost is extra argument-patching uploads with a host sync, plus lazy materialization logic that has to stay correct for state queries and partial resets.

```diff
diff --git a/hector_amd/csrc/ensemble_core.cpp b/hector_amd/csrc/ensemble_core.cpp
--- a/hector_amd/csrc/ensemble_core.cpp
+++ b/hector_amd/csrc/ensemble_core.cpp
@@ -39,7 +39,7 @@
                          size_t var_stride, hipStream_t st);
 hipError_t hx_launch_gather(const double *src, const int *lane_of_member, double *dst, int n,
                             int npad, int nyears, hipStream_t st);
-hipError_t hx_launch_stats(const double *var, int n, int npad, int iy0, int nyears,
+hipError_t hx_launch_stats(const double *const *vars, int nvars, int n, int npad, int iy0, int nyears,
                            double *stats, hipStream_t st);
 hipError_t hx_launch_derive(const double *params, double *derived, const double *ker,
                             int ker_per_member, int ns, int nbiome, int npad, hipStream_t st);
@@ -215,6 +215,7 @@
   for (const DerivedDef &d : kDerived) if (name == d.name) return &d;
   return nullptr;
 }
+const char *const *combo_of(const std::string &name);
 
 }
 
@@ -714,6 +715,8 @@
   b.spin_rec = d_spin_rec_;
   b.bscratch = d_bscratch_;
   b.wave_clk = d_wave_clk_;
+  b.state_in = d_state_ ? d_state_ + (size_t)npad_ * HX_NSTATE(B_) : nullptr;
+  b.status_in = d_status_ ? d_status_ + (size_t)npad_ : nullptr;
   return b;
 }
 
@@ -1444,6 +1447,20 @@
   member_con_mask_ = a.kc.con_mask & ~kc_.con_mask;
   check(hipMemcpyAsync(d_args_, &a, sizeof a, hipMemcpyHostToDevice, stream_), "upload args");
   check(hipStreamSynchronize(stream_), "sync args");
+  args_enter_snapshot_ = true;
+}
+
+void EnsembleCore::set_entry_half(bool snapshot) {
+  if (snapshot == args_enter_snapshot_) return;
+  struct { const double *state_in; const unsigned *status_in; } e;
+  static_assert(offsetof(HxBuffers, status_in) == offsetof(HxBuffers, state_in) + sizeof(const double *),
+                "state_in and status_in are written together");
+  e.state_in = snapshot ? d_state_ + (size_t)npad_ * HX_NSTATE(B_) : d_state_;
+  e.status_in = snapshot ? d_status_ + (size_t)npad_ : d_status_;
+  char *dst = reinterpret_cast<char *>(d_args_) + offsetof(HxArgs, buf) + offsetof(HxBuffers, state_in);
+  check(hipMemcpyAsync(dst, &e, sizeof e, hipMemcpyHostToDevice, stream_), "entry half");
+  check(hipStreamSynchronize(stream_), "sync entry half");
+  args_enter_snapshot_ = snapshot;
 }
 
 void EnsembleCore::run_gas_kernel() {
@@ -2062,6 +2079,7 @@
   }
   spin_valid_ = uniform;
   need_spinup_ = false;
+  entry_pending_ = false;
   ++out_epoch_;
   last_iy_ = 0;
   hist_valid_to_ = 0;
@@ -2086,13 +2104,10 @@
   if (iy == last_iy_) return;
   if (iy > last_iy_) throw std::runtime_error("reset: date is after the current date");
   const size_t np = (size_t)npad_, rows = (size_t)HX_NSTATE(B_);
-  sync();
   if (iy == 0) {
-    check(hipMemcpyAsync(d_state_, d_state_ + np * rows, sizeof(double) * np * rows,
-                         hipMemcpyDeviceToDevice, stream_), "restore state");
-    check(hipMemcpyAsync(d_status_, d_status_ + np, sizeof(unsigned) * np, hipMemcpyDeviceToDevice,
-                         stream_), "restore status");
+    entry_pending_ = true;
   } else {
+    sync();
     if (!d_hist_ || iy > hist_valid_to_)
       throw std::runtime_error("reset: no state history for that date (enable_history() before "
                                "running; only reset(0) and reset(startDate) work without it)");
@@ -2104,6 +2119,17 @@
   last_iy_ = iy;
   cost_from_iy_ = -1;
   if (dirty_from_iy_ >= iy) dirty_from_iy_ = -1;
+}
+
+void EnsembleCore::materialize_entry() {
+  if (!entry_pending_) return;
+  entry_pending_ = false;
+  if (!d_state_ || last_iy_ != 0) return;
+  const size_t np = (size_t)npad_, rows = (size_t)HX_NSTATE(B_);
+  check(hipMemcpyAsync(d_state_, d_state_ + np * rows, sizeof(double) * np * rows,
+                       hipMemcpyDeviceToDevice, stream_), "restore state");
+  check(hipMemcpyAsync(d_status_, d_status_ + np, sizeof(unsigned) * np, hipMemcpyDeviceToDevice,
+                       stream_), "restore status");
 }
 
 void EnsembleCore::prewarm_begin() {
@@ -2149,10 +2175,9 @@
   }
   dirty_from_iy_ = -1;
   if (target < last_iy_ + 1) return;
-  if (last_iy_ == 0) {
-    check(hipMemsetAsync(d_cost_, 0, sizeof(double) * (size_t)npad_, stream_), "zero lane cost");
-    cost_from_iy_ = 0;
-  }
+  if (last_iy_ == 0) cost_from_iy_ = 0;
+  set_entry_half(last_iy_ == 0);
+  entry_pending_ = false;
   last_run_prewarmed_ = false;
   prewarm_end();
   check(hipEventRecord(ev0_, stream_), "event");
@@ -2699,17 +2724,40 @@
 
 void EnsembleCore::stats_async(const std::string &capability, int year0, int year1,
                                double *d_stats) {
-  const PostSource ps = post_source(capability, "stats");
-  if (ps.v >= 0 && !d_out_[ps.v])
-    throw std::runtime_error("variable " + capability + " was not enabled with set_outputs()");
-  if (year0 < scen_.start || year1 > scen_.start + ps.last_iy || year1 < year0)
-    throw std::runtime_error("stats: dates must lie between startDate and the current date");
-  check(hx_launch_stats(ps.block, n_, npad_, year0 - scen_.start, year1 - year0 + 1, d_stats,
-                        stream_), "stats kernel");
+  stats_async(std::vector<std::string>{capability}, year0, year1, d_stats);
+}
+
+void EnsembleCore::stats_async(const std::vector<std::string> &capabilities, int year0, int year1,
+                               double *d_stats) {
+  const int ny = year1 - year0 + 1;
+  std::vector<const double *> blocks;
+  size_t done = 0;
+  bool kept_block = false;
+  auto flush = [&]() {
+    if (blocks.empty()) return;
+    check(hx_launch_stats(blocks.data(), (int)blocks.size(), n_, npad_, year0 - scen_.start, ny,
+                          d_stats + done * (size_t)ny * 5, stream_), "stats kernel");
+    done += blocks.size();
+    blocks.clear();
+    kept_block = false;
+  };
+  for (const std::string &capability : capabilities) {
+    const bool derived = find_series(capability) < 0 && (derived_of(capability) || combo_of(capability));
+    if (derived && kept_block) flush();
+    const PostSource ps = post_source(capability, "stats");
+    if (ps.v >= 0 && !d_out_[ps.v])
+      throw std::runtime_error("variable " + capability + " was not enabled with set_outputs()");
+    if (year0 < scen_.start || year1 > scen_.start + ps.last_iy || year1 < year0)
+      throw std::runtime_error("stats: dates must lie between startDate and the current date");
+    blocks.push_back(ps.block);
+    kept_block = kept_block || derived;
+  }
+  flush();
 }
 
 void EnsembleCore::status(unsigned *out_host) {
   prepare();
+  materialize_entry();
   sync();
   std::vector<unsigned> tmp((size_t)npad_);
   check(hipMemcpy(tmp.data(), d_status_, sizeof(unsigned) * (size_t)npad_, hipMemcpyDeviceToHost),
@@ -2719,6 +2767,7 @@
 
 void EnsembleCore::state_row(int row, double *out_host) {
   prepare();
+  materialize_entry();
   sync();
   if (row < 0 || row >= HX_NSTATE(B_)) throw std::runtime_error("state_row: bad row");
   std::vector<double> tmp((size_t)npad_);
diff --git a/hector_amd/csrc/ensemble_core.hpp b/hector_amd/csrc/ensemble_core.hpp
--- a/hector_amd/csrc/ensemble_core.hpp
+++ b/hector_amd/csrc/ensemble_core.hpp
@@ -93,6 +93,7 @@
   const double *device_var(const std::string &capability, int *npad);
   void stats_device(const std::string &capability, int year0, int year1, double *d_stats);
   void stats_async(const std::string &capability, int year0, int year1, double *d_stats);
+  void stats_async(const std::vector<std::string> &capabilities, int year0, int year1, double *d_stats);
   int member_score(const std::string &capability, const int *years, const double *obs,
                    const double *sigma, int n, int base_year0, int base_year1, double *out_host);
   void member_score_whitened(const std::string &capability, const int *years, const double *obs,
@@ -207,6 +208,10 @@
   std::vector<int> uploaded_order_;
   bool spin_valid_ = false;
   int last_iy_ = 0;
+  bool entry_pending_ = false;
+  void materialize_entry();
+  bool args_enter_snapshot_ = true;
+  void set_entry_half(bool snapshot);
   HxConst kc_{};
   std::vector<double> member_series_[HXM_N];
   std::map<int, std::vector<double>> member_points_[HXM_N];
diff --git a/hector_amd/csrc/hx_dev_member.h b/hector_amd/csrc/hx_dev_member.h
--- a/hector_amd/csrc/hx_dev_member.h
+++ b/hector_amd/csrc/hx_dev_member.h
@@ -285,6 +285,13 @@
 __device__ __forceinline__ void sto_(const HxBuffers &b, int var, size_t off, double v) {
   HX_GD(b.out[var])[off] = v;
 }
+__device__ __forceinline__ const double *hx_entry_state(const HxBuffers &b) { return b.state_in; }
+__device__ __forceinline__ unsigned hx_entry_status(const HxBuffers &b, int mem) {
+  return HX_GU(b.status_in)[mem];
+}
+__device__ __forceinline__ double lde_(const double *st, const HxBuffers &b, int row, int mem) {
+  return HX_GCD(st)[(size_t)row * b.npad + mem];
+}
 
 template <int B>
 __device__ __forceinline__ void bind_member(const HxBuffers &buf, int mem, Member<B> &m,
@@ -388,28 +395,28 @@
 }
 
 template <int B>
-__device__ __forceinline__ void load_state(const HxBuffers &buf, int mem, Member<B> &m) {
-  m.cHL = lds_(buf, HXS_C_HL, mem); m.cLL = lds_(buf, HXS_C_LL, mem);
-  m.cIO = lds_(buf, HXS_C_IO, mem); m.cDO = lds_(buf, HXS_C_DO, mem);
-  m.atmos = lds_(buf, HXS_ATMOS, mem); m.earth = lds_(buf, HXS_EARTH, mem);
-  m.cum_luc_va = lds_(buf, HXS_CUM_LUC_VA, mem);
-  m.cum_pf_ch4 = lds_(buf, HXS_CUM_PF_CH4, mem);
-  m.masstot = lds_(buf, HXS_MASSTOT, mem);
-  m.max_ts = lds_(buf, HXS_MAX_TS, mem);
-  m.ts_timeout = (int)lds_(buf, HXS_TS_TIMEOUT, mem);
-  m.lastflux_ann = lds_(buf, HXS_LASTFLUX_ANN, mem);
-  m.sdt = lds_(buf, HXS_SOLVER_DT, mem);
-  if constexpr (!hx_w2<B>()) { m.alkH = lds_(buf, HXS_ALK_HL, mem); m.alkL = lds_(buf, HXS_ALK_LL, mem); }
-  m.hH = lds_(buf, HXS_H_HL, mem); m.hL = lds_(buf, HXS_H_LL, mem);
+__device__ __forceinline__ void load_state(const HxBuffers &buf, int mem, Member<B> &m, const double *st) {
+  m.cHL = lde_(st, buf, HXS_C_HL, mem); m.cLL = lde_(st, buf, HXS_C_LL, mem);
+  m.cIO = lde_(st, buf, HXS_C_IO, mem); m.cDO = lde_(st, buf, HXS_C_DO, mem);
+  m.atmos = lde_(st, buf, HXS_ATMOS, mem); m.earth = lde_(st, buf, HXS_EARTH, mem);
+  m.cum_luc_va = lde_(st, buf, HXS_CUM_LUC_VA, mem);
+  m.cum_pf_ch4 = lde_(st, buf, HXS_CUM_PF_CH4, mem);
+  m.masstot = lde_(st, buf, HXS_MASSTOT, mem);
+  m.max_ts = lde_(st, buf, HXS_MAX_TS, mem);
+  m.ts_timeout = (int)lde_(st, buf, HXS_TS_TIMEOUT, mem);
+  m.lastflux_ann = lde_(st, buf, HXS_LASTFLUX_ANN, mem);
+  m.sdt = lde_(st, buf, HXS_SOLVER_DT, mem);
+  if constexpr (!hx_w2<B>()) { m.alkH = lde_(st, buf, HXS_ALK_HL, mem); m.alkL = lde_(st, buf, HXS_ALK_LL, mem); }
+  m.hH = lde_(st, buf, HXS_H_HL, mem); m.hL = lde_(st, buf, HXS_H_LL, mem);
 #pragma unroll hx_ur<B>()
   for (int b = 0; b < nbio<B>(m); ++b) {
     const int r = HXS_NGLOBAL + b * HXSB_N;
-    m.veg[b] = lds_(buf, r + HXSB_VEG, mem); m.det[b] = lds_(buf, r + HXSB_DET, mem);
-    m.soil[b] = lds_(buf, r + HXSB_SOIL, mem); m.pf[b] = lds_(buf, r + HXSB_PF, mem);
-    m.thawed[b] = lds_(buf, r + HXSB_THAWED, mem);
-    m.tempferts[b] = lds_(buf, r + HXSB_TEMPFERTS, mem);
-  }
-  m.status = HX_GU(buf.status)[mem];
+    m.veg[b] = lde_(st, buf, r + HXSB_VEG, mem); m.det[b] = lde_(st, buf, r + HXSB_DET, mem);
+    m.soil[b] = lde_(st, buf, r + HXSB_SOIL, mem); m.pf[b] = lde_(st, buf, r + HXSB_PF, mem);
+    m.thawed[b] = lde_(st, buf, r + HXSB_THAWED, mem);
+    m.tempferts[b] = lde_(st, buf, r + HXSB_TEMPFERTS, mem);
+  }
+  m.status = hx_entry_status(buf, mem);
 }
 
 template <int B>
diff --git a/hector_amd/csrc/hx_dev_pair.h b/hector_amd/csrc/hx_dev_pair.h
--- a/hector_amd/csrc/hx_dev_pair.h
+++ b/hector_amd/csrc/hx_dev_pair.h
@@ -281,10 +281,12 @@
   const HxConst &kc = args->kc;
   const size_t np = (size_t)buf.npad;
   hx_wave_stamp(buf, 2 * blockIdx.x + role, 0, lane);
-  unsigned status = HX_GU(buf.status)[mem];
+  const double *st_in = hx_entry_state(buf);
+  if (iy_from == 0 && role == 0 && buf.cost) HX_GD(buf.cost)[mem] = 0.0;
+  unsigned status = hx_entry_status(buf, mem);
   PairCtl c;
-  c.sdt = lds_(buf, HXS_SOLVER_DT, mem);
-  c.max_ts = lds_(buf, HXS_MAX_TS, mem);
+  c.sdt = lde_(st_in, buf, HXS_SOLVER_DT, mem);
+  c.max_ts = lde_(st_in, buf, HXS_MAX_TS, mem);
   c.alive = status == 0;
   c.nsteps = 0;
   int par = 0;
@@ -296,16 +298,16 @@
 #endif
 
   if (role == 0) {
-    double cHL = lds_(buf, HXS_C_HL, mem), cLL = lds_(buf, HXS_C_LL, mem),
-           cIO = lds_(buf, HXS_C_IO, mem), cDO = lds_(buf, HXS_C_DO, mem);
-    double atmos = lds_(buf, HXS_ATMOS, mem);
-    const double alkH = lds_(buf, HXS_ALK_HL, mem), alkL = lds_(buf, HXS_ALK_LL, mem);
-    double hH = lds_(buf, HXS_H_HL, mem);
-    int ts_timeout = (int)lds_(buf, HXS_TS_TIMEOUT, mem);
-    double lastflux_ann = lds_(buf, HXS_LASTFLUX_ANN, mem);
-    double tland = lds_(buf, HXS_TLAND, mem), sst = lds_(buf, HXS_SST, mem),
-           f_prev = lds_(buf, HXS_F_PREV, mem), base_tot = lds_(buf, HXS_BASE_TOT, mem),
-           base_co2 = lds_(buf, HXS_BASE_CO2, mem);
+    double cHL = lde_(st_in, buf, HXS_C_HL, mem), cLL = lde_(st_in, buf, HXS_C_LL, mem),
+           cIO = lde_(st_in, buf, HXS_C_IO, mem), cDO = lde_(st_in, buf, HXS_C_DO, mem);
+    double atmos = lde_(st_in, buf, HXS_ATMOS, mem);
+    const double alkH = lde_(st_in, buf, HXS_ALK_HL, mem), alkL = lde_(st_in, buf, HXS_ALK_LL, mem);
+    double hH = lde_(st_in, buf, HXS_H_HL, mem);
+    int ts_timeout = (int)lde_(st_in, buf, HXS_TS_TIMEOUT, mem);
+    double lastflux_ann = lde_(st_in, buf, HXS_LASTFLUX_ANN, mem);
+    double tland = lde_(st_in, buf, HXS_TLAND, mem), sst = lde_(st_in, buf, HXS_SST, mem),
+           f_prev = lde_(st_in, buf, HXS_F_PREV, mem), base_tot = lde_(st_in, buf, HXS_BASE_TOT, mem),
+           base_co2 = lde_(st_in, buf, HXS_BASE_CO2, mem);
     const double C0 = ldp(buf, HXP_C0, mem), p_aero = ldp(buf, HXP_AERO, mem),
                  p_vol = ldp(buf, HXP_VOL, mem);
     const double kLH = ldd(buf, HXD_KLH, mem), kLI = ldd(buf, HXD_KLI, mem),
@@ -651,21 +653,21 @@
 #pragma unroll
     for (int b = 0; b < NB; ++b) {
       const int rs = HXS_NGLOBAL + b * HXSB_N;
-      veg[b] = lds_(buf, rs + HXSB_VEG, mem); det[b] = lds_(buf, rs + HXSB_DET, mem);
-      soil[b] = lds_(buf, rs + HXSB_SOIL, mem); pf[b] = lds_(buf, rs + HXSB_PF, mem);
-      thawed[b] = lds_(buf, rs + HXSB_THAWED, mem); tempferts[b] = lds_(buf, rs + HXSB_TEMPFERTS, mem);
-      ffrozen[b] = lds_(buf, rs + HXSB_F_FROZEN, mem);
+      veg[b] = lde_(st_in, buf, rs + HXSB_VEG, mem); det[b] = lde_(st_in, buf, rs + HXSB_DET, mem);
+      soil[b] = lde_(st_in, buf, rs + HXSB_SOIL, mem); pf[b] = lde_(st_in, buf, rs + HXSB_PF, mem);
+      thawed[b] = lde_(st_in, buf, rs + HXSB_THAWED, mem); tempferts[b] = lde_(st_in, buf, rs + HXSB_TEMPFERTS, mem);
+      ffrozen[b] = lde_(st_in, buf, rs + HXSB_F_FROZEN, mem);
     }
-    double earth = lds_(buf, HXS_EARTH, mem), cum_luc_va = lds_(buf, HXS_CUM_LUC_VA, mem),
-           cum_pf_ch4 = lds_(buf, HXS_CUM_PF_CH4, mem), masstot = lds_(buf, HXS_MASSTOT, mem);
-    const double eos = lds_(buf, HXS_EOS_VEGC, mem);
-    double ch4 = lds_(buf, HXS_CH4, mem), ln_ch4 = hx_log(ch4), o3 = 0;
-    double twin = lds_(buf, HXS_TWIN, mem), tl_m1 = lds_(buf, HXS_TL_M1, mem),
-           tl_m2 = lds_(buf, HXS_TL_M2, mem);
-    double tland = lds_(buf, HXS_TLAND, mem);
-    double lnc = hx_log(hx_div(lds_(buf, HXS_ATMOS, mem) * PGC2PPM, ldp(buf, HXP_C0, mem)));
-    double cLL = lds_(buf, HXS_C_LL, mem), hL = lds_(buf, HXS_H_LL, mem);
-    const double alkL = lds_(buf, HXS_ALK_LL, mem);
+    double earth = lde_(st_in, buf, HXS_EARTH, mem), cum_luc_va = lde_(st_in, buf, HXS_CUM_LUC_VA, mem),
+           cum_pf_ch4 = lde_(st_in, buf, HXS_CUM_PF_CH4, mem), masstot = lde_(st_in, buf, HXS_MASSTOT, mem);
+    const double eos = lde_(st_in, buf, HXS_EOS_VEGC, mem);
+    double ch4 = lde_(st_in, buf, HXS_CH4, mem), ln_ch4 = hx_log(ch4), o3 = 0;
+    double twin = lde_(st_in, buf, HXS_TWIN, mem), tl_m1 = lde_(st_in, buf, HXS_TL_M1, mem),
+           tl_m2 = lde_(st_in, buf, HXS_TL_M2, mem);
+    double tland = lde_(st_in, buf, HXS_TLAND, mem);
+    double lnc = hx_log(hx_div(lde_(st_in, buf, HXS_ATMOS, mem) * PGC2PPM, ldp(buf, HXP_C0, mem)));
+    double cLL = lde_(st_in, buf, HXS_C_LL, mem), hL = lde_(st_in, buf, HXS_H_LL, mem);
+    const double alkL = lde_(st_in, buf, HXS_ALK_LL, mem);
     double npp0[NB], f_nppv[NB], f_nppd[NB], f_litterd[NB], rh_ch4_frac[NB], fpf_static[NB], beta[NB], wf[NB],
         lnq10[NB], pmu[NB], psigma[NB];
 #pragma unroll
diff --git a/hector_amd/csrc/hx_fleet.cpp b/hector_amd/csrc/hx_fleet.cpp
--- a/hector_amd/csrc/hx_fleet.cpp
+++ b/hector_amd/csrc/hx_fleet.cpp
@@ -1013,11 +1013,22 @@
   ensure_comm();
   const int world = comm_ready_ ? world_ : 1;
   const size_t nv = caps.size(), rows = nv * (size_t)ny, blk = rows * 5;
+  if (world == 1 && shards_.size() == 1) {
+    Shard &s = shards_[0];
+    use(s);
+    if (!d_out) ensure_stats_buffers(blk);
+    double *dst = d_out ? d_out : s.d_result;
+    s.core->stats_async(caps, year0, year1, dst);
+    if (out_host)
+      hip_ck(hipMemcpyAsync(out_host, dst, sizeof(double) * blk, hipMemcpyDeviceToHost,
+                            s.core->stream()), "stats result to host");
+    hip_ck(hipStreamSynchronize(s.core->stream()), "stats sync");
+    return;
+  }
   ensure_stats_buffers(blk);
   for (Shard &s : shards_) {
     use(s);
-    for (size_t v = 0; v < nv; ++v)
-      s.core->stats_async(caps[v], year0, year1, s.d_local + v * (size_t)ny * 5);
+    s.core->stats_async(caps, year0, year1, s.d_local);
   }
   if (world == 1) {
     Shard &s = shards_[0];
diff --git a/hector_amd/csrc/hx_kernels.hip b/hector_amd/csrc/hx_kernels.hip
--- a/hector_amd/csrc/hx_kernels.hip
+++ b/hector_amd/csrc/hx_kernels.hip
@@ -459,22 +459,29 @@
   for (int k = 0; k < HX_NCLK; ++k) hx_s_clk[k] = 0;
   hx_s_clk[HX_NCLK] = (long long)__builtin_readcyclecounter();
 #endif
-  load_state<B>(args->buf, mem, m);
+  const double *st_in = hx_entry_state(args->buf);
+  if (iy_from == 0 && args->buf.cost) HX_GD(args->buf.cost)[mem] = 0.0;
+  load_state<B>(args->buf, mem, m, st_in);
   {
     const HxBuffers &buf = args->buf;
-    PKM(m, PK_CH4) = lds_(buf, HXS_CH4, mem); PKM(m, PK_SST) = lds_(buf, HXS_SST, mem);
-    if constexpr (!hx_w2<B>()) PKM(m, PK_EOS) = lds_(buf, HXS_EOS_VEGC, mem);
-    PKM(m, PK_TLAND) = lds_(buf, HXS_TLAND, mem);
-    PKM(m, PK_TWIN) = lds_(buf, HXS_TWIN, mem); PKM(m, PK_TL_M1) = lds_(buf, HXS_TL_M1, mem);
-    PKM(m, PK_TL_M2) = lds_(buf, HXS_TL_M2, mem); PKM(m, PK_F_PREV) = lds_(buf, HXS_F_PREV, mem);
-    PKM(m, PK_BASE_TOT) = lds_(buf, HXS_BASE_TOT, mem);
-    PKM(m, PK_BASE_CO2) = lds_(buf, HXS_BASE_CO2, mem);
-    PKM(m, PK_LN_CH4) = hx_log(lds_(buf, HXS_CH4, mem));
+    PKM(m, PK_CH4) = lde_(st_in, buf, HXS_CH4, mem); PKM(m, PK_SST) = lde_(st_in, buf, HXS_SST, mem);
+    if constexpr (!hx_w2<B>()) PKM(m, PK_EOS) = lde_(st_in, buf, HXS_EOS_VEGC, mem);
+    PKM(m, PK_TLAND) = lde_(st_in, buf, HXS_TLAND, mem);
+    PKM(m, PK_TWIN) = lde_(st_in, buf, HXS_TWIN, mem); PKM(m, PK_TL_M1) = lde_(st_in, buf, HXS_TL_M1, mem);
+    PKM(m, PK_TL_M2) = lde_(st_in, buf, HXS_TL_M2, mem); PKM(m, PK_F_PREV) = lde_(st_in, buf, HXS_F_PREV, mem);
+    PKM(m, PK_BASE_TOT) = lde_(st_in, buf, HXS_BASE_TOT, mem);
+    PKM(m, PK_BASE_CO2) = lde_(st_in, buf, HXS_BASE_CO2, mem);
+    PKM(m, PK_LN_CH4) = hx_log(lde_(st_in, buf, HXS_CH4, mem));
     PKM(m, PK_LN_CO2R) = hx_log(hx_div(m.atmos * PGC2PPM, m.C0));
     if constexpr (!hx_slim_park<B>()) {
 #pragma unroll hx_ur<B>()
     for (int b = 0; b < nbio<B>(m); ++b)
-      PKM(m, pk_ff0<B>() + b) = lds_(buf, HXS_NGLOBAL + b * HXSB_N + HXSB_F_FROZEN, mem);
+      PKM(m, pk_ff0<B>() + b) = lde_(st_in, buf, HXS_NGLOBAL + b * HXSB_N + HXSB_F_FROZEN, mem);
+    } else if (iy_from == 0) {
+#pragma unroll hx_ur<B>()
+      for (int b = 0; b < nbio<B>(m); ++b)
+        sts_(buf, HXS_NGLOBAL + b * HXSB_N + HXSB_F_FROZEN, mem,
+             lde_(st_in, buf, HXS_NGLOBAL + b * HXSB_N + HXSB_F_FROZEN, mem));
     }
   }
   constexpr bool want_hf = HF;
@@ -1420,10 +1427,10 @@
   dst[(size_t)y * n + mem] = src[(size_t)y * npad + lane_of_member[mem]];
 }
 
-__global__ __launch_bounds__(256) void hx_stats_kernel(const double *var, int n, int npad,
+__global__ __launch_bounds__(256) void hx_stats_kernel(HxStatVars vars, int n, int npad,
                                                        int iy0, double *stats) {
   const int iy = iy0 + blockIdx.x;
-  const double *row = var + (size_t)iy * npad;
+  const double *row = vars.var[blockIdx.y] + (size_t)iy * npad;
   double sa[4] = {0, 0, 0, 0}, qa[4] = {0, 0, 0, 0};
   double mn = INFINITY, mx = -INFINITY;
   const int n2 = n >> 1;
@@ -1467,7 +1474,7 @@
     for (int k = 1; k < 4; ++k) { red[0][0] += red[k][0]; red[0][1] += red[k][1];
       red[0][2] += red[k][2]; red[0][3] = fmin(red[0][3], red[k][3]);
       red[0][4] = fmax(red[0][4], red[k][4]); }
-    double *o = stats + (size_t)blockIdx.x * 5;
+    double *o = stats + ((size_t)blockIdx.y * gridDim.x + blockIdx.x) * 5;
     o[0] = red[0][0]; o[1] = red[0][1]; o[2] = red[0][2]; o[3] = red[0][3]; o[4] = red[0][4];
   }
 }
@@ -2053,9 +2060,15 @@
                      world, rows, out);
   return hipGetLastError();
 }
-hipError_t hx_launch_stats(const double *var, int n, int npad, int iy0, int nyears,
+hipError_t hx_launch_stats(const double *const *vars, int nvars, int n, int npad, int iy0, int nyears,
                            double *stats, hipStream_t st) {
-  hipLaunchKernelGGL(hx_stats_kernel, dim3(nyears), dim3(256), 0, st, var, n, npad, iy0, stats);
+  for (int v0 = 0; v0 < nvars; v0 += HX_STATS_MAXV) {
+    const int nv = nvars - v0 < HX_STATS_MAXV ? nvars - v0 : HX_STATS_MAXV;
+    HxStatVars t;
+    for (int k = 0; k < HX_STATS_MAXV; ++k) t.var[k] = k < nv ? vars[v0 + k] : nullptr;
+    hipLaunchKernelGGL(hx_stats_kernel, dim3(nyears, nv), dim3(256), 0, st, t, n, npad, iy0,
+                       stats + (size_t)v0 * nyears * 5);
+  }
   return hipGetLastError();
 }
 }
diff --git a/hector_amd/csrc/hx_layout.h b/hector_amd/csrc/hx_layout.h
--- a/hector_amd/csrc/hx_layout.h
+++ b/hector_amd/csrc/hx_layout.h
@@ -195,6 +195,8 @@
   double *spin_rec;
   double *bscratch;
   long long *wave_clk;
+  const double *state_in;
+  const unsigned *status_in;
   double *out[HXO_NVAR];
 };
 enum { HXSR_NBP = 0, HXSR_NPP, HXSR_RH, HXSR_RH_DET, HXSR_RH_SOIL, HXSR_ATMOS_C, HXSR_CA_RESIDUAL,
@@ -205,6 +207,11 @@
 enum HxDiagKind {
   HXG_TEMP = 0, HXG_DIC, HXG_CO3, HXG_OMEGA_AR, HXG_OMEGA_CA, HXG_REVELLE, HXG_OCEAN_TAS,
   HXG_RF_N2O, HXG_RF_CH4, HXG_RF_H2O, HXG_RF_O3
+};
+
+#define HX_STATS_MAXV 8
+struct HxStatVars {
+  const double *var[HX_STATS_MAXV];
 };
 
 struct HxDiagArgs {
```

Measured after the change: 6.369 billion (median of 6 runs). About the same (+0.6%).
